# MarinerQ/npf_GWwaveform

Measured on AMD Instinct MI355X. Metric: waveform target-points/sec (train step), higher is better.
Workload: dtype f32 (every contraction of the step: fp32 operands as three exact bf16 terms, six v_mfma_f32_16x16x32_bf16 per product group, f32 accumulation -- f32 results, DESIGN.md 3.1 / 3.2; the 1-4-wide first / last layers: f32 FMAs); 1 GPU; BASELINE config 2: AttnCNP scaledot, r=256, 4-layer xy-encoder/decoder, 256 context / 1024 target points, 256 tasks per GPU (256 global), fp32 train step (fwd+loss+bwd+allreduce+Adam); tasks_per_gpu=256, global_tasks=256, context_points=256, target_points=1024, r_dim=256, n_params=799588, parallelism=dp1, hip_graph=True

## Files before the change

include/npf_hip.h:

```cpp
#ifndef NPF_HIP_H
#define NPF_HIP_H

#include <stdint.h>

#ifdef __cplusplus
extern "C" {
#endif

#define NPF_OK 0
#define NPF_EINVAL (-1)
#define NPF_ELAUNCH (-2)

#define NPF_MAX_OPS 40
#define NPF_MAX_FEATURES 512

enum npf_opcode {
  NPF_OP_END = 0,
  NPF_OP_LOAD_PT = 1,
  NPF_OP_STORE_PT = 2,
  NPF_OP_LOAD_ROWS = 3,
  NPF_OP_STORE_ROWS = 4,
  NPF_OP_LINEAR = 5,
  NPF_OP_SOFTMAX = 6,
  NPF_OP_ADD_PT = 7,
  NPF_OP_MASK_POS = 8,
  NPF_OP_ADD_TASKVEC = 9,
  NPF_OP_ROWDOT_PT = 10,
  NPF_OP_SOFTMAX_BWD = 11,
  NPF_OP_RELU = 12,
  NPF_OP_SCALE = 13,
  NPF_OP_STORE_TR = 14,
  NPF_OP_LAYERNORM = 15,
  NPF_OP_STORE_WB = 18,
  NPF_OP_STORE_TRB = 19,
  NPF_OP_LOAD_RM = 17,
  NPF_OP_STORE_MASK = 20,
  NPF_OP_MASK_BITS = 21,
  NPF_OP_LAYERNORM_BWD = 16
};

enum npf_wmode {
  NPF_W_ROWMAJOR = 0,
  NPF_W_PT_ROWS = 1,
  NPF_W_PT_COLS = 2
};

#define NPF_F_RELU 1u
#define NPF_F_ADD_PT 2u
#define NPF_F_MASK_PT 4u
#define NPF_F_P16 16u
#define NPF_F_MASK_BITS 32u
#define NPF_F_ADD_RM 8u
#define NPF_F_STORE_IN 64u
#define NPF_F_STORE_BITS 256u
#define NPF_F_STORE_P16 128u

typedef struct npf_op {
  int32_t op;
  int32_t i0;
  int32_t i1;
  int32_t i2;
  int32_t i3;
  uint32_t flags;
  float f0;
  int32_t i4;
  const void *p0;
  const void *p1;
  const void *p2;
  int64_t s0;
  int64_t s1;
  void *p3;
} npf_op_t;

typedef struct npf_program {
  int32_t n_ops;
  int32_t n_tasks;
  int32_t pts_per_task;
  int32_t tiles_per_task;
  int32_t wg_per_task;
  int32_t reserved[3];
  npf_op_t ops[NPF_MAX_OPS];
} npf_program_t;

int npf_chain_run(const npf_program_t *prog, void *stream);

typedef struct npf_wgrad_job {
  const float *dZ;
  const float *A;
  float *dW;
  float *db;
  int64_t ldw;
  int32_t N, K;
  int32_t per_task;
  int32_t accumulate;
  int32_t ldz, lda, ldo;
  int32_t reserved;
} npf_wgrad_job_t;
#define NPF_WGRAD_ACCUMULATE 1
#define NPF_WGRAD_BF16 2
#define NPF_WGRAD_DZ16 4
#define NPF_WGRAD_A16 8
#define NPF_WGRAD_F32X6 16
#define NPF_WGRAD_NO_H16 32

#define NPF_MAX_WGRAD_JOBS 16
int npf_wgrad_run(const npf_wgrad_job_t *jobs, int32_t n_jobs, int32_t n_tasks, int32_t tiles_per_task,
                  float *partials, int64_t partials_bytes, void *stream);
int64_t npf_wgrad_partials_bytes(const npf_wgrad_job_t *jobs, int32_t n_jobs, int32_t n_tasks,
                                 int32_t tiles_per_task);

int npf_gauss_head_fwd(const float *suff, int32_t n_rows, int32_t pts, int32_t dy, int32_t homoskedastic,
                       const float *Y, int32_t n_y_rows, float *loc, float *scale, float *sum_logp,
                       void *stream);
int npf_gauss_head_bwd(const float *suff, const float *loc, const float *scale, int32_t n_rows, int32_t pts,
                       int32_t dy, int32_t homoskedastic, const float *Y, int32_t n_y_rows,
                       const float *d_loc, const float *d_scale, const float *d_sum_logp, float *d_suff,
                       void *stream);

int npf_masked_gauss_head_fwd(const float *suff, const int32_t *n_valid, int32_t n_tasks, int32_t n_rows, int32_t pts, int32_t dy,
                              int32_t homoskedastic, const float *Y, int32_t n_y_rows, float *loc, float *scale,
                              float *sum_logp, void *stream);
int npf_masked_gauss_head_bwd(const float *suff, const float *loc, const float *scale, const int32_t *n_valid, int32_t n_tasks,
                              int32_t n_rows, int32_t pts, int32_t dy, int32_t homoskedastic, const float *Y, int32_t n_y_rows,
                              const float *d_loc, const float *d_scale, const float *d_sum_logp, float *d_suff, void *stream);

int npf_mixture_summary(const float *suff, const int32_t *n_valid, int32_t n_z, int32_t n_tasks, int32_t pts, int32_t dy,
                        int32_t homoskedastic, const float *z_p, int32_t n_probs, const float *probs, float *mean, float *std,
                        float *quant, void *stream);

int npf_mixture_score(const float *suff, const float *Y, const int32_t *n_valid, int32_t n_z, int32_t n_tasks, int32_t pts,
                      int32_t dy, int32_t homoskedastic, float *log_density, float *pit, float *crps, void *stream);

int npf_mc_objective_fwd(const float *log_w, int32_t n_z, int32_t n_tasks, int32_t mode, const float *inv_weights,
                         int32_t m, float *out, void *stream);
int npf_mc_objective_bwd(const float *log_w, int32_t n_z, int32_t n_tasks, int32_t mode, const float *inv_weights,
                         int32_t m, const float *d_out, float *d_log_w, float *workspace, void *stream);

int npf_mean_agg_fwd(const float *R_pt, int32_t n_tasks, int32_t pts_per_task, int32_t F, float *out,
                     void *stream);
int npf_mean_agg_bwd(const float *d_out, int32_t n_tasks, int32_t pts_per_task, int32_t F, float *dR_pt,
                     int32_t accumulate, void *stream);

int npf_pack_pt(const float *rows, int32_t n_tasks, int32_t pts_per_task, int32_t F_valid, float *pt,
                void *stream);
int npf_unpack_pt(const float *pt, int32_t n_tasks, int32_t pts_per_task, int32_t F_valid, float *rows,
                  void *stream);
int npf_transpose(const float *src, int32_t rows, int32_t cols, float *dst, void *stream);
int npf_split_heads(const float *src, int32_t n_tasks, int32_t pts_per_task, int32_t F, int32_t n_heads, float *dst,
                    void *stream);
int npf_merge_heads(const float *src, int32_t n_tasks, int32_t pts_per_task, int32_t F, int32_t n_heads, float *dst,
                    void *stream);

int npf_mha_fwd(const float *q, const float *k, const float *v, int32_t n_tasks, int32_t n_heads, int32_t n_keys,
                int32_t n_queries, int32_t F, float *out, float *lse, void *stream);
int npf_mha_bwd(const float *q, const float *k, const float *v, const float *out, const float *d_out, const float *lse,
                int32_t n_tasks, int32_t n_heads, int32_t n_keys, int32_t n_queries, int32_t F, float *d_q, float *d_k, float *d_v,
                void *stream);

int npf_add_layernorm_fwd(const float *a, const float *b, const float *gamma, const float *beta, float eps, int32_t n_tasks,
                          int32_t pts_per_task, int32_t F, float *y, float *stats, void *stream);
int npf_add_layernorm_bwd(const float *a, const float *b, const float *gamma, const float *stats, const float *dy, int32_t n_tasks,
                          int32_t pts_per_task, int32_t F, float *dx, float *partials, void *stream);

int npf_gather_points(const float *x, const float *y, const int64_t *idx, int32_t n_tasks, int32_t n_points,
                      int32_t n_sel, int32_t x_dim, int32_t y_dim, float *out_x, float *out_y, void *stream);

int npf_cast_bf16_weights(const float *src, int32_t n_rows, int32_t n_cols, int32_t ld, int32_t transposed, void *dst,
                          void *stream);

typedef struct npf_wprep_job {
  const float *src;
  void *dst;
  int32_t n_rows, n_cols, ld, kind;
} npf_wprep_job_t;
#define NPF_MAX_WPREP_JOBS 32
int npf_prepare_weights(const npf_wprep_job_t *jobs, int32_t n_jobs, void *stream);

#define NPF_X6_MAX_LAYERS 8
typedef struct {
  const void *w_img;
  const float *bias;
  const float *mask;
  float *store_in;
  float *store_out;
  const float *addend;
  unsigned long long *store_bits;
  const unsigned long long *mask_bits;
  int32_t relu;
  int32_t reserved;
} npf_x6_layer_t;
int npf_mlp_x6_run(const npf_x6_layer_t *layers, int32_t n_layers, const float *x, float *y, int32_t n_tasks,
                   int32_t tiles_per_task, void *stream);
int npf_mlp_x6_run_rows(const npf_x6_layer_t *layers, int32_t n_layers, const float *x, const float *in_rows, const float *in_w,
                        float *y, const float *out_w, const float *out_b, float *out_rows, int32_t n_tasks,
                        int32_t tiles_per_task, void *stream);

#define NPF_X6_MAX_OPS 12
typedef struct npf_x6_op {
  const float *in_pt;
  const float *in_rows;
  const float *in_w;
  const float *in_b;
  const float *pre_add;
  const float *mask;
  const unsigned long long *mask_bits;
  const float *sbwd_p;
  float *store_in;
  unsigned long long *store_in_bits;
  const void *w_img;
  int64_t w_task_stride;
  const float *bias;
  int64_t bias_task_stride;
  const float *addend;
  float *store_out;
  unsigned long long *store_bits;
  int32_t in_n;
  int32_t in_relu;
  int32_t relu;
  int32_t softmax_n;
  float softmax_scale;
  float sbwd_scale;
  int32_t reserved[2];
} npf_x6_op_t;
#define NPF_X6_IN_RM 1
#define NPF_X6_ADD_RM 2
#define NPF_X6_STORE_IN_F32 4
#define NPF_X6_STORE_OUT_F32 8
#define NPF_X6_DEFAULT_VARIANT 3
int npf_x6_run_ex(const npf_x6_op_t *ops, int32_t n_ops, const float *out_w, const float *out_b, float *out_rows,
                  int32_t n_tasks, int32_t tiles_per_task, int32_t pts_per_task, int32_t per_task, int32_t width,
                  int32_t variant, void *stream);
int npf_x6_run(const npf_x6_op_t *ops, int32_t n_ops, const float *out_w, const float *out_b, float *out_rows,
               int32_t n_tasks, int32_t tiles_per_task, int32_t per_task, int32_t width, void *stream);
int npf_x6_task_images(const float *src, int32_t n_tasks, int32_t pts, int32_t width, void *row_img, void *tr_img, void *stream);

int npf_b16_run(const npf_x6_op_t *ops, int32_t n_ops, const float *out_w, const float *out_b, float *out_rows, int32_t n_tasks,
                int32_t tiles_per_task, int32_t per_task, int32_t width, int32_t variant, void *stream);
int npf_b16_task_images(const float *src, int32_t n_tasks, int32_t pts, int32_t width, void *row_img, void *tr_img, void *stream);

int npf_masked_attn_fwd(const float *q, const float *k, const float *v, const int32_t *n_valid, int32_t n_tasks, int32_t n_keys,
                        int32_t n_queries, int32_t d, float scale, float *out, float *lse, void *stream);
int npf_masked_attn_bwd(const float *q, const float *k, const float *v, const int32_t *n_valid, const float *out, const float *d_out,
                        const float *lse, int32_t n_tasks, int32_t n_keys, int32_t n_queries, int32_t d, float scale, float *d_q,
                        float *d_k, float *d_v, void *stream);
int npf_masked_attn_fwd_nq(const float *q, const float *k, const float *v, const int32_t *n_valid, const int32_t *n_q_valid,
                           int32_t n_tasks, int32_t n_keys, int32_t n_queries, int32_t d, float scale, float *out, float *lse,
                           void *stream);
int npf_masked_attn_bwd_nq(const float *q, const float *k, const float *v, const int32_t *n_valid, const int32_t *n_q_valid,
                           const float *out, const float *d_out, const float *lse, int32_t n_tasks, int32_t n_keys, int32_t n_queries,
                           int32_t d, float scale, float *d_q, float *d_k, float *d_v, void *stream);
int npf_masked_attn_fwd_prefix(const float *q, const float *k_pre, const float *v_pre, const int32_t *n_prefix, const float *k_tail,
                               const float *v_tail, const int32_t *n_tail, const int32_t *n_q_valid, int32_t n_tasks,
                               int32_t n_prefix_tasks, int32_t c_pad, int32_t m_tail, int32_t n_queries, int32_t d, float scale,
                               float *out, void *stream);
int npf_masked_attn_fwd_loo(const float *q, const float *k, const float *v, const int32_t *n_valid, const int32_t *n_q_valid,
                            int32_t n_tasks, int32_t n_keys, int32_t n_queries, int32_t d, float scale, float *out, void *stream);
int npf_masked_mean_fwd(const float *R_pt, const int32_t *n_valid, int32_t n_tasks, int32_t pts_per_task, int32_t F, float *out,
                        void *stream);
int npf_masked_mean_bwd(const float *d_out, const int32_t *n_valid, int32_t n_tasks, int32_t pts_per_task, int32_t F, float *dR_pt,
                        int32_t accumulate, void *stream);
int npf_loo_mean(const float *R_pt, const int32_t *n_valid, int32_t n_tasks, int32_t pts_per_task, int32_t F, float *out,
                 void *stream);

#define NPF_APPEND_MAX_PAIRS 3
typedef struct npf_append_pair {
  const float *src;
  float *dst;
  int32_t F;
  int32_t reserved;
} npf_append_pair_t;
int npf_append_points(const npf_append_pair_t *pairs, int32_t n_pairs, int32_t *n_valid, const int32_t *n_new, int32_t n_tasks,
                      int32_t n_rows, int32_t capacity, void *stream);

int npf_version(void);

#ifdef __cplusplus
}
#endif
#endif
```

npf_gwwaveform_amd/_lib.py:

```python
from __future__ import annotations

import ctypes as C
import os
from typing import Optional

import torch

from . import _build

NPF_MAX_OPS = 40
NPF_MAX_FEATURES = 512
NPF_WGRAD_BLOCK = 256
NPF_MAX_FUSED_ROW = 256

OP_END, OP_LOAD_PT, OP_STORE_PT, OP_LOAD_ROWS, OP_STORE_ROWS, OP_LINEAR, OP_SOFTMAX, OP_ADD_PT, OP_MASK_POS, \
    OP_ADD_TASKVEC, OP_ROWDOT_PT, OP_SOFTMAX_BWD, OP_RELU, OP_SCALE, OP_STORE_TR, OP_LAYERNORM, OP_LAYERNORM_BWD, OP_LOAD_RM, OP_STORE_WB, OP_STORE_TRB, \
    OP_STORE_MASK, OP_MASK_BITS = range(22)
W_ROWMAJOR, W_PT_ROWS, W_PT_COLS = range(3)
F_RELU, F_ADD_PT, F_MASK_PT, F_ADD_RM, F_P16, F_MASK_BITS, F_STORE_IN, F_STORE_P16, F_STORE_BITS = 1, 2, 4, 8, 16, 32, 64, 128, 256


class NpfOp(C.Structure):
    _fields_ = [
        ("op", C.c_int32), ("i0", C.c_int32), ("i1", C.c_int32), ("i2", C.c_int32), ("i3", C.c_int32),
        ("flags", C.c_uint32), ("f0", C.c_float), ("i4", C.c_int32),
        ("p0", C.c_void_p), ("p1", C.c_void_p), ("p2", C.c_void_p),
        ("s0", C.c_int64), ("s1", C.c_int64), ("p3", C.c_void_p),
    ]


class NpfProgram(C.Structure):
    _fields_ = [
        ("n_ops", C.c_int32), ("n_tasks", C.c_int32), ("pts_per_task", C.c_int32), ("tiles_per_task", C.c_int32),
        ("wg_per_task", C.c_int32), ("reserved", C.c_int32 * 3),
        ("ops", NpfOp * NPF_MAX_OPS),
    ]


class NpfWgradJob(C.Structure):
    _fields_ = [
        ("dZ", C.c_void_p), ("A", C.c_void_p), ("dW", C.c_void_p), ("db", C.c_void_p), ("ldw", C.c_int64),
        ("N", C.c_int32), ("K", C.c_int32), ("per_task", C.c_int32), ("accumulate", C.c_int32),
        ("ldz", C.c_int32), ("lda", C.c_int32), ("ldo", C.c_int32), ("reserved", C.c_int32),
    ]


NPF_MAX_WGRAD_JOBS = 16
WGRAD_F32X6 = 16
WGRAD_NO_H16 = 32


class NpfWprepJob(C.Structure):
    _fields_ = [("src", C.c_void_p), ("dst", C.c_void_p), ("n_rows", C.c_int32), ("n_cols", C.c_int32), ("ld", C.c_int32),
                ("kind", C.c_int32)]


NPF_MAX_WPREP_JOBS = 32
NPF_X6_MAX_LAYERS = 8


class NpfX6Layer(C.Structure):
    _fields_ = [("w_img", C.c_void_p), ("bias", C.c_void_p), ("mask", C.c_void_p), ("store_in", C.c_void_p),
                ("store_out", C.c_void_p), ("addend", C.c_void_p), ("store_bits", C.c_void_p), ("mask_bits", C.c_void_p),
                ("relu", C.c_int32), ("reserved", C.c_int32)]


NPF_X6_MAX_OPS = 12
X6_IN_RM, X6_ADD_RM = 1, 2
X6_STORE_IN_F32, X6_STORE_OUT_F32 = 4, 8


class NpfX6Op(C.Structure):
    _fields_ = [("in_pt", C.c_void_p), ("in_rows", C.c_void_p), ("in_w", C.c_void_p), ("in_b", C.c_void_p),
                ("pre_add", C.c_void_p), ("mask", C.c_void_p), ("mask_bits", C.c_void_p), ("sbwd_p", C.c_void_p),
                ("store_in", C.c_void_p), ("store_in_bits", C.c_void_p), ("w_img", C.c_void_p), ("w_task_stride", C.c_int64),
                ("bias", C.c_void_p), ("bias_task_stride", C.c_int64), ("addend", C.c_void_p), ("store_out", C.c_void_p),
                ("store_bits", C.c_void_p), ("in_n", C.c_int32), ("in_relu", C.c_int32), ("relu", C.c_int32),
                ("softmax_n", C.c_int32), ("softmax_scale", C.c_float), ("sbwd_scale", C.c_float), ("reserved", C.c_int32 * 2)]


NPF_APPEND_MAX_PAIRS = 3


class NpfAppendPair(C.Structure):
    _fields_ = [("src", C.c_void_p), ("dst", C.c_void_p), ("F", C.c_int32), ("reserved", C.c_int32)]


assert C.sizeof(NpfAppendPair) == 24
assert C.sizeof(NpfX6Op) == 17 * 8 + 8 * 4
assert C.sizeof(NpfOp) == 80 and C.sizeof(NpfProgram) == 32 + 80 * NPF_MAX_OPS and C.sizeof(NpfWgradJob) == 72 and C.sizeof(NpfWprepJob) == 32

_i32, _i64, _p = C.c_int32, C.c_int64, C.c_void_p
SIGNATURES = {
    "npf_chain_run": (C.c_int, [C.POINTER(NpfProgram), _p]),
    "npf_wgrad_run": (C.c_int, [C.POINTER(NpfWgradJob), _i32, _i32, _i32, _p, _i64, _p]),
    "npf_wgrad_partials_bytes": (_i64, [C.POINTER(NpfWgradJob), _i32, _i32, _i32]),
    "npf_gauss_head_fwd": (C.c_int, [_p, _i32, _i32, _i32, _i32, _p, _i32, _p, _p, _p, _p]),
    "npf_gauss_head_bwd": (C.c_int, [_p, _p, _p, _i32, _i32, _i32, _i32, _p, _i32, _p, _p, _p, _p, _p]),
    "npf_mc_objective_fwd": (C.c_int, [_p, _i32, _i32, _i32, _p, _i32, _p, _p]),
    "npf_mc_objective_bwd": (C.c_int, [_p, _i32, _i32, _i32, _p, _i32, _p, _p, _p, _p]),
    "npf_mean_agg_fwd": (C.c_int, [_p, _i32, _i32, _i32, _p, _p]),
    "npf_mean_agg_bwd": (C.c_int, [_p, _i32, _i32, _i32, _p, _i32, _p]),
    "npf_pack_pt": (C.c_int, [_p, _i32, _i32, _i32, _p, _p]),
    "npf_unpack_pt": (C.c_int, [_p, _i32, _i32, _i32, _p, _p]),
    "npf_transpose": (C.c_int, [_p, _i32, _i32, _p, _p]),
    "npf_cast_bf16_weights": (C.c_int, [_p, _i32, _i32, _i32, _i32, _p, _p]),
    "npf_prepare_weights": (C.c_int, [C.POINTER(NpfWprepJob), _i32, _p]),
    "npf_gather_points": (C.c_int, [_p, _p, _p, _i32, _i32, _i32, _i32, _i32, _p, _p, _p]),
    "npf_split_heads": (C.c_int, [_p, _i32, _i32, _i32, _i32, _p, _p]),
    "npf_merge_heads": (C.c_int, [_p, _i32, _i32, _i32, _i32, _p, _p]),
    "npf_mlp_x6_run": (C.c_int, [C.POINTER(NpfX6Layer), _i32, _p, _p, _i32, _i32, _p]),
    "npf_mlp_x6_run_rows": (C.c_int, [C.POINTER(NpfX6Layer), _i32, _p, _p, _p, _p, _p, _p, _p, _i32, _i32, _p]),
    "npf_x6_run": (C.c_int, [C.POINTER(NpfX6Op), _i32, _p, _p, _p, _i32, _i32, _i32, _i32, _p]),
    "npf_x6_run_ex": (C.c_int, [C.POINTER(NpfX6Op), _i32, _p, _p, _p, _i32, _i32, _i32, _i32, _i32, _i32, _p]),
    "npf_x6_task_images": (C.c_int, [_p, _i32, _i32, _i32, _p, _p, _p]),
    "npf_b16_run": (C.c_int, [C.POINTER(NpfX6Op), _i32, _p, _p, _p, _i32, _i32, _i32, _i32, _i32, _p]),
    "npf_b16_task_images": (C.c_int, [_p, _i32, _i32, _i32, _p, _p, _p]),
    "npf_mha_fwd": (C.c_int, [_p, _p, _p, _i32, _i32, _i32, _i32, _i32, _p, _p, _p]),
    "npf_mha_bwd": (C.c_int, [_p, _p, _p, _p, _p, _p, _i32, _i32, _i32, _i32, _i32, _p, _p, _p, _p]),
    "npf_add_layernorm_fwd": (C.c_int, [_p, _p, _p, _p, C.c_float, _i32, _i32, _i32, _p, _p, _p]),
    "npf_add_layernorm_bwd": (C.c_int, [_p, _p, _p, _p, _p, _i32, _i32, _i32, _p, _p, _p]),
    "npf_masked_attn_fwd": (C.c_int, [_p, _p, _p, _p, _i32, _i32, _i32, _i32, C.c_float, _p, _p, _p]),
    "npf_masked_attn_bwd": (C.c_int, [_p, _p, _p, _p, _p, _p, _p, _i32, _i32, _i32, _i32, C.c_float, _p, _p, _p, _p]),
    "npf_masked_attn_fwd_nq": (C.c_int, [_p, _p, _p, _p, _p, _i32, _i32, _i32, _i32, C.c_float, _p, _p, _p]),
    "npf_masked_attn_bwd_nq": (C.c_int, [_p, _p, _p, _p, _p, _p, _p, _p, _i32, _i32, _i32, _i32, C.c_float, _p, _p, _p, _p]),
    "npf_masked_attn_fwd_prefix": (C.c_int, [_p, _p, _p, _p, _p, _p, _p, _p, _i32, _i32, _i32, _i32, _i32, _i32, C.c_float, _p, _p]),
    "npf_masked_attn_fwd_loo": (C.c_int, [_p, _p, _p, _p, _p, _i32, _i32, _i32, _i32, C.c_float, _p, _p]),
    "npf_loo_mean": (C.c_int, [_p, _p, _i32, _i32, _i32, _p, _p]),
    "npf_masked_gauss_head_fwd": (C.c_int, [_p, _p, _i32, _i32, _i32, _i32, _i32, _p, _i32, _p, _p, _p, _p]),
    "npf_masked_gauss_head_bwd": (C.c_int, [_p, _p, _p, _p, _i32, _i32, _i32, _i32, _i32, _p, _i32, _p, _p, _p, _p, _p]),
    "npf_mixture_summary": (C.c_int, [_p, _p, _i32, _i32, _i32, _i32, _i32, _p, _i32, _p, _p, _p, _p, _p]),
    "npf_mixture_score": (C.c_int, [_p, _p, _p, _i32, _i32, _i32, _i32, _i32, _p, _p, _p, _p]),
    "npf_masked_mean_fwd": (C.c_int, [_p, _p, _i32, _i32, _i32, _p, _p]),
    "npf_masked_mean_bwd": (C.c_int, [_p, _p, _i32, _i32, _i32, _p, _i32, _p]),
    "npf_append_points": (C.c_int, [C.POINTER(NpfAppendPair), _i32, _p, _p, _i32, _i32, _i32, _p]),
    "npf_version": (C.c_int, []),
}

_lib: Optional[C.CDLL] = None


def lib_path() -> str:
    return os.environ.get("NPF_HIP_LIB") or _build.LIB_PATH


def load() -> C.CDLL:
    global _lib
    if _lib is not None:
        return _lib
    path = lib_path()
    if not os.path.exists(path):
        raise RuntimeError(
            f"HIP extension {path} is missing. Build it with `python -m npf_gwwaveform_amd._build` "
            "(needs hipcc); there is no CPU fallback for the neural-process path."
        )
    try:
        lib = C.CDLL(path)
    except OSError as e:
        raise RuntimeError(f"HIP extension {path} failed to load: {e}") from e
    for name, (res, args) in SIGNATURES.items():
        fn = getattr(lib, name)
        fn.restype = res
        fn.argtypes = args
    _lib = lib
    return lib


def check(rc: int, what: str) -> None:
    if rc != 0:
        raise RuntimeError(f"{what} failed with status {rc} "
                           f"({'invalid argument/unsupported size' if rc == -1 else 'kernel launch error'})")


def stream_ptr(device: Optional[torch.device] = None) -> int:
    return torch.cuda.current_stream(device).cuda_stream


def ptr(t: Optional[torch.Tensor], strided: bool = False) -> Optional[int]:
    if t is None:
        return None
    if not t.is_cuda:
        raise RuntimeError("the HIP path takes device tensors only (got a CPU tensor); there is no CPU fallback")
    if t.dtype != torch.float32:
        raise RuntimeError(f"the HIP path computes in fp32 (got {t.dtype})")
    if not strided and not t.is_contiguous():
        raise RuntimeError("tensor handed to the HIP path must be contiguous")
    return t.data_ptr()
```

npf_gwwaveform_amd/chain.py:

```python
from __future__ import annotations

import ctypes as C
import os
import sys
from dataclasses import dataclass, field
from typing import List, Optional, Sequence, Tuple

import torch

from . import _lib as L


PROFILE = None
TRACE = None
DEBUG_ABLATE = 0
FORCE_WG = int(os.environ.get("NPF_FORCE_WG", "0"))
PT16_INTERNAL = os.environ.get("NPF_NO_PT16", "0") != "1"
MASK_BITS = os.environ.get("NPF_NO_MASK_BITS", "0") != "1"
PAD_SMALL_K = os.environ.get("NPF_NO_PAD_SMALL_K", "0") != "1"
DUMP_PROGRAMS = os.environ.get("NPF_DUMP_PROGRAMS", "0") == "1"
FUSE_STORES = os.environ.get("NPF_NO_FUSED_STORE", "0") != "1"
WGRAD_X6 = os.environ.get("NPF_NO_WGRAD_X6", "0") != "1"
X6_NARROW_NATIVE = os.environ.get("NPF_X6_ALL", "0") != "1"
WGRAD_H16 = os.environ.get("NPF_NO_WGRAD_H16", "0") != "1"
# ... 208 lines not shown
            raise ValueError("a program is either all-fp32 or all-bf16")
        ok = W_img.dtype == torch.bfloat16 and W_img.is_contiguous() and W_img.shape[-1] == pad32(K)
        ok = ok and ((W_img.dim() == 3 and W_img.shape[0] == self.n_tasks and W_img.shape[1] >= N) if per_task
                     else tuple(W_img.shape) == (N, pad32(K)))
        if not ok:
            raise ValueError(f"bad bf16 weight image {tuple(W_img.shape)} {W_img.dtype} for a {K}->{N} layer")
        self.bf16 = True
        if true_K is not None:
            self._pad_k += (K - true_K) * N
        p_add, fl_add = self._pt(addend) if addend is not None else (None, 0)
        flags = (L.F_RELU if relu else 0) | ((L.F_ADD_PT | fl_add) if addend is not None else 0)
        p3 = None
        last = self.ops[-1] if self.ops else None
        if FUSE_STORES and last is not None and last.op == L.OP_STORE_PT and last.i0 == pad32(K):
            self.ops.pop()
            p3 = last.p0
            flags |= L.F_STORE_IN | (L.F_STORE_P16 if last.flags & L.F_P16 else 0)
        self.keep.append(W_img)
        self._op(op=L.OP_LINEAR, i0=K, i1=N, i2=L.W_ROWMAJOR, i3=pad32(K) // 2, flags=flags, i4=addend_modulus,
                 p0=W_img.data_ptr(), p1=self._p(bias), p2=p_add, p3=p3,
                 s0=(W_img.shape[1] * pad32(K) // 2 if per_task else 0), s1=b_task_stride)

    def store_wb(self, img, F):
        self.bf16 = True
        self.keep.append(img)
        self._op(op=L.OP_STORE_WB, i0=F, i1=img.shape[1], p0=img.data_ptr())

    def store_trb(self, img, F):
        self.bf16 = True
        self.keep.append(img)
        self._op(op=L.OP_STORE_TRB, i0=F, i1=img.shape[2], p0=img.data_ptr())

    def flops(self) -> int:
        return (sum(2 * o.i0 * o.i1 for o in self.ops if o.op == L.OP_LINEAR) - 2 * self._pad_k) * self.n_tasks * self.pts

    def hbm_bytes(self) -> int:
        pts = self.n_tasks * tiles_of(self.pts) * 32
        per_pt = 0
        fixed = 0
        for o in self.ops:
            if o.op in (L.OP_LOAD_PT, L.OP_STORE_PT, L.OP_ADD_PT, L.OP_MASK_POS, L.OP_ROWDOT_PT, L.OP_SOFTMAX_BWD,
                        L.OP_LOAD_RM):
                per_pt += (2 if o.flags & L.F_P16 else 4) * o.i0
            elif o.op in (L.OP_LOAD_ROWS, L.OP_STORE_ROWS, L.OP_STORE_TR):
                per_pt += 4 * o.i0
            elif o.op in (L.OP_STORE_WB, L.OP_STORE_TRB):
                per_pt += 2 * pad32(o.i0)
            elif o.op in (L.OP_STORE_MASK, L.OP_MASK_BITS):
                per_pt += 16 * ((o.i0 + 127) // 128)
            elif o.op == L.OP_SOFTMAX and o.i1:
                per_pt += 8
            elif o.op == L.OP_LAYERNORM_BWD:
                per_pt += 4 * pad32(o.i0) * (2 if o.p2 else 1)
            elif o.op == L.OP_LINEAR:
                if o.flags & (L.F_ADD_PT | L.F_MASK_PT | L.F_ADD_RM):
                    per_pt += (2 if o.flags & L.F_P16 else 4) * pad32(o.i1)
                if o.flags & (L.F_MASK_BITS | L.F_STORE_BITS):
                    per_pt += 16 * ((pad32(o.i1) + 127) // 128)
                if o.flags & L.F_STORE_IN:
                    per_pt += (2 if o.flags & L.F_STORE_P16 else 4) * pad32(o.i0)
                per_task = o.i2 != L.W_ROWMAJOR or o.s0 != 0
                fixed += 4 * o.i0 * o.i1 * (self.n_tasks if per_task else 1)
        return per_pt * pts + fixed - 4 * self._pad_k

    def launch(self) -> None:
        if not self.ops:
            return
        if PROFILE is not None:
            ev0, ev1 = torch.cuda.Event(enable_timing=True), torch.cuda.Event(enable_timing=True)
            ev0.record()
            self._launch()
            ev1.record()
            PROFILE.append(("chain_kernel", self.flops(), ev0, ev1, self.hbm_bytes()))
        else:
            self._launch()

    def only_rows_loaded(self) -> bool:
        return bool(self.ops) and self.ops[0].op == L.OP_LOAD_ROWS and all(o.op == L.OP_STORE_PT for o in self.ops[1:])

    def describe(self) -> str:
        names = {v: k[3:] for k, v in vars(L).items() if k.startswith("OP_")}
        flag_names = [(L.F_RELU, "relu"), (L.F_ADD_PT, "add_pt"), (L.F_MASK_PT, "mask_pt"), (L.F_ADD_RM, "add_rm"),
                      (L.F_P16, "p16"), (L.F_MASK_BITS, "mask_bits"), (L.F_STORE_IN, "store_in"),
                      (L.F_STORE_P16, "store_p16"), (L.F_STORE_BITS, "store_bits")]
        lines = [f"program: {self.n_tasks} tasks x {self.pts} points, wg_per_task={int(self.wg_per_task)}, bf16={int(self.bf16)}"]
        for o in self.ops:
            fl = "|".join(n for b, n in flag_names if o.flags & b)
            lines.append(f"  {names.get(o.op, o.op):12s} i0={o.i0:4d} i1={o.i1:4d} i2={o.i2} i4={o.i4} {fl}")
        return "\n".join(lines)

    def _launch(self) -> None:
        if DUMP_PROGRAMS:
            print(self.describe(), file=sys.stderr)
        prog = L.NpfProgram()
        prog.n_ops = len(self.ops)
        prog.n_tasks, prog.pts_per_task, prog.tiles_per_task = self.n_tasks, self.pts, tiles_of(self.pts)
        prog.wg_per_task = int(self.wg_per_task)
        prog.reserved[0] = DEBUG_ABLATE
        prog.reserved[1] = FORCE_WG
        prog.reserved[2] = int(self.bf16)
        for i, o in enumerate(self.ops):
            prog.ops[i] = o
        L.check(L.load().npf_chain_run(C.byref(prog), L.stream_ptr()), "npf_chain_run")


def run_wgrad(jobs: Sequence[dict], n_tasks: int, pts: int, device, tag: str = "") -> None:
    if not jobs:
        return
    if PROFILE is not None:
        ev0, ev1 = torch.cuda.Event(enable_timing=True), torch.cuda.Event(enable_timing=True)
        ev0.record()
        _run_wgrad(jobs, n_tasks, pts, device)
        ev1.record()
        padded = n_tasks * tiles_of(pts) * 32
        nbytes = sum((j["dZ"].element_size() * pad32(j["N"]) + j["A"].element_size() * pad32(j["K"])) * padded
                     + 4 * j["N"] * j["K"] * (n_tasks if j.get("per_task") else 1) for j in jobs)
        PROFILE.append(("wgrad_kernel", sum(2 * j["N"] * j["K"] for j in jobs) * n_tasks * pts, ev0, ev1, nbytes, tag))
    else:
        _run_wgrad(jobs, n_tasks, pts, device)


def _block_jobs(jobs: Sequence[dict]) -> List[dict]:
    Bk = L.NPF_WGRAD_BLOCK
    out = []
    for jb in jobs:
        N, K = jb["N"], jb["K"]
        if N <= Bk and K <= Bk:
            out.append(jb)
            continue
        if jb.get("per_task") and N > Bk:
            raise NotImplementedError("per-task weight gradients (attention keys / values) over more than 256 points")
        dZ, A = jb["dZ"], jb["A"]
        Fz, Fa = pad32(N), pad32(K)
        ldw = jb.get("ldw") or K
        for n0 in range(0, N, Bk):
            for k0 in range(0, K, Bk):
                blk = dict(jb, N=min(Bk, N - n0), K=min(Bk, K - k0), ldz=Fz, lda=Fa,
                           dZ_off=n0 * 32, A_off=k0 * 32)
                if jb.get("per_task"):
                    blk.update(dW_off=k0 * 32, ldo=Fa)
                else:
                    blk.update(dW_off=n0 * ldw + k0, ldw=ldw, db=jb.get("db") if k0 == 0 else None, db_off=n0)
                out.append(blk)
    return out


def _run_wgrad(jobs: Sequence[dict], n_tasks: int, pts: int, device) -> None:
    jobs = _block_jobs(jobs)
    x6 = WGRAD_X6 and COMPUTE_DTYPE != "bf16"
    if x6 and X6_NARROW_NATIVE:
        narrow = [jb for jb in jobs if min(jb["N"], jb["K"]) <= 32]
        wide = [jb for jb in jobs if min(jb["N"], jb["K"]) > 32]
        if narrow and wide:
            _launch_wgrad(wide, n_tasks, pts, device, True)
            _launch_wgrad(narrow, n_tasks, pts, device, False)
            return
        x6 = bool(wide)
    _launch_wgrad(jobs, n_tasks, pts, device, x6)


def _launch_wgrad(jobs: Sequence[dict], n_tasks: int, pts: int, device, x6: bool) -> None:
    lib = L.load()
    for i0 in range(0, len(jobs), L.NPF_MAX_WGRAD_JOBS):
        chunk = jobs[i0:i0 + L.NPF_MAX_WGRAD_JOBS]
        arr = (L.NpfWgradJob * len(chunk))()
        for j, jb in enumerate(chunk):
            z16, a16 = jb["dZ"].dtype == torch.bfloat16, jb["A"].dtype == torch.bfloat16
            if (z16 or a16) and COMPUTE_DTYPE != "bf16":
                raise RuntimeError("PT16 operands exist in the bf16 compute mode only")
            arr[j].dZ = (jb["dZ"].data_ptr() if z16 else L.ptr(jb["dZ"])) + jb.get("dZ_off", 0) * jb["dZ"].element_size()
            arr[j].A = (jb["A"].data_ptr() if a16 else L.ptr(jb["A"])) + jb.get("A_off", 0) * jb["A"].element_size()
            arr[j].dW = L.ptr(jb["dW"]) + 4 * jb.get("dW_off", 0)
            arr[j].db = (L.ptr(jb["db"]) + 4 * jb.get("db_off", 0)) if jb.get("db") is not None else None
            arr[j].ldz, arr[j].lda, arr[j].ldo = jb.get("ldz", 0), jb.get("lda", 0), jb.get("ldo", 0)
            arr[j].ldw = jb.get("ldw") or jb["K"]
            arr[j].N, arr[j].K = jb["N"], jb["K"]
            arr[j].per_task = int(jb.get("per_task", False))
            arr[j].accumulate = (int(jb.get("accumulate", False)) | (2 if COMPUTE_DTYPE == "bf16" else 0)
                                 | (4 if z16 else 0) | (8 if a16 else 0)
                                 | (L.WGRAD_F32X6 if x6 else 0) | (L.WGRAD_NO_H16 if (x6 and not WGRAD_H16) else 0))
        nbytes = lib.npf_wgrad_partials_bytes(arr, len(chunk), n_tasks, tiles_of(pts))
        if nbytes < 0:
            raise RuntimeError("npf_wgrad_partials_bytes: invalid wgrad jobs")
        ws = torch.empty((nbytes + 3) // 4, dtype=torch.float32, device=device)
        L.check(lib.npf_wgrad_run(arr, len(chunk), n_tasks, tiles_of(pts), L.ptr(ws), nbytes, L.stream_ptr()),
                "npf_wgrad_run")


def cast_bf16_weights(W: torch.Tensor, transposed: bool = False) -> torch.Tensor:
    N, K = W.shape
    if W.stride(1) != 1:
        raise ValueError("weight rows must be contiguous")
    rows, cols = (K, N) if transposed else (N, K)
    out = torch.empty((rows, pad32(cols)), dtype=torch.bfloat16, device=W.device)
    L.check(L.load().npf_cast_bf16_weights(L.ptr(W, strided=True), N, K, W.stride(0), int(transposed), out.data_ptr(),
                                           L.stream_ptr()), "npf_cast_bf16_weights")
    return out


def prepare_weights(specs: Sequence[Tuple[torch.Tensor, int]], dsts: Optional[Sequence[torch.Tensor]] = None) -> List[torch.Tensor]:
    outs: List[torch.Tensor] = []
    lib = L.load()
    if dsts is not None:
        assert len(dsts) == len(specs) and os.environ.get("NPF_NO_BATCH_PREP") != "1"
    if os.environ.get("NPF_NO_BATCH_PREP") == "1":
        if any(kind & 4 for _, kind in specs):
            raise RuntimeError("NPF_NO_BATCH_PREP needs NPF_NO_PAD_SMALL_K=1 as well")
        return [transpose(W.contiguous()) if kind == 0 else cast_bf16_weights(W, transposed=kind == 2) for W, kind in specs]
    for i0 in range(0, len(specs), L.NPF_MAX_WPREP_JOBS):
        chunk = specs[i0:i0 + L.NPF_MAX_WPREP_JOBS]
        arr = (L.NpfWprepJob * len(chunk))()
        for j, (W, kind) in enumerate(chunk):
            N, K = W.shape
            if W.stride(1) != 1 or W.dtype != torch.float32:
                raise ValueError("weight rows must be contiguous fp32")
            if kind == 0:
                shape, dt = (K, N), torch.float32
            else:
                rows, cols = (K, N) if kind & 3 == 2 else (N, K)
                shape, dt = (rows, 256 if kind & 4 else pad32(cols)), torch.bfloat16
            if dsts is not None:
                out = dsts[i0 + j]
                if tuple(out.shape) != shape or out.dtype != dt or not out.is_contiguous():
                    raise ValueError(f"prepare_weights: destination {tuple(out.shape)} {out.dtype} for an image {shape} {dt}")
            else:
                out = torch.empty(shape, dtype=dt, device=W.device)
            arr[j].src, arr[j].dst = L.ptr(W, strided=True), out.data_ptr()
            arr[j].n_rows, arr[j].n_cols, arr[j].ld, arr[j].kind = N, K, W.stride(0), kind
            outs.append(out)
        L.check(lib.npf_prepare_weights(arr, len(chunk), L.stream_ptr()), "npf_prepare_weights")
    return outs


def transpose(W: torch.Tensor) -> torch.Tensor:
    rows, cols = W.shape
    out = torch.empty((cols, rows), dtype=torch.float32, device=W.device)
    L.check(L.load().npf_transpose(L.ptr(W.contiguous()), rows, cols, L.ptr(out), L.stream_ptr()), "npf_transpose")
    return out


@dataclass
class _Step:
    kind: str
    t: dict = field(default_factory=dict)
    a: dict = field(default_factory=dict)


class Chain:

    def __init__(self, n_tasks: int, pts_per_task: int, device, wg_per_task: bool = False):
        self.n_tasks, self.pts, self.device, self.wg_per_task = n_tasks, pts_per_task, device, wg_per_task
        self.steps: List[_Step] = []
        self.tensors: List[Optional[torch.Tensor]] = []
        self.F = 0

    def _t(self, t: Optional[torch.Tensor]) -> int:
        if t is None:
            return -1
        self.tensors.append(t)
        return len(self.tensors) - 1

    def input_pt(self, t: torch.Tensor, F: int, modulus: int = 0) -> "Chain":
        self.steps.append(_Step("input_pt", {"x": self._t(t)}, {"F": F, "mod": modulus}))
        self.F = F
        return self

    def input_rm(self, t: torch.Tensor, F: int, modulus: int = 0) -> "Chain":
        if F % 32 or not t.is_contiguous() or t.shape[-1] != F:
            raise ValueError("input_rm needs a contiguous tensor with a multiple of 32 features")
        self.steps.append(_Step("input_rm", {"x": self._t(t)}, {"F": F, "mod": modulus}))
        self.F = F
        return self

    def input_rows(self, t: torch.Tensor, kd: int, modulus: int = 0) -> "Chain":
        if kd > 32:
            raise NotImplementedError("row-major chain inputs are limited to 32 features")
        self.steps.append(_Step("input_rows", {"x": self._t(t)}, {"kd": kd, "mod": modulus}))
        self.F = kd
        return self

    def linear(self, W: torch.Tensor, b: Optional[torch.Tensor], relu: bool = False,
               addend: Optional[torch.Tensor] = None, addend_modulus: int = 0,
               bias_per_task: bool = False, addend_rm: bool = False, residual: bool = False) -> "Chain":
        N, K = W.shape
        if residual and N != K:
            raise ValueError(f"a residual layer keeps its width, got {K} -> {N}")
        if addend_rm and (addend is None or N % 32 or not addend.is_contiguous() or addend.shape[-1] != N):
            raise ValueError("a row-major addend must be contiguous with N % 32 == 0 features")
        if K != self.F:
            raise ValueError(f"Linear expects {K} inputs, chain carries {self.F}")
        if max(N, K) > L.NPF_MAX_FEATURES:
            raise NotImplementedError(
                f"layer {K}->{N}: the HIP chain keeps at most {L.NPF_MAX_FEATURES} features in registers")
        if W.stride(1) != 1:
            raise ValueError("weight rows must be contiguous")
        if bias_per_task and not self.wg_per_task:
            raise ValueError("per-task biases need wg_per_task=True")
        self.steps.append(_Step("linear", {"W": self._t(W), "b": self._t(b), "add": self._t(addend)},
                                {"N": N, "K": K, "relu": relu, "mod": addend_modulus, "bpt": bias_per_task,
                                 "add_rm": addend_rm, "res": residual}))
        self.F = N
        return self

    def add_pt(self, t: torch.Tensor, relu: bool = False, modulus: int = 0) -> "Chain":
        self.steps.append(_Step("add_pt", {"x": self._t(t)}, {"F": self.F, "relu": relu, "mod": modulus}))
        return self

    def dropout(self, sign_mask: torch.Tensor, p: float) -> "Chain":
        if not 0.0 <= p < 1.0:
            raise ValueError(f"dropout probability {p}")
        self.steps.append(_Step("dropout", {"m": self._t(sign_mask)}, {"F": self.F, "p": float(p)}))
        return self

    def add_taskvec(self, v: torch.Tensor, relu: bool = False, modulus: int = 0) -> "Chain":
        self.steps.append(_Step("add_taskvec", {"v": self._t(v)}, {"F": self.F, "relu": relu, "mod": modulus}))
        return self

    def layernorm(self, weight: torch.Tensor, bias: torch.Tensor, eps: float = 1e-5) -> "Chain":
        if self.F > L.NPF_MAX_FUSED_ROW or weight.shape != (self.F,) or bias.shape != (self.F,):
            raise ValueError(f"LayerNorm over {self.F} features with parameters {tuple(weight.shape)}")
        self.steps.append(_Step("layernorm", {"g": self._t(weight), "b": self._t(bias)}, {"F": self.F, "eps": float(eps)}))
        return self

    def store_bf16_images(self) -> "Chain":
        self.steps.append(_Step("store_wb", {}, {"F": self.F}))
        self.steps.append(_Step("store_trb", {}, {"F": self.F}))
        return self

    def attn_scores(self, keys_pt: torch.Tensor, n_keys: int, keys_tr: Optional[torch.Tensor] = None,
                    keys_img=None) -> "Chain":
        if not self.wg_per_task:
            raise ValueError("attention needs wg_per_task=True")
        if n_keys > L.NPF_MAX_FUSED_ROW:
# ... 452 lines not shown
```

npf_gwwaveform_amd/csrc/layout_kernels.hip:

```cpp
#include "npf_common.hpp"

namespace npf {

__global__ void pack_pt_kernel(const float* __restrict__ rows, int n_tasks, int pts, int Fv, int Fp, float* __restrict__ pt) {
  const int tiles = (pts + 31) / 32;
  const size_t total = (size_t)n_tasks * tiles * (Fp / 4) * 32;
  for (size_t idx = blockIdx.x * (size_t)blockDim.x + threadIdx.x; idx < total; idx += (size_t)gridDim.x * blockDim.x) {
    const int p = idx & 31;
    const size_t r = idx >> 5;
    const int f4 = r % (Fp / 4);
    const size_t tt = r / (Fp / 4);
    const int tile = tt % tiles;
    const size_t task = tt / tiles;
    const int point = tile * 32 + p;
    f32x4 v = {0.f, 0.f, 0.f, 0.f};
    if (point < pts) {
      const float* src = rows + (task * pts + point) * (size_t)Fv + 4 * f4;
#pragma unroll
      for (int j = 0; j < 4; ++j)
        if (4 * f4 + j < Fv) v[j] = src[j];
    }
    *(f32x4*)(pt + idx * 4) = v;
  }
}

__global__ void unpack_pt_kernel(const float* __restrict__ pt, int n_tasks, int pts, int Fv, int Fp, float* __restrict__ rows) {
  const int tiles = (pts + 31) / 32;
  const size_t total = (size_t)n_tasks * tiles * (Fp / 4) * 32;
  for (size_t idx = blockIdx.x * (size_t)blockDim.x + threadIdx.x; idx < total; idx += (size_t)gridDim.x * blockDim.x) {
    const int p = idx & 31;
    const size_t r = idx >> 5;
    const int f4 = r % (Fp / 4);
    const size_t tt = r / (Fp / 4);
    const int tile = tt % tiles;
    const size_t task = tt / tiles;
    const int point = tile * 32 + p;
    if (point < pts) {
      const f32x4 v = *(const f32x4*)(pt + idx * 4);
      float* dst = rows + (task * pts + point) * (size_t)Fv + 4 * f4;
#pragma unroll
      for (int j = 0; j < 4; ++j)
        if (4 * f4 + j < Fv) dst[j] = v[j];
    }
  }
}

template <bool SPLIT>
__global__ void heads_kernel(const float* __restrict__ src, int n_tasks, int pts, int Fp, int hsz, int n_heads,
                             float* __restrict__ dst) {
  const int tiles = (pts + 31) / 32;
  const int hq = ((hsz + 31) / 32) * 8;
  const int fq = Fp / 4;
  if (SPLIT) {
    const size_t total = (size_t)n_heads * n_tasks * tiles * hq * 32;
    for (size_t idx = blockIdx.x * (size_t)blockDim.x + threadIdx.x; idx < total; idx += (size_t)gridDim.x * blockDim.x) {
      const int p = idx & 31;
      const size_t r = idx >> 5;
      const int q = r % hq;
      const size_t tt = r / hq;
      const int tile = tt % tiles;
      const size_t ht = tt / tiles;
      const int h = ht / n_tasks, b = ht - (size_t)h * n_tasks;
      f32x4 v = {0.f, 0.f, 0.f, 0.f};
      if (4 * q < hsz) v = *(const f32x4*)(src + ((((size_t)b * tiles + tile) * fq + (h * hsz) / 4 + q) * 32 + p) * 4);
      *(f32x4*)(dst + idx * 4) = v;
    }
  } else {
    const size_t total = (size_t)n_tasks * tiles * fq * 32;
    for (size_t idx = blockIdx.x * (size_t)blockDim.x + threadIdx.x; idx < total; idx += (size_t)gridDim.x * blockDim.x) {
      const int p = idx & 31;
      const size_t r = idx >> 5;
      const int q = r % fq;
      const size_t tt = r / fq;
      const int tile = tt % tiles;
      const size_t b = tt / tiles;
      const int h = (4 * q) / hsz, qh = q - (h * hsz) / 4;
      f32x4 v = {0.f, 0.f, 0.f, 0.f};
      if (h < n_heads) v = *(const f32x4*)(src + (((((size_t)h * n_tasks + b) * tiles + tile) * hq + qh) * 32 + p) * 4);
      *(f32x4*)(dst + idx * 4) = v;
    }
  }
}

__global__ void gather_points_kernel(const float* __restrict__ x, const float* __restrict__ y,
                                     const long long* __restrict__ idx, int n_tasks, int n_points, int n_sel, int x_dim,
                                     int y_dim, float* __restrict__ out_x, float* __restrict__ out_y) {
  const size_t total = (size_t)n_tasks * n_sel;
  for (size_t t = blockIdx.x * (size_t)blockDim.x + threadIdx.x; t < total; t += (size_t)gridDim.x * blockDim.x) {
    const size_t b = t / n_sel;
    long long j = idx[t];
    j = j < 0 ? 0 : (j >= n_points ? n_points - 1 : j);
    const float* xs = x + (b * n_points + (size_t)j) * x_dim;
    for (int d = 0; d < x_dim; ++d) out_x[t * x_dim + d] = xs[d];
    if (y) {
      const float* ys = y + (b * n_points + (size_t)j) * y_dim;
      for (int d = 0; d < y_dim; ++d) out_y[t * y_dim + d] = ys[d];
    }
  }
}

__global__ void cast_bf16_weights_kernel(const float* __restrict__ src, int n_rows, int n_cols, int ld, int transposed,
                                         unsigned short* __restrict__ dst) {
  const int rows = transposed ? n_cols : n_rows, cols = transposed ? n_rows : n_cols;
  const int Kp = ((cols + 31) >> 5) * 32;
  const size_t total = (size_t)rows * Kp;
  for (size_t idx = blockIdx.x * (size_t)blockDim.x + threadIdx.x; idx < total; idx += (size_t)gridDim.x * blockDim.x) {
    const int r = idx / Kp, q = idx - (size_t)r * Kp;
    const int sgrp = q >> 5, g = (q & 31) >> 3, i = q & 7;
    const int c = 32 * sgrp + (i < 4 ? 4 * g + i : 16 + 4 * g + (i - 4));
    float v = 0.f;
    if (c < cols) v = transposed ? src[(size_t)c * ld + r] : src[(size_t)r * ld + c];
    const __bf16 b = (__bf16)v;
    dst[idx] = __builtin_bit_cast(unsigned short, b);
  }
}

__global__ void transpose_kernel(const float* __restrict__ src, int rows, int cols, float* __restrict__ dst) {
  __shared__ float tile[32][33];
  const int c0 = blockIdx.x * 32, r0 = blockIdx.y * 32;
  const int tx = threadIdx.x & 31, ty = threadIdx.x >> 5;
  for (int i = ty; i < 32; i += 8)
    if (r0 + i < rows && c0 + tx < cols) tile[i][tx] = src[(size_t)(r0 + i) * cols + c0 + tx];
  __syncthreads();
  for (int i = ty; i < 32; i += 8)
    if (c0 + i < cols && r0 + tx < rows) dst[(size_t)(c0 + i) * rows + r0 + tx] = tile[tx][i];
}

struct WprepJobs {
  npf_wprep_job_t job[NPF_MAX_WPREP_JOBS];
};
__global__ void prepare_weights_kernel(const WprepJobs J) {
  __shared__ float tile[32][33];
  const npf_wprep_job_t& jb = J.job[blockIdx.y];
  const float* __restrict__ src = jb.src;
  if (jb.kind == 0) {
    float* __restrict__ dst = (float*)jb.dst;
    const int rows = jb.n_rows, cols = jb.n_cols, ld = jb.ld;
    const int tc = (cols + 31) / 32, tr = (rows + 31) / 32;
    const int tx = threadIdx.x & 31, ty = threadIdx.x >> 5;
    for (int tl = blockIdx.x; tl < tc * tr; tl += gridDim.x) {
      const int c0 = (tl % tc) * 32, r0 = (tl / tc) * 32;
      for (int i = ty; i < 32; i += 8)
        if (r0 + i < rows && c0 + tx < cols) tile[i][tx] = src[(size_t)(r0 + i) * ld + c0 + tx];
      __syncthreads();
      for (int i = ty; i < 32; i += 8)
        if (c0 + i < cols && r0 + tx < rows) dst[(size_t)(c0 + i) * rows + r0 + tx] = tile[tx][i];
      __syncthreads();
    }
  } else {
    unsigned short* __restrict__ dst = (unsigned short*)jb.dst;
    const bool transposed = (jb.kind & 3) == 2;
    const int term = (jb.kind >> 4) & 3;
    const int rows = transposed ? jb.n_cols : jb.n_rows, cols = transposed ? jb.n_rows : jb.n_cols, ld = jb.ld;
    const int Kp = (jb.kind & 4) ? 256 : ((cols + 31) >> 5) * 32;
    const size_t total = (size_t)rows * Kp;
    for (size_t idx = blockIdx.x * (size_t)blockDim.x + threadIdx.x; idx < total; idx += (size_t)gridDim.x * blockDim.x) {
      const int r = idx / Kp, q = idx - (size_t)r * Kp;
      const int sgrp = q >> 5, g = (q & 31) >> 3, i = q & 7;
      const int c = 32 * sgrp + (i < 4 ? 4 * g + i : 16 + 4 * g + (i - 4));
      float v = 0.f;
      if (c < cols) v = transposed ? src[(size_t)c * ld + r] : src[(size_t)r * ld + c];
      for (int t = 1; t < term; ++t) v -= (float)(__bf16)v;
      const __bf16 b = (__bf16)v;
      dst[idx] = __builtin_bit_cast(unsigned short, b);
    }
  }
}

template <bool MASKED>
__global__ void mean_fwd_kernel(const float* __restrict__ R, const int32_t* __restrict__ n_valid, int pts, int F,
                                float* __restrict__ out) {
  const int tiles = (pts + 31) / 32;
  const int p = threadIdx.x & 31, f4 = blockIdx.x * 8 + (threadIdx.x >> 5);
  const size_t task = blockIdx.y;
  const int n = MASKED ? clamp_count(n_valid, task, pts) : pts;
  const bool in_F = MASKED || f4 < F / 4;
  f32x4 s = {0.f, 0.f, 0.f, 0.f};
  if (in_F) {
    const float* base = R + task * tiles * (size_t)(F * 32) + pt_off(f4, p);
    for (int t = 0; t * 32 < n; ++t)
      if (t * 32 + p < n) s += *(const f32x4*)(base + (size_t)t * F * 32);
  }
#pragma unroll
  for (int off = 16; off >= 1; off >>= 1)
#pragma unroll
    for (int j = 0; j < 4; ++j) s[j] += __shfl_xor(s[j], off);
  if (p == 0 && in_F) *(f32x4*)(out + task * F + 4 * f4) = (!MASKED || n > 0) ? s * (1.f / (float)n) : f32x4{0.f, 0.f, 0.f, 0.f};
}

__global__ void loo_mean_kernel(const float* __restrict__ R, const int32_t* __restrict__ n_valid, int pts, int F,
                                float* __restrict__ out) {
  const int tiles = (pts + 31) / 32;
  const int p = threadIdx.x & 31, f4 = blockIdx.x * 8 + (threadIdx.x >> 5);
  const size_t task = blockIdx.y;
  const int n = clamp_count(n_valid, task, pts);
  const size_t at = task * tiles * (size_t)(F * 32) + pt_off(f4, p);
  double s[4] = {0.0, 0.0, 0.0, 0.0};
  for (int t = 0; t * 32 < n; ++t)
    if (t * 32 + p < n) {
      const f32x4 r = *(const f32x4*)(R + at + (size_t)t * F * 32);
#pragma unroll
      for (int j = 0; j < 4; ++j) s[j] += (double)r[j];
    }
#pragma unroll
  for (int off = 16; off >= 1; off >>= 1)
#pragma unroll
    for (int j = 0; j < 4; ++j) s[j] += __shfl_xor(s[j], off);
  const double others = (double)(n - 1);
  for (int t = 0; t < tiles; ++t) {
    f32x4 v = {0.f, 0.f, 0.f, 0.f};
    if (n > 1 && t * 32 + p < n) {
      const f32x4 r = *(const f32x4*)(R + at + (size_t)t * F * 32);
#pragma unroll
      for (int j = 0; j < 4; ++j) v[j] = (float)((s[j] - (double)r[j]) / others);
    }
    *(f32x4*)(out + at + (size_t)t * F * 32) = v;
  }
}

template <bool MASKED>
__global__ void mean_bwd_kernel(const float* __restrict__ d_out, const int32_t* __restrict__ n_valid, int n_tasks, int pts, int F,
                                float* __restrict__ dR, int accumulate) {
  const int tiles = (pts + 31) / 32;
  const size_t total = (size_t)n_tasks * tiles * (F / 4) * 32;
  for (size_t idx = blockIdx.x * (size_t)blockDim.x + threadIdx.x; idx < total; idx += (size_t)gridDim.x * blockDim.x) {
    const int p = idx & 31;
    const size_t r = idx >> 5;
    const int f4 = r % (F / 4);
    const size_t tt = r / (F / 4);
    const int tile = tt % tiles;
    const size_t task = tt / tiles;
    const int n = MASKED ? clamp_count(n_valid, task, pts) : pts;
    f32x4 v = {0.f, 0.f, 0.f, 0.f};
    if (tile * 32 + p < n) v = *(const f32x4*)(d_out + task * F + 4 * f4) * (1.f / (float)n);
    if (accumulate) v += *(const f32x4*)(dR + idx * 4);
    *(f32x4*)(dR + idx * 4) = v;
  }
}

static unsigned grid_for(size_t total, int block) {
  size_t g = (total + block - 1) / block;
  if (g > 256u * 8u) g = 256u * 8u;
  if (g == 0) g = 1;
  return (unsigned)g;
}

}

extern "C" int npf_pack_pt(const float* rows, int32_t n_tasks, int32_t pts, int32_t Fv, float* pt, void* stream) {
  if (!rows || !pt || n_tasks <= 0 || pts <= 0 || Fv <= 0) return NPF_EINVAL;
  const int Fp = npf::round_up(Fv, 32);
  const size_t total = (size_t)n_tasks * ((pts + 31) / 32) * (Fp / 4) * 32;
  hipLaunchKernelGGL(npf::pack_pt_kernel, dim3(npf::grid_for(total, 256)), dim3(256), 0, (hipStream_t)stream, rows, n_tasks,
                     pts, Fv, Fp, pt);
  NPF_CHECK_LAUNCH();
  return NPF_OK;
}

extern "C" int npf_unpack_pt(const float* pt, int32_t n_tasks, int32_t pts, int32_t Fv, float* rows, void* stream) {
  if (!rows || !pt || n_tasks <= 0 || pts <= 0 || Fv <= 0) return NPF_EINVAL;
  const int Fp = npf::round_up(Fv, 32);
  const size_t total = (size_t)n_tasks * ((pts + 31) / 32) * (Fp / 4) * 32;
  hipLaunchKernelGGL(npf::unpack_pt_kernel, dim3(npf::grid_for(total, 256)), dim3(256), 0, (hipStream_t)stream, pt,
                     n_tasks, pts, Fv, Fp, rows);
  NPF_CHECK_LAUNCH();
  return NPF_OK;
}

extern "C" int npf_transpose(const float* src, int32_t rows, int32_t cols, float* dst, void* stream) {
  if (!src || !dst || rows <= 0 || cols <= 0) return NPF_EINVAL;
  hipLaunchKernelGGL(npf::transpose_kernel, dim3((cols + 31) / 32, (rows + 31) / 32), dim3(256), 0, (hipStream_t)stream,
                     src, rows, cols, dst);
  NPF_CHECK_LAUNCH();
  return NPF_OK;
}

static int heads_launch(bool split, const float* src, int32_t n_tasks, int32_t pts, int32_t F, int32_t n_heads, float* dst,
                        void* stream) {
  if (!src || !dst || n_tasks <= 0 || pts <= 0 || F <= 0 || n_heads <= 0 || F % n_heads) return NPF_EINVAL;
  const int hsz = F / n_heads;
  if (hsz & 3) return NPF_EINVAL;
  const int Fp = npf::round_up(F, 32), tiles = (pts + 31) / 32;
  if (split) {
    const size_t total = (size_t)n_heads * n_tasks * tiles * (npf::round_up(hsz, 32) / 4) * 32;
    hipLaunchKernelGGL(npf::heads_kernel<true>, dim3(npf::grid_for(total, 256)), dim3(256), 0, (hipStream_t)stream, src,
                       n_tasks, pts, Fp, hsz, n_heads, dst);
  } else {
    const size_t total = (size_t)n_tasks * tiles * (Fp / 4) * 32;
    hipLaunchKernelGGL(npf::heads_kernel<false>, dim3(npf::grid_for(total, 256)), dim3(256), 0, (hipStream_t)stream, src,
                       n_tasks, pts, Fp, hsz, n_heads, dst);
  }
  NPF_CHECK_LAUNCH();
  return NPF_OK;
}

extern "C" int npf_gather_points(const float* x, const float* y, const int64_t* idx, int32_t n_tasks, int32_t n_points,
                                 int32_t n_sel, int32_t x_dim, int32_t y_dim, float* out_x, float* out_y, void* stream) {
  if (!x || !idx || !out_x || n_tasks <= 0 || n_points <= 0 || n_sel < 0 || x_dim <= 0) return NPF_EINVAL;
  if (y && (!out_y || y_dim <= 0)) return NPF_EINVAL;
  if (n_sel == 0) return NPF_OK;
  const size_t total = (size_t)n_tasks * n_sel;
  hipLaunchKernelGGL(npf::gather_points_kernel, dim3(npf::grid_for(total, 256)), dim3(256), 0, (hipStream_t)stream, x, y,
                     (const long long*)idx, n_tasks, n_points, n_sel, x_dim, y_dim, out_x, out_y);
  NPF_CHECK_LAUNCH();
  return NPF_OK;
}

extern "C" int npf_cast_bf16_weights(const float* src, int32_t n_rows, int32_t n_cols, int32_t ld, int32_t transposed,
                                     void* dst, void* stream) {
  if (!src || !dst || n_rows <= 0 || n_cols <= 0 || ld < n_cols || (((uintptr_t)dst) & 15)) return NPF_EINVAL;
  const int rows = transposed ? n_cols : n_rows, cols = transposed ? n_rows : n_cols;
  const size_t total = (size_t)rows * npf::round_up(cols, 32);
  hipLaunchKernelGGL(npf::cast_bf16_weights_kernel, dim3(npf::grid_for(total, 256)), dim3(256), 0, (hipStream_t)stream, src,
                     n_rows, n_cols, ld, transposed, (unsigned short*)dst);
  NPF_CHECK_LAUNCH();
  return NPF_OK;
}

extern "C" int npf_prepare_weights(const npf_wprep_job_t* jobs, int32_t n_jobs, void* stream) {
  if (!jobs || n_jobs <= 0 || n_jobs > NPF_MAX_WPREP_JOBS) return NPF_EINVAL;
  npf::WprepJobs J;
  size_t most = 0;
  for (int j = 0; j < n_jobs; ++j) {
    const npf_wprep_job_t& b = jobs[j];
    const int base = b.kind & 15, term = b.kind >> 4;
    const bool kind_ok = b.kind >= 0 && ((term == 0 && (base <= 2 || base == 5 || base == 6)) || (term >= 1 && term <= 3 && (base == 1 || base == 2)));
    if (!b.src || !b.dst || b.n_rows <= 0 || b.n_cols <= 0 || b.ld < b.n_cols || !kind_ok) return NPF_EINVAL;
    if (b.kind != 0 && (((uintptr_t)b.dst) & 15)) return NPF_EINVAL;
    if ((b.kind == 5 && b.n_cols > 256) || (b.kind == 6 && b.n_rows > 256)) return NPF_EINVAL;
    J.job[j] = b;
    const size_t img_rows = (b.kind & 3) == 2 ? b.n_cols : b.n_rows;
    const size_t blocks = b.kind == 0   ? (size_t)((b.n_rows + 31) / 32) * ((b.n_cols + 31) / 32)
                          : (b.kind & 4) ? (img_rows * 256 + 255) / 256
                                         : ((size_t)b.n_rows * b.n_cols + 255) / 256;
    most = blocks > most ? blocks : most;
  }
  for (int j = n_jobs; j < NPF_MAX_WPREP_JOBS; ++j) J.job[j] = jobs[0];
  const unsigned gx = (unsigned)(most < 64 ? most : 64);
  hipLaunchKernelGGL(npf::prepare_weights_kernel, dim3(gx ? gx : 1, n_jobs), dim3(256), 0, (hipStream_t)stream, J);
  NPF_CHECK_LAUNCH();
  return NPF_OK;
}

extern "C" int npf_split_heads(const float* src, int32_t n_tasks, int32_t pts, int32_t F, int32_t n_heads, float* dst,
                               void* stream) {
  return heads_launch(true, src, n_tasks, pts, F, n_heads, dst, stream);
}

extern "C" int npf_merge_heads(const float* src, int32_t n_tasks, int32_t pts, int32_t F, int32_t n_heads, float* dst,
                               void* stream) {
  return heads_launch(false, src, n_tasks, pts, F, n_heads, dst, stream);
}

extern "C" int npf_mean_agg_fwd(const float* R_pt, int32_t n_tasks, int32_t pts, int32_t F, float* out, void* stream) {
  if (!R_pt || !out || n_tasks <= 0 || pts <= 0 || F <= 0 || (F & 31)) return NPF_EINVAL;
  hipLaunchKernelGGL(npf::mean_fwd_kernel<false>, dim3(F / 32, n_tasks), dim3(256), 0, (hipStream_t)stream, R_pt, nullptr, pts, F,
                     out);
  NPF_CHECK_LAUNCH();
  return NPF_OK;
}

extern "C" int npf_mean_agg_bwd(const float* d_out, int32_t n_tasks, int32_t pts, int32_t F, float* dR_pt,
                                int32_t accumulate, void* stream) {
  if (!d_out || !dR_pt || n_tasks <= 0 || pts <= 0 || F <= 0 || (F & 31)) return NPF_EINVAL;
  const size_t total = (size_t)n_tasks * ((pts + 31) / 32) * (F / 4) * 32;
  hipLaunchKernelGGL(npf::mean_bwd_kernel<false>, dim3(npf::grid_for(total, 256)), dim3(256), 0, (hipStream_t)stream, d_out,
                     nullptr, n_tasks, pts, F, dR_pt, accumulate);
  NPF_CHECK_LAUNCH();
  return NPF_OK;
}

extern "C" int npf_masked_mean_fwd(const float* R_pt, const int32_t* n_valid, int32_t n_tasks, int32_t pts, int32_t F, float* out,
                                   void* stream) {
  if (!R_pt || !n_valid || !out || n_tasks < 0 || pts <= 0 || F <= 0 || (F & 31)) return NPF_EINVAL;
  if ((((uintptr_t)R_pt) | ((uintptr_t)out)) & 15) return NPF_EINVAL;
  if (n_tasks == 0) return NPF_OK;
  hipLaunchKernelGGL(npf::mean_fwd_kernel<true>, dim3(F / 32, n_tasks), dim3(256), 0, (hipStream_t)stream, R_pt, n_valid, pts, F, out);
  NPF_CHECK_LAUNCH();
  return NPF_OK;
}

extern "C" int npf_masked_mean_bwd(const float* d_out, const int32_t* n_valid, int32_t n_tasks, int32_t pts, int32_t F, float* dR_pt,
                                   int32_t accumulate, void* stream) {
  if (!d_out || !n_valid || !dR_pt || n_tasks < 0 || pts <= 0 || F <= 0 || (F & 31)) return NPF_EINVAL;
  if ((((uintptr_t)d_out) | ((uintptr_t)dR_pt)) & 15) return NPF_EINVAL;
  if (n_tasks == 0) return NPF_OK;
  const size_t total = (size_t)n_tasks * ((pts + 31) / 32) * (F / 4) * 32;
  hipLaunchKernelGGL(npf::mean_bwd_kernel<true>, dim3(npf::grid_for(total, 256)), dim3(256), 0, (hipStream_t)stream, d_out, n_valid,
                     n_tasks, pts, F, dR_pt, accumulate);
  NPF_CHECK_LAUNCH();
  return NPF_OK;
}

extern "C" int npf_loo_mean(const float* R_pt, const int32_t* n_valid, int32_t n_tasks, int32_t pts, int32_t F, float* out,
                            void* stream) {
  if (!R_pt || !n_valid || !out || n_tasks < 0 || pts <= 0 || F <= 0 || (F & 31)) return NPF_EINVAL;
  if ((((uintptr_t)R_pt) | ((uintptr_t)out)) & 15) return NPF_EINVAL;
  if (n_tasks == 0) return NPF_OK;
  if (n_tasks > 65535) return NPF_EINVAL;
  hipLaunchKernelGGL(npf::loo_mean_kernel, dim3(F / 32, n_tasks), dim3(256), 0, (hipStream_t)stream, R_pt, n_valid, pts, F, out);
  NPF_CHECK_LAUNCH();
  return NPF_OK;
}

extern "C" int npf_version(void) { return 2; }
```

npf_gwwaveform_amd/csrc/wgrad_kernel.hip:

```cpp
#include "npf_common.hpp"

namespace npf {

constexpr int kWgThreads = 1024;
constexpr int kWgWaves = kWgThreads / 64;
constexpr int kWgMaxF = 256;
constexpr int kQRows = kWgMaxF / 4;
constexpr int kMaxJobs = 16;

struct WgradJobs {
  npf_wgrad_job_t job[kMaxJobs];
  int32_t first_wg[kMaxJobs + 1];
  int32_t n_jobs;
  int32_t n_tasks;
  int32_t tiles_per_task;
  int32_t pad;
  int64_t part_off[kMaxJobs];
};

__device__ __forceinline__ void wg_dma16(const float* src, float* lds_dst_wave_uniform) {
  __builtin_amdgcn_global_load_lds((const __attribute__((address_space(1))) void*)src,
                                   (__attribute__((address_space(3))) void*)lds_dst_wave_uniform, 16, 0, 0);
}

// ... 747 lines not shown
        for (int r = 0; r < 16; ++r) {
          const int row = 64 * rg + 32 * i + (r & 3) + 8 * (r >> 2) + row_l, col = 128 * cp + 32 * c + col_l;
          part[(size_t)row * Kp + col] = acc[i][c][r];
        }
#pragma unroll
    for (int v = 0; v < 2; ++v) {
#pragma unroll
      for (int e = 0; e < 4; ++e) {
        float x = dbacc[v][e];
        x += __shfl_xor(x, 1);
        x += __shfl_xor(x, 2);
        x += __shfl_xor(x, 16);
        x += __shfl_xor(x, 32);
        dbacc[v][e] = x;
      }
      if (pt_ld == 0) *(f32x4*)(part + (size_t)Np * Kp + 4 * (8 * wave + 4 * v + q_ld)) = dbacc[v];
    }
  }
}

__global__ void wgrad_reduce_kernel(const WgradJobs J, const float* __restrict__ partials) {
  const int j = blockIdx.y;
  const npf_wgrad_job_t& job = J.job[j];
  if (job.per_task) return;
  const int n_split = J.first_wg[j + 1] - J.first_wg[j];
  const int Np = ((job.N + 31) >> 5) * 32, Kp = ((job.K + 31) >> 5) * 32;
  const size_t slab = (size_t)Np * Kp + Np;
  const float* part = partials + J.part_off[j];
  const int total4 = (Np * Kp + Np) >> 2;
  for (int i4 = blockIdx.x * blockDim.x + threadIdx.x; i4 < total4; i4 += gridDim.x * blockDim.x) {
    const float* p = part + (size_t)i4 * 4;
    f32x4 s0 = {0.f, 0.f, 0.f, 0.f}, s1 = s0, s2 = s0, s3 = s0;
    int sp = 0;
    for (; sp + 4 <= n_split; sp += 4) {
      s0 += *(const f32x4*)(p + (size_t)sp * slab);
      s1 += *(const f32x4*)(p + (size_t)(sp + 1) * slab);
      s2 += *(const f32x4*)(p + (size_t)(sp + 2) * slab);
      s3 += *(const f32x4*)(p + (size_t)(sp + 3) * slab);
    }
    for (; sp < n_split; ++sp) s0 += *(const f32x4*)(p + (size_t)sp * slab);
    const f32x4 s = (s0 + s1) + (s2 + s3);
    const int idx = i4 * 4;
    if (idx < Np * Kp) {
      const int n = idx / Kp, k = idx - n * Kp;
      if (n < job.N) {
        float* d = job.dW + (size_t)n * job.ldw + k;
#pragma unroll
        for (int e = 0; e < 4; ++e)
          if (k + e < job.K) d[e] = (job.accumulate & NPF_WGRAD_ACCUMULATE) ? d[e] + s[e] : s[e];
      }
    } else if (job.db) {
      const int n = idx - Np * Kp;
#pragma unroll
      for (int e = 0; e < 4; ++e)
        if (n + e < job.N) job.db[n + e] = (job.accumulate & NPF_WGRAD_ACCUMULATE) ? job.db[n + e] + s[e] : s[e];
    }
  }
}

static int plan(const npf_wgrad_job_t* jobs, int n_jobs, int n_tasks, int tiles_per_task, WgradJobs* J) {
  if (!jobs || n_jobs <= 0 || n_jobs > kMaxJobs || n_tasks <= 0 || tiles_per_task <= 0) return NPF_EINVAL;
  const long total_tiles = (long)n_tasks * tiles_per_task;
  int n_shared = 0;
  for (int j = 0; j < n_jobs; ++j) {
    const npf_wgrad_job_t& b = jobs[j];
    if (!b.dZ || !b.A || !b.dW || b.N <= 0 || b.K <= 0 || b.N > npf::kWgMaxF || b.K > npf::kWgMaxF) return NPF_EINVAL;
    if ((((uintptr_t)b.dZ) | ((uintptr_t)b.A)) & 15) return NPF_EINVAL;
    if (b.per_task && (((uintptr_t)b.dW) & 15)) return NPF_EINVAL;
    if (!b.per_task && b.ldw < b.K) return NPF_EINVAL;
    if (b.ldz < 0 || b.lda < 0 || b.ldo < 0 || (b.ldz & 31) || (b.lda & 31) || (b.ldo & 31)) return NPF_EINVAL;
    if ((b.ldz && b.ldz < npf::round_up(b.N, 32)) || (b.lda && b.lda < npf::round_up(b.K, 32)) ||
        (b.ldo && b.ldo < npf::round_up(b.K, 32)))
      return NPF_EINVAL;
    n_shared += b.per_task ? 0 : 1;
  }
  bool bf16 = true, x6 = true;
  for (int j = 0; j < n_jobs; ++j) {
    bf16 &= (jobs[j].accumulate & NPF_WGRAD_BF16) != 0;
    x6 &= (jobs[j].accumulate & (NPF_WGRAD_F32X6 | NPF_WGRAD_BF16)) == NPF_WGRAD_F32X6;
  }
  double cost[kMaxJobs], cost_sum = 0.0;
  for (int j = 0; j < n_jobs; ++j) {
    const int Np = npf::round_up(jobs[j].N, 32), Kp = npf::round_up(jobs[j].K, 32);
    const int ar = (Np + 63) / 64, ac = (Kp + 63) / 64;
    const double zb = (jobs[j].accumulate & NPF_WGRAD_DZ16) ? 2.0 : 4.0, ab = (jobs[j].accumulate & NPF_WGRAD_A16) ? 2.0 : 4.0;
    const double bytes = 32.0 * (Np * zb + Kp * ab);
    if (jobs[j].per_task) cost[j] = 0.0;
    else if (bf16) cost[j] = bytes > 18432.0 ? bytes : 18432.0;
    else if (x6) {
      const int waves = ar * ((ac + 1) / 2);
      const double mf = 3072.0 * 1.6 * ((waves + 3) / 4) + 2500.0, mem = bytes / 6.5;
      cost[j] = mf > mem ? mf : mem;
    } else {
      const double mf = 4096.0 * (ar < ac ? ar : ac), mem = bytes / 6.5;
      cost[j] = mf > mem ? mf : mem;
    }
    cost_sum += cost[j];
  }
  J->n_jobs = n_jobs;
  J->n_tasks = n_tasks;
  J->tiles_per_task = tiles_per_task;
  J->pad = 0;
  long splits_of[kMaxJobs];
  long used = 0;
  for (int j = 0; j < n_jobs; ++j) {
    splits_of[j] = 0;
    if (jobs[j].per_task) continue;
    long sp = (long)(256.0 * cost[j] / cost_sum);
    if (sp < 1) sp = 1;
    if (sp > total_tiles) sp = total_tiles;
    splits_of[j] = sp;
    used += sp;
  }
  for (int j = 0; j < n_jobs && used < 256; ++j)
    if (!jobs[j].per_task && cost[j] * n_shared >= cost_sum && splits_of[j] < total_tiles) {
      ++splits_of[j];
      ++used;
    }
  int wg = 0;
  int64_t off = 0;
  for (int j = 0; j < n_jobs; ++j) {
    J->job[j] = jobs[j];
    J->first_wg[j] = wg;
    J->part_off[j] = off;
    if (jobs[j].per_task) {
      wg += n_tasks;
    } else {
      const int Np = npf::round_up(jobs[j].N, 32), Kp = npf::round_up(jobs[j].K, 32);
      const long splits = splits_of[j];
      wg += (int)splits;
      off += (int64_t)splits * ((int64_t)Np * Kp + Np);
    }
  }
  J->first_wg[n_jobs] = wg;
  for (int j = n_jobs + 1; j <= kMaxJobs; ++j) J->first_wg[j] = wg;
  return (int)0;
}

}

extern "C" int64_t npf_wgrad_partials_bytes(const npf_wgrad_job_t* jobs, int32_t n_jobs, int32_t n_tasks,
                                            int32_t tiles_per_task) {
  npf::WgradJobs J;
  if (npf::plan(jobs, n_jobs, n_tasks, tiles_per_task, &J) != 0) return -1;
  int64_t off = 0;
  for (int j = 0; j < n_jobs; ++j) {
    if (jobs[j].per_task) continue;
    const int Np = npf::round_up(jobs[j].N, 32), Kp = npf::round_up(jobs[j].K, 32);
    off += (int64_t)(J.first_wg[j + 1] - J.first_wg[j]) * ((int64_t)Np * Kp + Np);
  }
  return off * 4 + 16;
}

extern "C" int npf_wgrad_run(const npf_wgrad_job_t* jobs, int32_t n_jobs, int32_t n_tasks, int32_t tiles_per_task,
                             float* partials, int64_t partials_bytes, void* stream) {
  npf::WgradJobs J;
  const int rc = npf::plan(jobs, n_jobs, n_tasks, tiles_per_task, &J);
  if (rc != 0) return rc;
  const int64_t need = npf_wgrad_partials_bytes(jobs, n_jobs, n_tasks, tiles_per_task);
  bool any_shared = false;
  for (int j = 0; j < n_jobs; ++j) any_shared |= !jobs[j].per_task;
  if (any_shared && (!partials || partials_bytes < need || (((uintptr_t)partials) & 15))) return NPF_EINVAL;
  const int n_wg = J.first_wg[n_jobs];
  bool bf16 = true, x6 = true;
  for (int j = 0; j < n_jobs; ++j) {
    bf16 &= (jobs[j].accumulate & NPF_WGRAD_BF16) != 0;
    x6 &= (jobs[j].accumulate & (NPF_WGRAD_F32X6 | NPF_WGRAD_BF16)) == NPF_WGRAD_F32X6;
  }
  bool h16 = x6;
  for (int j = 0; j < n_jobs; ++j) h16 &= jobs[j].N == 256 && jobs[j].K == 256 && !(jobs[j].accumulate & NPF_WGRAD_NO_H16);
  if (h16)
    hipLaunchKernelGGL(npf::wgrad_h16_kernel, dim3(n_wg), dim3(512), 0, (hipStream_t)stream, J, partials);
  else if (x6)
    hipLaunchKernelGGL(npf::wgrad_x6_kernel, dim3(n_wg), dim3(npf::kXThreads), 0, (hipStream_t)stream, J, partials);
  else if (bf16)
    hipLaunchKernelGGL(npf::wgrad_kernel<true>, dim3(n_wg), dim3(npf::kWgThreads), 0, (hipStream_t)stream, J, partials);
  else
    hipLaunchKernelGGL(npf::wgrad_kernel<false>, dim3(n_wg), dim3(npf::kWgThreads), 0, (hipStream_t)stream, J, partials);
  NPF_CHECK_LAUNCH();
  if (any_shared) {
    hipLaunchKernelGGL(npf::wgrad_reduce_kernel, dim3(65, n_jobs), dim3(256), 0, (hipStream_t)stream, J,
                       (const float*)partials);
    NPF_CHECK_LAUNCH();
  }
  return NPF_OK;
}
```

npf_gwwaveform_amd/functional.py:

```python
from __future__ import annotations

import os
from typing import Optional

import torch

from . import _lib as L
from .chain import pad32, pt_empty, pt_shape, tiles_of


def _pack(rows: torch.Tensor) -> torch.Tensor:
    n_tasks, pts, F = rows.shape
    out = pt_empty(n_tasks, pts, F, rows.device)
    L.check(L.load().npf_pack_pt(L.ptr(rows.contiguous()), n_tasks, pts, F, L.ptr(out), L.stream_ptr()), "npf_pack_pt")
    return out


def _unpack(pt: torch.Tensor, pts: int, F: int) -> torch.Tensor:
    n_tasks = pt.shape[0]
    out = torch.empty((n_tasks, pts, F), dtype=torch.float32, device=pt.device)
    L.check(L.load().npf_unpack_pt(L.ptr(pt.contiguous()), n_tasks, pts, F, L.ptr(out), L.stream_ptr()), "npf_unpack_pt")
    return out


class _PackFn(torch.autograd.Function):
    @staticmethod
    def forward(ctx, rows):
        ctx.pts, ctx.F = rows.shape[1], rows.shape[2]
        return _pack(rows)

    @staticmethod
    def backward(ctx, g):
        return _unpack(g.contiguous(), ctx.pts, ctx.F)


class _UnpackFn(torch.autograd.Function):
    @staticmethod
    def forward(ctx, pt, pts, F):
        return _unpack(pt, pts, F)

    @staticmethod
    def backward(ctx, g):
        return _pack(g.contiguous()), None, None


def pack_pt(rows: torch.Tensor) -> torch.Tensor:
    return _PackFn.apply(rows)


def unpack_pt(pt: torch.Tensor, pts: int, F: int) -> torch.Tensor:
    return _UnpackFn.apply(pt, pts, F)


def sum_points_pt(pt: torch.Tensor, pts: int, F: int) -> torch.Tensor:
    n_tasks = pt.shape[0]
    Fp = pad32(F)
    out = torch.empty((n_tasks, Fp), dtype=torch.float32, device=pt.device)
    L.check(L.load().npf_mean_agg_fwd(L.ptr(pt), n_tasks, pts, Fp, L.ptr(out), L.stream_ptr()), "npf_mean_agg_fwd")
    return out * float(pts)


class _MeanFn(torch.autograd.Function):

    @staticmethod
    def forward(ctx, pt, n_valid, n_tasks, pts, F):
        Fp = pad32(F)
        ctx.geo = (n_tasks, pts, Fp)
        if n_valid is not None:
            ctx.save_for_backward(n_valid)
        out = torch.empty((n_tasks, Fp), dtype=torch.float32, device=pt.device)
        name, counts = ("npf_mean_agg_fwd", ()) if n_valid is None else ("npf_masked_mean_fwd", (_iptr(n_valid),))
        L.check(getattr(L.load(), name)(L.ptr(pt.contiguous()), *counts, n_tasks, pts, Fp, L.ptr(out), L.stream_ptr()), name)
        return out

    @staticmethod
    def backward(ctx, g):
        n_tasks, pts, Fp = ctx.geo
        d = pt_empty(n_tasks, pts, Fp, g.device)
        name, counts = ("npf_masked_mean_bwd", (_iptr(ctx.saved_tensors[0]),)) if ctx.saved_tensors else ("npf_mean_agg_bwd", ())
        L.check(getattr(L.load(), name)(L.ptr(g.contiguous()), *counts, n_tasks, pts, Fp, L.ptr(d), 0, L.stream_ptr()), name)
        return d, None, None, None, None


def mean_agg(pt: torch.Tensor, pts: int, F: int) -> torch.Tensor:
    return _MeanFn.apply(pt, None, pt.shape[0], pts, F)


class _GaussHeadFn(torch.autograd.Function):

    @staticmethod
    def forward(ctx, suff, Y, n_valid, dy, homosk, want_dist):
        n_rows, pts, two_dy = suff.shape
        n_tasks = 1 if n_valid is None else n_valid.shape[0]
        assert two_dy == 2 * dy and n_rows % n_tasks == 0
        suff = suff.contiguous()
        loc = scale = None
        if want_dist:
            loc = torch.empty((n_rows, pts, dy), dtype=torch.float32, device=suff.device)
            scale = torch.empty_like(loc)
        slp = None
        n_y = 0
        if Y is not None:
            Y = Y.contiguous()
            n_y = Y.shape[0]
            assert Y.shape[1:] == (pts, dy) and n_rows % n_y == 0 and n_y % n_tasks == 0
            slp = torch.empty((n_rows,), dtype=torch.float32, device=suff.device)
        elif not want_dist:
            raise ValueError("a loss-only head launch needs the targets")
        name, counts = ("npf_gauss_head_fwd", ()) if n_valid is None else ("npf_masked_gauss_head_fwd", (_iptr(n_valid), n_tasks))
        L.check(getattr(L.load(), name)(L.ptr(suff), *counts, n_rows, pts, dy, int(homosk), L.ptr(Y), n_y, L.ptr(loc), L.ptr(scale),
                                        L.ptr(slp), L.stream_ptr()), name)
        ctx.save_for_backward(suff, loc, scale, Y, *(() if n_valid is None else (n_valid,)))
        ctx.cfg = (dy, homosk)
        empty = suff.new_zeros((0,))
        outs = [loc if want_dist else empty, scale if want_dist else empty, slp if slp is not None else suff.new_zeros((n_rows,))]
        nd = ([] if want_dist else [outs[0], outs[1]]) + ([] if slp is not None else [outs[2]])
        if nd:
            ctx.mark_non_differentiable(*nd)
        return tuple(outs)

    @staticmethod
    def backward(ctx, d_loc, d_scale, d_slp):
        suff, loc, scale, Y, *n_valid = ctx.saved_tensors
        dy, homosk = ctx.cfg
        n_rows, pts, _ = suff.shape
        d_suff = torch.empty_like(suff)
        c = lambda t: t.contiguous() if t is not None else None
        if loc is None:
            d_loc = d_scale = None
        name, counts = ("npf_masked_gauss_head_bwd", (_iptr(n_valid[0]), n_valid[0].shape[0])) if n_valid else ("npf_gauss_head_bwd", ())
        L.check(getattr(L.load(), name)(L.ptr(suff), L.ptr(loc), L.ptr(scale), *counts, n_rows, pts, dy, int(homosk), L.ptr(Y),
                                        Y.shape[0] if Y is not None else 0, L.ptr(c(d_loc)), L.ptr(c(d_scale)),
                                        L.ptr(c(d_slp)) if Y is not None else None, L.ptr(d_suff), L.stream_ptr()), name)
        return d_suff, None, None, None, None, None


def gauss_head(suff: torch.Tensor, Y: Optional[torch.Tensor], dy: int, homoskedastic: bool, want_dist: bool = True,
               n_valid: Optional[torch.Tensor] = None):
    if n_valid is not None:
        n_tasks = n_valid.shape[0] if isinstance(n_valid, torch.Tensor) and n_valid.dim() == 1 else suff.shape[0]
        if suff.shape[0] % max(n_tasks, 1) != 0 or n_tasks == 0:
            raise ValueError(f"n_valid has {n_tasks} counts, the head {suff.shape[0]} rows (not a multiple)")
        n_valid = counts_i32(n_valid, n_tasks)
    return _GaussHeadFn.apply(suff, Y, n_valid, dy, homoskedastic, want_dist)


MIXTURE_MAX_NZ = 128
_Z_P_CACHE = {}


def check_probs(probs) -> tuple:
    if isinstance(probs, torch.Tensor) or not isinstance(probs, (tuple, list)):
        raise ValueError(f"probs must be a host sequence (tuple / list) of probabilities, got {type(probs).__name__}")
    out = []
    for p in probs:
        if isinstance(p, torch.Tensor) or isinstance(p, bool) or not isinstance(p, (int, float)):
            raise ValueError(f"probs must hold host floats, got {type(p).__name__}")
        if not (0.0 < float(p) < 1.0):
            raise ValueError(f"probs must lie strictly inside (0, 1), got {p}")
        out.append(float(p))
    return tuple(out)


def normal_quantiles(probs) -> tuple:
    probs = check_probs(probs)
    if not probs:
        return ()
    return tuple(torch.special.ndtri(torch.tensor(probs, dtype=torch.float64)).tolist())


def _z_p_device(probs: tuple, device: torch.device):
    key = (probs, device.type, device.index if device.index is not None else torch.cuda.current_device())
    hit = _Z_P_CACHE.get(key)
    if hit is None:
        hit = (torch.tensor(normal_quantiles(probs), dtype=torch.float64).to(torch.float32).to(device),
# ... 422 lines not shown
```

npf_gwwaveform_amd/neuralproc.py:

```python
from __future__ import annotations

import abc
import math
from functools import partial
from typing import NamedTuple, Optional, Tuple

import torch
import torch.nn as nn
from torch.distributions import Independent, Normal

from . import functional as FN
from .architectures import (MLP, DotAttender, LeaveOneOut, MergeFlatInputs, MultiheadAttender, PrefixTail, SelfAttention,
                            get_attender, merge_flat_input)
from .chain import Chain, PTensor, pad32, pt_shape

__all__ = ["NeuralProcessFamily", "LatentNeuralProcessFamily", "CNP", "LNP", "AttnCNP", "AttnLNP",
           "MultivariateNormalDiag", "HeadDistribution", "Conditioned", "Prediction", "Score"]


def MultivariateNormalDiag(loc, scale_diag):
    if loc.dim() < 1:
        raise ValueError("loc must be at least one-dimensional.")
    return Independent(Normal(loc, scale_diag, validate_args=False), 1)

# ... 394 lines not shown
            Xc_pt, R_pts = x6.context_side(self, X_cntxt, Y_cntxt)
            return Xc_pt, self._pool_pt(R_pts, B)
        Xc_pt = self._xenc_pt(X_cntxt, with_tr=self._attentive and not fused_t) if C > 0 else None
        return Xc_pt, self._encode_globally_pt(Xc_pt, Y_cntxt, B, C)

    def _target_stage(self, Xc_pt, R, X_trgt, Y_trgt, B, C, n_cntxt, n_trgt, fused_t, latent=None):
        T = X_trgt.shape[1]
        padded = n_cntxt is not None and C > 0
        n_valid = n_cntxt if padded else None
        X_raw = None
        if padded:
            Xt_pt = self._xenc_pt(X_trgt)
        elif fused_t:
            Xt_pt, X_raw = None, X_trgt
        elif self._xenc_with_query_projection(C, T):
            from . import x6

            Xt_pt, q_proj = x6.xenc_proj(self, X_trgt, self.attender.query_transform)
            Xt_pt.proj = q_proj
        else:
            Xt_pt = self._xenc_pt(X_trgt)
        self._X_trgt_raw = X_raw
        try:
            if latent is not None:
                z_samples, q_zCc, q_zCct = latent[0], latent[1], None
            elif self.encoded_path in ["latent", "both"]:
                z_samples, q_zCc, q_zCct = self._latent_path_pt(R, C, Xt_pt, Y_trgt, B, T, n_valid=n_valid, n_trgt=n_trgt)
            else:
                z_samples, q_zCc, q_zCct = None, None, None
            if self.encoded_path == "latent":
                R = None
            suff = self._target_suffstat(Xc_pt, z_samples, R, Xt_pt, B, C, T, n_valid=n_valid,
                                         n_q_valid=n_trgt if padded else None)
        finally:
            self._X_trgt_raw = None
        return self._head(suff, Y_trgt, B, T, n_trgt=n_trgt), z_samples, q_zCc, q_zCct

    def _n_z_for(self, n_z_samples=None) -> Optional[int]:
        return None

    def condition(self, X_cntxt, Y_cntxt, n_cntxt=None, n_z_samples=None) -> "Conditioned":
        with torch.no_grad():
            n_z = self._n_z_for(n_z_samples)
            if n_cntxt is not None:
                n_cntxt = self._check_counts(n_cntxt, X_cntxt, "n_cntxt")
            self._check_tensors(X_cntxt, Y_cntxt)
            B, C, _ = X_cntxt.shape
            if n_z is not None:
                self.n_z_samples = n_z
            fused_t = self._fused_target_side(C, 1)
            Xc_pt, R = self._context_stage(X_cntxt, Y_cntxt, n_cntxt, fused_t)
            z_samples = q_zCc = None
            if n_z is not None:
                q_zCc = self._infer_q_zCc(R, B, n_cntxt if C > 0 else None)
                z_samples = q_zCc.rsample([n_z])
        return Conditioned(self, Xc_pt, R, z_samples, q_zCc, n_cntxt, B, C, fused_t)

    def condition_with_capacity(self, X_cntxt, Y_cntxt, capacity, n_cntxt=None, n_z_samples=None) -> "Conditioned":
        self._refuse_unimplemented("capacity")
        with torch.no_grad():
            n_z = self._n_z_for(n_z_samples)
            if X_cntxt.dim() != 3 or Y_cntxt.dim() != 3 or X_cntxt.shape[:2] != Y_cntxt.shape[:2]:
                raise ValueError(f"X_cntxt / Y_cntxt must be [B, C, x_dim] / [B, C, y_dim], got {list(X_cntxt.shape)} / {list(Y_cntxt.shape)}")
            B, C, _ = X_cntxt.shape
            capacity = int(capacity)
            if capacity < max(C, 1):
                raise ValueError(f"capacity={capacity} must be at least the context size C={C} (and at least 1)")
            self._check_tensors(X_cntxt, Y_cntxt)
            if n_cntxt is not None:
                n_cntxt = self._check_counts(n_cntxt, X_cntxt, "n_cntxt")
            if n_z is not None:
                self.n_z_samples = n_z
            dev = X_cntxt.device
            R_pts = PTensor(torch.zeros(pt_shape(B, capacity, self.r_dim), device=dev), capacity, self.r_dim)
            Xc_pt = PTensor(torch.zeros(pt_shape(B, capacity, self.x_transf_dim), device=dev), capacity, self.x_transf_dim)
            counts = torch.zeros(B, dtype=torch.int32, device=dev)
            post = Conditioned(self, Xc_pt, R_pts if self._attentive else torch.zeros(B, 1, self.r_dim, device=dev), None, None, counts,
                               B, C, False, capacity=capacity, R_pts=R_pts)
            if C > 0:
                Xn_pt, Rn_pts = self._encode_points(X_cntxt, Y_cntxt)
                pairs = [(Rn_pts.t, R_pts.t, self.r_dim), (Xn_pt.t, Xc_pt.t, self.x_transf_dim)]
                FN.append_points(pairs, counts, n_cntxt, B, C, capacity)
            post._refresh()
            if n_z is not None:
                post.q_zCc = q = self._infer_q_zCc(post._R, B, counts)
                post.eps = torch.randn(n_z, B, 1, self.z_dim, device=dev)
                post.z_samples = q.base_dist.loc + q.base_dist.scale * post.eps
        return post

    def loo(self, X_cntxt, Y_cntxt, n_cntxt=None) -> HeadDistribution:
        self._refuse_loo()
        if X_cntxt.dim() != 3 or Y_cntxt.dim() != 3 or X_cntxt.shape[:2] != Y_cntxt.shape[:2]:
            raise ValueError(f"X_cntxt / Y_cntxt must be [B, C, x_dim] / [B, C, y_dim], got {list(X_cntxt.shape)} / {list(Y_cntxt.shape)}")
        B, C, _ = X_cntxt.shape
        if C == 0:
            raise ValueError("loo: no context points")
        with torch.no_grad():
            if n_cntxt is not None:
                n_cntxt = self._check_counts(n_cntxt, X_cntxt, "n_cntxt")
            self._check_tensors(X_cntxt, Y_cntxt)
            if n_cntxt is None:
                n_cntxt = torch.full((B,), C, dtype=torch.int32, device=X_cntxt.device)
            Xc_pt, R_pts = self._encode_points(X_cntxt, Y_cntxt)
            return self._loo_from(Xc_pt, R_pts, n_cntxt, B, C)

    def _refuse_loo(self):
        if self.encoded_path != "deterministic":
            raise NotImplementedError("loo is not implemented for latent models (LNP / AttnLNP): q(z | C without i) differs per "
                                      "left-out point and the decoder takes one z per task")
        self._refuse_unimplemented("loo")

    def _loo_from(self, Xc_pt, R_pts, n, B, rows) -> HeadDistribution:
        return self._head(self._loo_suffstat(Xc_pt, R_pts, n, B, rows), None, B, rows, n_trgt=n)

    def _decode_pointwise(self, R_t, X1_pt, B, T):
        from . import x6

        if x6.decoder_side_usable(self, T):
            return x6.decoder_side(self, R_t, X1_pt, T)
        ch = Chain(B, T, X1_pt.device, wg_per_task=True)
        ch.input_pt(R_t, self.r_dim)
        return self.decoder.finish_rows(ch, x1_pt=X1_pt)

    def _encode_points(self, X, Y):
        if self._fused_context_side(X.shape[1]):
            from . import x6

            return x6.context_side(self, X, Y)
        X_pt = self._xenc_pt(X)
        return X_pt, self._xyenc_pt(X_pt, Y, with_tr=False)

    def predict(self, X_cntxt, Y_cntxt, X_trgt, n_cntxt=None, n_trgt=None, n_z_samples=None, probs=(0.025, 0.5, 0.975)) -> Prediction:
        probs = FN.check_probs(probs)
        return self.condition(X_cntxt, Y_cntxt, n_cntxt=n_cntxt, n_z_samples=n_z_samples).query(X_trgt, n_trgt=n_trgt).summary(probs)

    def _refuse_unimplemented(self, what):
        from . import chain as _chain

        if getattr(self, "is_self_attn", False):
            raise NotImplementedError(f"{what} is not implemented for self-attention context encoders (is_self_attn=True)")
        if _chain.COMPUTE_DTYPE != "fp32":
            raise NotImplementedError(f"{what} is not implemented in the bf16 compute mode (set_compute_dtype('bf16'))")

    def _check_counts(self, n, X, what):
        self._refuse_unimplemented(what)
        n = FN.counts_i32(n, X.shape[0], what)
        if n.device != X.device:
            raise ValueError(f"{what} lives on {n.device}, the batch on {X.device}")
        return n

    def _validate_inputs(self, X_cntxt, Y_cntxt, X_trgt, Y_trgt):
        self._check_tensors(X_cntxt, Y_cntxt, X_trgt, Y_trgt)
        if self.training and self.validate_inputs:
            m = X_trgt.abs().amax() if X_trgt.numel() else X_trgt.new_zeros(())
            if X_cntxt.numel():
                m = torch.maximum(m, X_cntxt.abs().amax())
            if self.validate_inputs == "deferred":
                if getattr(self, "_range_seen", None) is None or self._range_seen.device != m.device:
                    self._range_seen = torch.zeros((), device=m.device)
                self._range_seen.copy_(torch.maximum(self._range_seen, m))
                return
            if not (m.item() <= 1.0):
                lo = min(X_cntxt.min().item() if X_cntxt.numel() else 0.0, X_trgt.min().item())
                hi = max(X_cntxt.max().item() if X_cntxt.numel() else 0.0, X_trgt.max().item())
                raise ValueError(f"Features during training should be in [-1,1]. Got [{lo}, {hi}].")

    @staticmethod
    def _check_tensors(*tensors):
        for t in tensors:
            if t is not None and (not t.is_cuda or t.dtype != torch.float32):
                raise RuntimeError("the HIP path takes fp32 device tensors only; there is no CPU fallback")

    def check_deferred_inputs(self):
        seen = getattr(self, "_range_seen", None)
        if seen is None:
            return
        worst = seen.item()
        seen.zero_()
        if not (worst <= 1.0):
            raise ValueError(f"Features during training should be in [-1,1]. Got max |x| = {worst}.")

    _attentive = False

    def _fused_target_side(self, C, T) -> bool:
        return False

    def _xenc_with_query_projection(self, C, T) -> bool:
        from . import x6

        att = getattr(self, "attender", None)
        if not (self._attentive and isinstance(att, MultiheadAttender) and C > 0):
            return False
        return FN.mha_usable(att.kq_head_size, att.value_head_size, C) and x6.xenc_proj_usable(self, att.query_transform, T)

    def _fused_context_side(self, C) -> bool:
        from . import x6

        return hasattr(self, "xy_encoder") and hasattr(self, "_pool_pt") and x6.context_side_usable(self, C)

    def _xenc_pt(self, X, with_tr=False) -> PTensor:
        B, P, dx = X.shape
        ch = Chain(B, P, X.device)
        ch.input_rows(X.contiguous(), dx)
        return self.x_encoder.append_to(ch).run_pt(as_weights=with_tr)

    def _xyenc_pt(self, X_enc: PTensor, Y, with_tr: Optional[bool] = None) -> PTensor:
        ch = Chain(X_enc.n_tasks, X_enc.pts, Y.device)
        ch.input_rows(Y.contiguous(), self.y_dim)
        return self.xy_encoder.run_pt(ch, X_enc.t, X_enc.n_tasks, X_enc.pts,
                                      with_tr=self._attentive if with_tr is None else with_tr)

    def _head(self, suff, Y_trgt, B, T, n_trgt=None):
        return HeadDistribution(suff, self.y_dim, not self.is_heteroskedastic, suff.shape[0] // B, B, T, n_trgt=n_trgt)

    def _decode_taskvec(self, Xt_pt, vec, B, T, n_rows):
        ch = Chain(n_rows, T, Xt_pt.t.device)
        ch.input_pt(Xt_pt.t, self.x_transf_dim, modulus=(B if n_rows != B else 0))
        return self.decoder.finish_rows(ch, taskvec=vec)

    @abc.abstractmethod
    def encode_globally(self, X_cntxt, Y_cntxt):
        pass

    @abc.abstractmethod
    def trgt_dependent_representation(self, X_cntxt, z_samples, R, X_trgt):
        pass

    def latent_path(self, X_cntxt, R, X_trgt, Y_trgt):
        raise NotImplementedError(
            f"`latent_path` not implemented. Cannot use encoded_path={self.encoded_path} in such case.")

    def decode(self, X_trgt, R_trgt):
        n_z, B, T, _ = R_trgt.shape
        suff = self.decoder(X_trgt, R_trgt).reshape(n_z * B, T, 2 * self.y_dim)
        return self._head(suff, None, B, T)

    def set_extrapolation(self, min_max):
        pass


class LatentNeuralProcessFamily(NeuralProcessFamily):

    _valid_paths = ["latent", "both"]

    def __init__(self, *args, is_q_zCct=False, n_z_samples_train=32, n_z_samples_test=32, LatentEncoder=None,
                 LatentDistribution=MultivariateNormalDiag, q_z_loc_transformer=None, q_z_scale_transformer=None,
                 z_dim=None, **kwargs):
        super().__init__(*args, **kwargs)
        self.is_q_zCct = is_q_zCct
        self.n_z_samples_train, self.n_z_samples_test = n_z_samples_train, n_z_samples_test
        self.z_dim = self.r_dim if z_dim is None else z_dim
        if LatentEncoder is None:
            LatentEncoder = self.dflt_Modules["LatentEncoder"]
        self.latent_encoder = LatentEncoder(self.r_dim, self.z_dim * 2)
        if self.encoded_path == "both":
            self.r_z_merger = nn.Linear(self.r_dim + self.z_dim, self.r_dim)
        self.LatentDistribution = LatentDistribution
        self.q_z_loc_transformer = nn.Identity() if q_z_loc_transformer is None else q_z_loc_transformer
        self.q_z_scale_transformer = _q_z_scale if q_z_scale_transformer is None else q_z_scale_transformer
        if self.z_dim != self.r_dim and self.encoded_path == "latent":
            self.reshaper_z = nn.Linear(self.z_dim, self.r_dim)

    @property
    def dflt_Modules(self):
        d = NeuralProcessFamily.dflt_Modules.__get__(self)
        d["LatentEncoder"] = partial(MLP, n_hidden_layers=1, hidden_size=self.r_dim)
        return d

    def forward(self, *args, **kwargs):
        self.n_z_samples = self._n_z_for()
        return super().forward(*args, **kwargs)

    def _n_z_for(self, n_z_samples=None) -> int:
        if n_z_samples is not None:
            if int(n_z_samples) < 1:
                raise ValueError(f"n_z_samples must be at least 1, got {n_z_samples}")
            return int(n_z_samples)
        try:
            return self.n_z_samples_train.rvs() if self.training else self.n_z_samples_test.rvs()
        except AttributeError:
            return self.n_z_samples_train if self.training else self.n_z_samples_test

    def infer_latent_dist(self, X, R):
        R_lat_inp = self.rep_to_lat_input(R)
        return self._latent_dist_from(R_lat_inp)

    def _latent_dist_from(self, R_lat_inp):
        suff = self.latent_encoder(R_lat_inp)
        q_z_loc, q_z_scale = suff.split(self.z_dim, dim=-1)
        return self.LatentDistribution(self.q_z_loc_transformer(q_z_loc), self.q_z_scale_transformer(q_z_scale))

    def rep_to_lat_input(self, R):
        return R

    def latent_path(self, X_cntxt, R, X_trgt, Y_trgt):
        q_zCc = self.infer_latent_dist(X_cntxt, R)
        if self.is_q_zCct and Y_trgt is not None:
            R_from_trgt = self.encode_globally(X_trgt, Y_trgt)
            q_zCct = self.infer_latent_dist(X_trgt, R_from_trgt)
            sampling_dist = q_zCct
        else:
            q_zCct, sampling_dist = None, q_zCc
        return sampling_dist.rsample([self.n_z_samples]), q_zCc, q_zCct

    def _infer_q_zCc(self, R, B, n_valid=None):
        return self._latent_dist_from(self._lat_input(R, B, n_valid=n_valid))

    def _latent_path_pt(self, R, C, Xt_pt, Y_trgt, B, T, n_valid=None, n_trgt=None):
        q_zCc = self._infer_q_zCc(R, B, n_valid)
        if self.is_q_zCct and Y_trgt is not None:
            if Xt_pt is None:
                if self._fused_context_side(T):
                    from . import x6

# ... 309 lines not shown
```

npf_gwwaveform_amd/x6.py:

```python
from __future__ import annotations

import ctypes as C
import math
import os
from typing import List, Optional, Sequence

import torch

from . import _lib as L
from . import chain as CH
from . import functional as FN

ENABLED = os.environ.get("NPF_NO_X6_FUSED", "0") != "1"
WIDTH = 256
VARIANT = int(os.environ.get("NPF_X6_VARIANT", "0"))
B16_ENABLED = os.environ.get("NPF_NO_B16_FUSED", "0") != "1"
B16_VARIANT = int(os.environ.get("NPF_B16_VARIANT", "0"))


class Program:

    def __init__(self, n_tasks: int, tiles: int, per_task: bool, width: int = WIDTH, pts: Optional[int] = None,
                 bf16: bool = False):
        self.n_tasks, self.tiles, self.per_task, self.width = n_tasks, tiles, per_task, width
# ... 18 lines not shown
    def _pt_ok(self, t, what, p16=False):
        want = (self.n_tasks, self.tiles, self.width // 8, 32, 8) if p16 else (self.n_tasks, self.tiles, self.width // 4, 32, 4)
        dt = torch.bfloat16 if p16 else torch.float32
        if t is not None and (tuple(t.shape) != want or t.dtype != dt):
            raise ValueError(f"x6 program operand {what}: {'PT16' if p16 else 'PT32'} tensor {tuple(t.shape)} {t.dtype}, "
                             f"expected {want} {dt}")

    def launch(self) -> None:
        if len(self.ops) > L.NPF_X6_MAX_OPS:
            raise RuntimeError(f"x6 program longer than NPF_X6_MAX_OPS={L.NPF_X6_MAX_OPS}")
        arr = (L.NpfX6Op * len(self.ops))()
        F, pts = self.width, self.n_tasks * self.tiles * 32
        flops = 0
        nbytes = 0
        for j, o in enumerate(self.ops):
            flags = 0
            for k in ("in_pt", "pre_add", "mask", "sbwd_p", "store_in", "addend", "store_out"):
                t = o.get(k)
                if t is not None and o.get(k + "_rm"):
                    if k not in ("in_pt", "addend") or tuple(t.shape) != (self.n_tasks, self.pts, F) or t.dtype != torch.float32:
                        raise ValueError(f"x6 program operand {k}: row-major tensor {tuple(t.shape)} {t.dtype}")
                    if self.bf16:
                        raise ValueError("b16 programs take no row-major operands")
                    flags |= L.X6_IN_RM if k == "in_pt" else L.X6_ADD_RM
                else:
                    p16 = self.bf16 and (k == "sbwd_p" or (k in ("store_in", "store_out") and not o.get(k + "_f32")))
                    if self.bf16 and k in ("store_in", "store_out") and o.get(k + "_f32") and t is not None:
                        flags |= L.X6_STORE_IN_F32 if k == "store_in" else L.X6_STORE_OUT_F32
                    if self.bf16 and k == "mask" and t is not None:
                        raise ValueError("b16 programs take ReLU masks as bits")
                    self._pt_ok(t, k, p16)
                setattr(arr[j], k, self._ptr(t, k))
                nbytes += pts * F * (t.element_size() if t is not None else 0)
            arr[j].reserved[0] = flags
            for k in ("mask_bits", "store_in_bits", "store_bits"):
                t = o.get(k)
                if t is not None and (tuple(t.shape) != (self.n_tasks, self.tiles, 2, 64) or t.dtype != torch.int64):
                    raise ValueError(f"x6 program operand {k}: bits tensor {tuple(t.shape)} {t.dtype}")
                setattr(arr[j], k, self._ptr(t, k))
                nbytes += pts * F // 8 if t is not None else 0
            if o.get("in_rows") is not None:
                rows, w, b = o["in_rows"], o["in_w"], o.get("in_b")
                n = w.shape[1]
                if tuple(rows.shape) != (self.n_tasks, self.tiles * 32, 4) or w.shape[0] != 4 or n % 16 or n > F:
                    raise ValueError(f"x6 rows prologue: rows {tuple(rows.shape)}, matrix {tuple(w.shape)}")
                if b is not None and tuple(b.shape) != (n,):
                    raise ValueError("x6 rows prologue: bias shape")
                arr[j].in_rows, arr[j].in_w, arr[j].in_b = L.ptr(rows), L.ptr(w), L.ptr(b)
                arr[j].in_n, arr[j].in_relu = n, int(bool(o.get("in_relu", False)))
                flops += 2 * 4 * n * pts
                nbytes += pts * 16
            img = o.get("img")
            if img is not None:
                per_task = bool(o.get("img_per_task", False))
                terms = (1,) if self.bf16 else (3,)
                want = ((self.n_tasks,) if per_task else ()) + (() if self.bf16 else (3,)) + (F, F)
                if tuple(img.shape) != want or img.dtype != torch.bfloat16 or not img.is_contiguous():
                    raise ValueError(f"x6 program weight image {tuple(img.shape)} {img.dtype}, expected {want} bfloat16")
                arr[j].w_img = img.data_ptr()
                arr[j].w_task_stride = terms[0] * F * F * 2 if per_task else 0
                bias = o.get("bias")
                if bias is not None:
                    bpt = bool(o.get("bias_per_task", False))
                    if tuple(bias.shape) != ((self.n_tasks, F) if bpt else (F,)):
                        raise ValueError(f"x6 program bias {tuple(bias.shape)}")
                    arr[j].bias = L.ptr(bias)
                    arr[j].bias_task_stride = F if bpt else 0
                arr[j].relu = int(bool(o.get("relu", False)))
                arr[j].softmax_n = int(o.get("softmax_n", 0))
                arr[j].softmax_scale = float(o.get("softmax_scale", 1.0))
                flops += 2 * o.get("true_k", F) * o.get("true_n", F) * pts
                nbytes += terms[0] * 2 * F * F * (self.n_tasks if per_task else 1)
            elif any(o.get(k) is not None for k in ("bias", "addend", "store_out", "store_bits")) or o.get("relu") or o.get("softmax_n"):
                raise ValueError("x6 program: an op without a multiply has no output side")
            arr[j].sbwd_scale = float(o.get("sbwd_scale", 1.0))
        tail = self.tail
        if tail is not None:
            flops += 2 * 4 * F * pts
            nbytes += pts * 16
        if CH.PROFILE is not None:
            ev0, ev1 = torch.cuda.Event(enable_timing=True), torch.cuda.Event(enable_timing=True)
            ev0.record()
        tw, tb, tr = (L.ptr(tail[0]) if tail else None, L.ptr(tail[1]) if (tail and tail[1] is not None) else None,
                      L.ptr(tail[2]) if tail else None)
        if self.bf16:
            if self.pts != self.tiles * 32:
                raise ValueError("b16 programs run on whole tiles")
            L.check(L.load().npf_b16_run(arr, len(self.ops), tw, tb, tr, self.n_tasks, self.tiles, int(self.per_task), F,
                                         B16_VARIANT, L.stream_ptr()), "npf_b16_run")
        else:
            L.check(L.load().npf_x6_run_ex(arr, len(self.ops), tw, tb, tr, self.n_tasks, self.tiles, self.pts, int(self.per_task), F,
                                           VARIANT if F in (256, 512) else 0, L.stream_ptr()), "npf_x6_run_ex")
        if CH.PROFILE is not None:
            ev1.record()
            CH.PROFILE.append(("b16_program_kernel" if self.bf16 else "x6_program_kernel", flops, ev0, ev1, nbytes, self.tag))
        if CH.TRACE is not None:
            CH.TRACE.append(("prog", self))


def task_images(pt: torch.Tensor, pts: int, row: bool = True, tr: bool = True, width: int = WIDTH, bf16: bool = False):
    n_tasks = pt.shape[0]
    if tuple(pt.shape) != (n_tasks, CH.tiles_of(pts), width // 4, 32, 4) or pts > width:
        raise ValueError(f"task_images: PT32 tensor {tuple(pt.shape)} for {pts} points x {width} features")
    shape = (n_tasks, width, width) if bf16 else (n_tasks, 3, width, width)
    mk = lambda: torch.empty(shape, dtype=torch.bfloat16, device=pt.device)
    ri, ti = (mk() if row else None), (mk() if tr else None)
    if CH.PROFILE is not None:
        ev0, ev1 = torch.cuda.Event(enable_timing=True), torch.cuda.Event(enable_timing=True)
        ev0.record()
    fn = L.load().npf_b16_task_images if bf16 else L.load().npf_x6_task_images
    L.check(fn(L.ptr(pt.detach().contiguous()), n_tasks, pts, width, ri.data_ptr() if row else None,
               ti.data_ptr() if tr else None, L.stream_ptr()), "npf_x6_task_images")
    if CH.PROFILE is not None:
        ev1.record()
        CH.PROFILE.append(("x6_task_images_kernel", 0, ev0, ev1,
                           pt.numel() * 4 + (int(row) + int(tr)) * n_tasks * (1 if bf16 else 3) * width * width * 2))
    return ri, ti


def _weight_images(Ws: Sequence[torch.Tensor], kinds: Sequence[int], width: int = WIDTH, bf16: bool = False) -> List[List[torch.Tensor]]:
    if bf16:
        n = len(Ws)
        buf = torch.empty((len(kinds), n, width, width), dtype=torch.bfloat16, device=Ws[0].device)
        CH.prepare_weights([(Ws[i].detach(), kind) for kind in kinds for i in range(n)],
                           dsts=[buf[k, i] for k in range(len(kinds)) for i in range(n)])
        return [[buf[k, i] for i in range(n)] for k in range(len(kinds))]
    from .mlp_x6 import _three_term_images

    return _three_term_images(Ws, kinds, width)


def _r16(t: Optional[torch.Tensor]) -> Optional[torch.Tensor]:
    return None if t is None else t.to(torch.bfloat16).to(torch.float32)


def _bits(n_tasks, tiles, dev):
    return torch.empty((n_tasks, tiles, 2, 64), dtype=torch.int64, device=dev)


_ZEROS = {}


def _zeros(shape, device) -> torch.Tensor:
    key = (tuple(shape), str(device))
    z = _ZEROS.get(key)
    if z is None:
        z = torch.zeros(shape, dtype=torch.float32, device=device)
        if not (z.is_cuda and torch.cuda.is_current_stream_capturing()):
            _ZEROS[key] = z
    return z


def _pad_rows4(X: torch.Tensor) -> torch.Tensor:
    d = X.shape[-1]
    if d == 4:
        return X.contiguous()
    return torch.cat((X, _zeros((*X.shape[:-1], 4 - d), X.device)), dim=-1)


def _first_layer_matrix(W: torch.Tensor, n_out: int) -> torch.Tensor:
    n, d = W.shape
    Wt = W.detach().t()
    if n < n_out:
        Wt = torch.cat((Wt, _zeros((d, n_out - n), W.device)), dim=1)
    if d < 4:
        Wt = torch.cat((Wt, _zeros((4 - d, n_out), W.device)), dim=0)
    return Wt.contiguous()


def decode_rows_usable(mod, x1: torch.Tensor, x2: torch.Tensor) -> bool:
    from .architectures import MLP

    if not (ENABLED and CH.COMPUTE_DTYPE == "fp32" and mod.is_sum_merge and isinstance(mod.flat_module, MLP)):
        return False
    F = x1.shape[-1]
    fm, rs = mod.flat_module, mod.resizer
    if F not in (128, 256, 512) or x2.shape[-1] != F or x1.shape[:-1] != x2.shape[:-1] or fm.is_res or rs.is_res:
        return False
    if any(m.dropout_p > 0 and m.training for m in (fm, rs)):
        return False
    if not (_square(rs.layers(), F) and _square([fm.to_hidden, *fm.linears], F) and fm.out.in_features == F
            and fm.out.out_features <= 4):
        return False
    return len(rs.layers()) + len(fm.linears) + 1 <= L.NPF_X6_MAX_OPS and x1.shape[-2] > 0


def decode_rows(mod, x1: torch.Tensor, x2: torch.Tensor) -> torch.Tensor:
    n, T, F = x1.shape
    fm, rs = mod.flat_module, mod.resizer
    lins = [*rs.layers(), fm.to_hidden, *fm.linears]
    imgs = _weight_images([l.weight for l in lins], (1,), F)[0]
    tiles = CH.tiles_of(T)
    prog = Program(n, tiles, per_task=False, width=F, pts=T)
    n_res = len(rs.layers())
    for i, lin in enumerate(lins):
        o = dict(img=imgs[i], bias=lin.bias.detach() if lin.bias is not None else None, relu=True)
        if i == 0:
            o.update(in_pt=x2.detach().contiguous(), in_pt_rm=True)
        if i == n_res - 1:
            o.update(addend=x1.detach().contiguous(), addend_rm=True)
        prog.op(**o)
    rows = torch.empty((n, tiles * 32, 4), dtype=torch.float32, device=x1.device)
    Wo, bo = _pad_out(fm.out.weight, fm.out.bias)
    prog.tail = (Wo, bo, rows)
    prog.tag = f"decode (merge + {F}-wide decoder + output layer) from row-major inputs"
    prog.launch()
    return rows[:, :T, :fm.out.out_features]


def _pad_out(W: torch.Tensor, b: Optional[torch.Tensor]):
    n = W.shape[0]
    if n == 4:
        return W.detach().contiguous(), (b.detach().contiguous() if b is not None else None)
    Wp = torch.zeros((4, W.shape[1]), dtype=torch.float32, device=W.device)
    Wp[:n] = W.detach()
    bp = None
    if b is not None:
        bp = torch.zeros((4,), dtype=torch.float32, device=W.device)
        bp[:n] = b.detach()
    return Wp, bp


class _TargetSideFn(torch.autograd.Function):

    @staticmethod
    def forward(ctx, X, K_pt, V_pt, C, scale, spec, zb, *params):
        n_x, n_mrz, n_res, n_flat = spec
        B, T, dx = X.shape
        dev = X.device
        tiles = T // 32
        Ws, bs = list(params[0::2]), list(params[1::2])
        W1, b1 = Ws[0], bs[0]
        W_out, b_out = Ws[-1], bs[-1]
        n_out = W_out.shape[0]
        mid_W, mid_b = Ws[1:-1], bs[1:-1]
        F = mid_W[0].shape[0]
        if n_mrz:
            mid_b[n_x] = zb
        train = any(ctx.needs_input_grad)
        bf16 = CH.COMPUTE_DTYPE == "bf16"
        imgs = _weight_images(mid_W, (1, 2) if train else (1,), F, bf16)
        fw = imgs[0]
        K_row, K_tr = task_images(K_pt, C, row=True, tr=train, width=F, bf16=bf16)
        V_row, V_tr = task_images(V_pt, C, row=train, tr=True, width=F, bf16=bf16)
        X4 = _pad_rows4(X.detach())
        W1p = _first_layer_matrix(W1, F)
        if bf16:
            X4, W1p = _r16(X4), _r16(W1p)
        pt = lambda: CH.pt_empty(B, T, F, dev)
        pb = (lambda: CH.pt16_empty(B, T, F, dev)) if bf16 else pt
        prog = Program(B, tiles, per_task=True, width=F, bf16=bf16)
        saved_acts, saved_bits = [], []
        h1 = pb() if train else None
        bits_h1 = _bits(B, tiles, dev) if train else None
        Xt_enc = pt()
        for i in range(n_x):
            last = i == n_x - 1
            o = dict(img=fw[i], w_ref=("shared", mid_W[i]), bias=mid_b[i].detach() if mid_b[i] is not None else None, relu=not last)
            if i == 0:
                o.update(in_rows=X4, in_w=W1p, in_b=b1.detach() if b1 is not None else None, in_relu=True, store_in=h1,
                         store_in_bits=bits_h1)
            if last:
                o["store_out"], o["store_out_f32"] = Xt_enc, True
            elif train:
                o["store_out"], o["store_bits"] = pb(), _bits(B, tiles, dev)
                saved_acts.append(o["store_out"])
                saved_bits.append(o["store_bits"])
            prog.op(**o)
        P = pb() if train else None
        prog.op(img=K_row, w_ref=("task_row", K_pt, C), img_per_task=True, softmax_n=C, softmax_scale=scale, store_out=P, true_n=C)
        R_trgt = pb() if train else None
        prog.op(img=V_tr, w_ref=("task_tr", V_pt, C), img_per_task=True, store_out=R_trgt, true_k=C)
        for i in range(n_mrz + n_res + n_flat):
            j = n_x + i
            o = dict(img=fw[j], w_ref=("shared", mid_W[j]), bias=mid_b[j].detach().contiguous() if mid_b[j] is not None else None,
                     relu=True, bias_per_task=bool(n_mrz and i == 0))
            if i == n_mrz + n_res - 1:
                o["addend"] = Xt_enc
            if train:
                o["store_out"], o["store_bits"] = pb(), _bits(B, tiles, dev)
                saved_acts.append(o["store_out"])
                saved_bits.append(o["store_bits"])
            prog.op(**o)
        rows = torch.empty((B, T, 4), dtype=torch.float32, device=dev)
        Wo, bo = _pad_out(W_out, b_out)
        if bf16:
            Wo = _r16(Wo)
        prog.tail = (Wo, bo, rows)
        prog.tag = "target side forward (x-encoder, attention, decoder, output layer)"
        prog.launch()
        ctx.geom = (B, T, tiles, dx, C, float(scale), n_out, F)
        ctx.spec, ctx.bf16 = spec, bf16
        ctx.trace_ref = ([W.detach() for W in mid_W], K_pt, V_pt) if CH.TRACE is not None else None
        ctx.has_b = [b is not None for b in bs]
        ctx.set_materialize_grads(False)
        if train:
            ctx.n_acts, ctx.n_bits = len(saved_acts), len(saved_bits)
            ctx.save_for_backward(X4, h1, bits_h1, Xt_enc, P, R_trgt, *saved_acts, *saved_bits, *imgs[1], V_row, K_tr, Wo)
        return rows[..., :n_out] if n_out != 4 else rows

    @staticmethod
    def backward(ctx, g):
        n_x, n_mrz, n_res, n_flat = ctx.spec
        n_dec = n_mrz + n_res + n_flat
        n_mid = n_x + n_dec
        n_par = 2 * (n_mid + 2)
        if g is None:
            return (None,) * (7 + n_par)
        B, T, tiles, dx, C, scale, n_out, F = ctx.geom
        sv = list(ctx.saved_tensors)
        X4, h1, bits_h1, Xt_enc, P, R_trgt = sv[:6]
        acts = sv[6:6 + ctx.n_acts]
        bits = sv[6 + ctx.n_acts:6 + ctx.n_acts + ctx.n_bits]
        rest = sv[6 + ctx.n_acts + ctx.n_bits:]
        bw, (V_row, K_tr, Wo) = rest[:n_mid], rest[n_mid:]
        dev = g.device
        bf16 = ctx.bf16
        g4 = g.contiguous() if n_out == 4 else torch.nn.functional.pad(g, (0, 4 - n_out)).contiguous()
        if bf16:
            g4 = _r16(g4)
        pt = lambda: CH.pt_empty(B, T, F, dev)
        pb = (lambda: CH.pt16_empty(B, T, F, dev)) if bf16 else pt
        x_acts, x_bits = acts[:n_x - 1], bits[:n_x - 1]
        d_acts, d_bits = acts[n_x - 1:], bits[n_x - 1:]
        prog = Program(B, tiles, per_task=True, width=F, bf16=bf16)
        tr = ctx.trace_ref
        wref = lambda j: ("shared", tr[0][j].t()) if tr is not None else None
        dz = [None] * n_mid
        for i in range(n_dec - 1, -1, -1):
            j = n_x + i
            is_merge = i == n_mrz + n_res - 1 or (n_mrz and i == 0)
            dz[j] = pt() if is_merge else pb()
            o = dict(mask_bits=d_bits[i], store_in=dz[j], store_in_f32=is_merge, img=bw[j], w_ref=wref(j))
            if i == n_dec - 1:
                o.update(in_rows=g4, in_w=Wo)
            prog.op(**o)
        dO, dS = pb(), pb()
        prog.op(store_in=dO, img=V_row, w_ref=("task_row", tr[2], C) if tr is not None else None, img_per_task=True, true_n=C)
        prog.op(sbwd_p=P, sbwd_scale=scale, store_in=dS, img=K_tr, w_ref=("task_tr", tr[1], C) if tr is not None else None,
                img_per_task=True, addend=dz[n_x + n_mrz + n_res - 1], true_k=C)
        for i in range(n_x - 1, -1, -1):
            dz[i] = pb()
            o = dict(store_in=dz[i], img=bw[i], w_ref=wref(i))
            if i < n_x - 1:
                o["mask_bits"] = x_bits[i]
            prog.op(**o)
        dz1 = pb()
        prog.op(mask_bits=bits_h1, store_in=dz1)
        prog.tag = "target side dgrad (decoder, attention backward, x-encoder)"
        prog.launch()
        jobs, grads = [], []
        dW1p = torch.empty((F, 4), dtype=torch.float32, device=dev)
        db1 = torch.empty((F,), dtype=torch.float32, device=dev) if ctx.has_b[0] else None
        jobs.append(dict(dZ=dz1, A=FN._pack(X4), N=F, K=4, dW=dW1p, db=db1))
        grads += [None, db1]
        ins = [h1, *x_acts, R_trgt, *d_acts[:-1]]
        for j in range(n_mid):
            dW = torch.empty((F, F), dtype=torch.float32, device=dev)
            db = torch.empty((F,), dtype=torch.float32, device=dev) if (ctx.has_b[1 + j] and not (n_mrz and j == n_x)) else None
            jobs.append(dict(dZ=dz[j], A=ins[j], N=F, K=F, dW=dW, db=db))
            grads += [dW, db]
        dz_out = torch.zeros(CH.pt_shape(B, T, 4), dtype=torch.float32, device=dev)
        dz_out[:, :, 0] = g4.view(B, tiles, 32, 4)
        dWo = torch.empty((n_out, F), dtype=torch.float32, device=dev)
        dbo = torch.empty((n_out,), dtype=torch.float32, device=dev) if ctx.has_b[-1] else None
        jobs.append(dict(dZ=dz_out, A=d_acts[-1], N=n_out, K=F, dW=dWo, db=dbo))
        grads += [dWo, dbo]
        mk = torch.zeros if C % 32 else torch.empty
        dK = mk(CH.pt_shape(B, C, F), dtype=torch.float32, device=dev) if ctx.needs_input_grad[1] else None
        dV = mk(CH.pt_shape(B, C, F), dtype=torch.float32, device=dev) if ctx.needs_input_grad[2] else None
        if dV is not None:
            jobs.append(dict(dZ=P, A=dO, N=C, K=F, dW=dV, per_task=True, ldz=F))
        if dK is not None:
            jobs.append(dict(dZ=dS, A=Xt_enc, N=C, K=F, dW=dK, per_task=True, ldz=F))
        CH.run_wgrad(jobs, B, T, dev, tag="target side weight / key / value gradients")
        if CH.TRACE is not None:
            CH.TRACE.append(("wgrad", jobs, B, T, bf16))
        grads[0] = dW1p[:, :dx].contiguous() if dx != 4 else dW1p
        d_zb = FN.sum_points_pt(dz[n_x], T, F)[:, :F].contiguous() if (n_mrz and ctx.needs_input_grad[6]) else None
        return (None, dK, dV, None, None, None, d_zb, *grads)


class _DecoderSideFn(torch.autograd.Function):

    @staticmethod
    def forward(ctx, R_pt, X1_pt, T, spec, zb, *params):
        n_mrz, n_res, n_flat = spec
        B, tiles = R_pt.shape[0], R_pt.shape[1]
        dev = R_pt.device
        Ws, bs = list(params[0::2]), list(params[1::2])
        W_out, b_out = Ws[-1], bs[-1]
        n_out = W_out.shape[0]
        mid_W, mid_b = Ws[:-1], bs[:-1]
        F = mid_W[0].shape[0]
        n_mid = n_mrz + n_res + n_flat
        if n_mrz:
            mid_b[0] = zb
        train = any(ctx.needs_input_grad)
        imgs = _weight_images(mid_W, (1, 2) if train else (1,), F)
        fw = imgs[0]
        R_pt, X1_pt = R_pt.contiguous(), X1_pt.contiguous()
        pt = lambda: CH.pt_empty(B, tiles * 32, F, dev)
        prog = Program(B, tiles, per_task=bool(n_mrz), width=F)
        acts, bits = [], []
        for i in range(n_mid):
            o = dict(img=fw[i], w_ref=("shared", mid_W[i]), bias=mid_b[i].detach().contiguous() if mid_b[i] is not None else None,
                     relu=True, bias_per_task=bool(n_mrz and i == 0))
            if i == 0:
                o["in_pt"] = R_pt.detach()
            if i == n_mrz + n_res - 1:
                o["addend"] = X1_pt.detach()
            if train:
                o["store_out"], o["store_bits"] = pt(), _bits(B, tiles, dev)
                acts.append(o["store_out"])
                bits.append(o["store_bits"])
            prog.op(**o)
        rows = torch.empty((B, tiles * 32, 4), dtype=torch.float32, device=dev)
        Wo, bo = _pad_out(W_out, b_out)
        prog.tail = (Wo, bo, rows)
        prog.tag = "decoder forward (resizer, merge, flat MLP, output layer)"
        prog.launch()
        ctx.geom = (B, T, tiles, n_out, F)
        ctx.spec = spec
        ctx.has_b = [b is not None for b in bs]
        ctx.set_materialize_grads(False)
        ctx.trace_ref = [W.detach() for W in mid_W] if CH.TRACE is not None else None
        if train:
            ctx.save_for_backward(R_pt.detach(), *acts, *bits, *imgs[1], Wo)
        return rows[:, :T, :n_out]

    @staticmethod
    def backward(ctx, g):
        n_mrz, n_res, n_flat = ctx.spec
        n_mid = n_mrz + n_res + n_flat
        if g is None:
            return (None,) * (5 + 2 * (n_mid + 1))
        B, T, tiles, n_out, F = ctx.geom
        sv = list(ctx.saved_tensors)
        R_pt, acts, bits, bw, Wo = sv[0], sv[1:1 + n_mid], sv[1 + n_mid:1 + 2 * n_mid], sv[1 + 2 * n_mid:1 + 3 * n_mid], sv[-1]
        dev = g.device
        if T == tiles * 32 and n_out == 4:
            g4 = g.contiguous()
        else:
            g4 = torch.zeros((B, tiles * 32, 4), dtype=torch.float32, device=dev)
            g4[:, :T, :n_out] = g
        pt = lambda: CH.pt_empty(B, tiles * 32, F, dev)
        tr = ctx.trace_ref
        prog = Program(B, tiles, per_task=bool(n_mrz), width=F)
        dz = [None] * n_mid
        dR = pt() if ctx.needs_input_grad[0] else None
        for i in range(n_mid - 1, -1, -1):
            dz[i] = pt()
            o = dict(mask_bits=bits[i], store_in=dz[i], img=bw[i], w_ref=("shared", tr[i].t()) if tr is not None else None)
            if i == n_mid - 1:
                o.update(in_rows=g4, in_w=Wo)
            if i == 0 and dR is not None:
                o["store_out"] = dR
            prog.op(**o)
        prog.tag = "decoder dgrad"
        prog.launch()
        jobs, grads = [], []
        ins = [R_pt, *acts[:-1]]
        for j in range(n_mid):
            dW = torch.empty((F, F), dtype=torch.float32, device=dev)
            db = torch.empty((F,), dtype=torch.float32, device=dev) if (ctx.has_b[j] and not (n_mrz and j == 0)) else None
            jobs.append(dict(dZ=dz[j], A=ins[j], N=F, K=F, dW=dW, db=db))
            grads += [dW, db]
        dz_out = torch.zeros(CH.pt_shape(B, tiles * 32, 4), dtype=torch.float32, device=dev)
        dz_out[:, :, 0] = g4.view(B, tiles, 32, 4)
        dWo = torch.empty((n_out, F), dtype=torch.float32, device=dev)
        dbo = torch.empty((n_out,), dtype=torch.float32, device=dev) if ctx.has_b[-1] else None
        jobs.append(dict(dZ=dz_out, A=acts[-1], N=n_out, K=F, dW=dWo, db=dbo))
        grads += [dWo, dbo]
        CH.run_wgrad(jobs, B, tiles * 32, dev, tag="decoder weight gradients")
        if CH.TRACE is not None:
            CH.TRACE.append(("wgrad", jobs, B, tiles * 32, False))
        dX1 = dz[n_mrz + n_res - 1] if ctx.needs_input_grad[1] else None
        d_zb = FN.sum_points_pt(dz[0], tiles * 32, F)[:, :F].contiguous() if (n_mrz and ctx.needs_input_grad[4]) else None
        return (dR, dX1, None, None, d_zb, *grads)


def decoder_side_usable(model, T: int) -> bool:
    from .architectures import MLP, MergeFlatInputs

    if not (ENABLED and CH.COMPUTE_DTYPE == "fp32") or T <= 0:
        return False
    dec = getattr(model, "decoder", None)
    F = getattr(model, "r_dim", 0)
    if F != 128 or getattr(model, "x_transf_dim", F) != F or not isinstance(dec, MergeFlatInputs):
        return False
    if not (dec.is_sum_merge and isinstance(dec.flat_module, MLP)):
        return False
    fm, rs = dec.flat_module, dec.resizer
    for m in (fm, rs):
        if m.is_res or (m.dropout_p > 0 and m.training):
            return False
    if not (_square(rs.layers(), F) and _square([fm.to_hidden, *fm.linears], F) and fm.out.in_features == F
            and fm.out.out_features <= 4):
        return False
    return len(rs.layers()) + len(fm.linears) + 2 <= L.NPF_X6_MAX_OPS


def decoder_side(model, R_pt: torch.Tensor, X1_pt: torch.Tensor, T: int, zb: Optional[torch.Tensor] = None) -> torch.Tensor:
    dec = model.decoder
    fm, rs = dec.flat_module, dec.resizer
    lins = [*rs.layers(), fm.to_hidden, *fm.linears, fm.out]
    params = []
    for lin in lins:
        params += [lin.weight, lin.bias]
    if zb is not None:
        params[0:0] = [model.r_z_merger.weight[:, :model.r_dim], None]
    return _DecoderSideFn.apply(R_pt, X1_pt, T, (int(zb is not None), len(rs.layers()), len(fm.linears) + 1), zb, *params)


class _PairLinearFn(torch.autograd.Function):

    @staticmethod
    def forward(ctx, a_pt, b_pt, pts, Wa, Wb):
        B, tiles = a_pt.shape[0], a_pt.shape[1]
        F = Wa.shape[0]
        dev = a_pt.device
        train = any(ctx.needs_input_grad)
        imgs = _weight_images([Wa, Wb], (1, 2) if train else (1,), F)
        a_pt, b_pt = a_pt.contiguous(), b_pt.contiguous()
        oa, ob = CH.pt_empty(B, tiles * 32, F, dev), CH.pt_empty(B, tiles * 32, F, dev)
        prog = Program(B, tiles, per_task=False, width=F)
        prog.op(in_pt=a_pt.detach(), img=imgs[0][0], w_ref=("shared", Wa), store_out=oa)
        prog.op(in_pt=b_pt.detach(), img=imgs[0][1], w_ref=("shared", Wb), store_out=ob)
        prog.tag = "key / value projections"
        prog.launch()
        ctx.geom = (B, tiles, F, pts)
        ctx.set_materialize_grads(False)
        if train:
            ctx.save_for_backward(a_pt.detach(), b_pt.detach(), *imgs[1])
        return oa, ob

    @staticmethod
    def backward(ctx, ga, gb):
        if ga is None and gb is None:
            return (None,) * 5
        B, tiles, F, pts = ctx.geom
        a_pt, b_pt, ia, ib = ctx.saved_tensors
        dev = a_pt.device
        zeros = lambda: torch.zeros(CH.pt_shape(B, tiles * 32, F), dtype=torch.float32, device=dev)
        ga = ga.contiguous() if ga is not None else zeros()
        gb = gb.contiguous() if gb is not None else zeros()
        da, db = CH.pt_empty(B, tiles * 32, F, dev), CH.pt_empty(B, tiles * 32, F, dev)
        prog = Program(B, tiles, per_task=False, width=F)
        prog.op(in_pt=ga, img=ia, store_out=da)
        prog.op(in_pt=gb, img=ib, store_out=db)
        prog.tag = "key / value projections dgrad"
        prog.launch()
        dWa, dWb = (torch.empty((F, F), dtype=torch.float32, device=dev) for _ in range(2))
        CH.run_wgrad([dict(dZ=ga, A=a_pt, N=F, K=F, dW=dWa, db=None), dict(dZ=gb, A=b_pt, N=F, K=F, dW=dWb, db=None)], B, pts, dev,
                     tag="key / value projection weight gradients")
        return da, db, None, dWa, dWb


def pair_linear_usable(lin_a, lin_b) -> bool:
    F = lin_a.in_features
    return (ENABLED and CH.COMPUTE_DTYPE == "fp32" and F in (128, 256) and lin_a.bias is None and lin_b.bias is None
            and _square([lin_a, lin_b], F))


def pair_linear(a_pt: torch.Tensor, b_pt: torch.Tensor, pts: int, lin_a, lin_b):
    return _PairLinearFn.apply(a_pt, b_pt, pts, lin_a.weight, lin_b.weight)


class _XEncProjFn(torch.autograd.Function):

    @staticmethod
    def forward(ctx, X, n_x, *params):
        B, P, dx = X.shape
        dev = X.device
        tiles = P // 32
        Ws, bs = list(params[0::2]), list(params[1::2])
        W1, b1 = Ws[0], bs[0]
        x_W, x_b = Ws[1:1 + n_x], bs[1:1 + n_x]
        Wq, bq = Ws[-1], bs[-1]
        F = Wq.shape[0]
        train = any(ctx.needs_input_grad)
        imgs = _weight_images([*x_W, Wq], (1, 2) if train else (1,), F)
        fw = imgs[0]
        X4 = _pad_rows4(X.detach())
        pt = lambda: CH.pt_empty(B, P, F, dev)
        prog = Program(B, tiles, per_task=False, width=F)
        acts, bits = [], []
        h1 = pt() if train else None
        bits_h1 = _bits(B, tiles, dev) if train else None
        X_enc, Q = pt(), pt()
        for i in range(n_x):
            last = i == n_x - 1
            o = dict(img=fw[i], w_ref=("shared", x_W[i]), bias=x_b[i].detach() if x_b[i] is not None else None, relu=not last)
            if i == 0:
                o.update(in_rows=X4, in_w=_first_layer_matrix(W1, F), in_b=b1.detach() if b1 is not None else None, in_relu=True,
                         store_in=h1, store_in_bits=bits_h1)
            if last:
                o["store_out"] = X_enc
            elif train:
                o["store_out"], o["store_bits"] = pt(), _bits(B, tiles, dev)
                acts.append(o["store_out"])
                bits.append(o["store_bits"])
            prog.op(**o)
        prog.op(img=fw[n_x], w_ref=("shared", Wq), bias=bq.detach() if bq is not None else None, store_out=Q)
        prog.tag = "x-encoder + query projection"
        prog.launch()
        ctx.geom = (B, P, tiles, dx, F)
        ctx.n_x = n_x
        ctx.has_b = [b is not None for b in bs]
        ctx.set_materialize_grads(False)
        if train:
            ctx.save_for_backward(X4, h1, bits_h1, X_enc, *acts, *bits, *imgs[1])
        return X_enc, Q

    @staticmethod
    def backward(ctx, gX, gQ):
        n_x = ctx.n_x
        n_par = 2 * (n_x + 2)
        if gX is None and gQ is None:
            return (None,) * (2 + n_par)
        B, P, tiles, dx, F = ctx.geom
        sv = list(ctx.saved_tensors)
        X4, h1, bits_h1, X_enc = sv[:4]
        acts, bits, bw = sv[4:4 + n_x - 1], sv[4 + n_x - 1:4 + 2 * (n_x - 1)], sv[4 + 2 * (n_x - 1):]
        dev = X4.device
        pt = lambda: CH.pt_empty(B, P, F, dev)
        prog = Program(B, tiles, per_task=False, width=F)
        jobs, grads = [], [None] * n_par

        def wjob(pos, dZ, A, N, K):
            dW = torch.empty((N, K), dtype=torch.float32, device=dev)
            db = torch.empty((N,), dtype=torch.float32, device=dev) if ctx.has_b[pos] else None
            jobs.append(dict(dZ=dZ, A=A, N=N, K=K, dW=dW, db=db))
            grads[2 * pos], grads[2 * pos + 1] = dW, db
            return dW

        if gQ is not None:
            gQ = gQ.contiguous()
            prog.op(in_pt=gQ, img=bw[n_x])
            wjob(n_x + 1, gQ, X_enc, F, F)
            first = dict(pre_add=gX.contiguous()) if gX is not None else {}
        else:
            first = dict(in_pt=gX.contiguous())
        x_in = [h1, *acts]
        for i in range(n_x - 1, -1, -1):
            dz = pt()
            o = dict(store_in=dz, img=bw[i])
            if i == n_x - 1:
                o.update(first)
            else:
                o["mask_bits"] = bits[i]
            prog.op(**o)
            wjob(1 + i, dz, x_in[i], F, F)
        dz1 = pt()
        prog.op(mask_bits=bits_h1, store_in=dz1)
        dW1p = wjob(0, dz1, FN._pack(X4), F, 4)
        prog.tag = "x-encoder + query projection dgrad"
        prog.launch()
        CH.run_wgrad(jobs, B, P, dev, tag="x-encoder + query projection weight gradients")
        if dx != 4:
            grads[0] = dW1p[:, :dx].contiguous()
        return (None, None, *grads)


def xenc_proj_usable(model, lin_q, T: int) -> bool:
    from .architectures import MLP

    if not (ENABLED and CH.COMPUTE_DTYPE == "fp32") or T <= 0:
        return False
    F = _width_of(model)
    xe = model.x_encoder
    if not F or not (isinstance(xe, MLP) and xe.input_size <= 4 and xe.hidden_size == F and xe.output_size == F
                     and not xe.is_res and not (xe.dropout_p > 0 and xe.training)):
        return False
    return lin_q.in_features == F and lin_q.out_features == F and len(xe.linears) + 3 <= L.NPF_X6_MAX_OPS


def xenc_proj(model, X: torch.Tensor, lin_q):
    xe = model.x_encoder
    lins = [xe.to_hidden, *xe.linears, xe.out, lin_q]
    params = []
    for lin in lins:
        params += [lin.weight, lin.bias]
    T = X.shape[1]
    if T % 32:
        X = torch.nn.functional.pad(X, (0, 0, 0, CH.pad32(T) - T))
    Xe, Q = _XEncProjFn.apply(X, len(xe.linears) + 1, *params)
    return CH.PTensor(Xe, T, model.r_dim), Q


class _MlpPtFn(torch.autograd.Function):

    @staticmethod
    def forward(ctx, x_pt, pts, *params):
        B, tiles = x_pt.shape[0], x_pt.shape[1]
        dev = x_pt.device
        Ws, bs = list(params[0::2]), list(params[1::2])
        n, F = len(Ws), Ws[0].shape[0]
        train = any(ctx.needs_input_grad)
        imgs = _weight_images(Ws, (1, 2) if train else (1,), F)
        x_pt = x_pt.contiguous()
        pt = lambda: CH.pt_empty(B, tiles * 32, F, dev)
        prog = Program(B, tiles, per_task=False, width=F)
        acts, bits = [], []
        y = pt()
        for i in range(n):
            last = i == n - 1
            o = dict(img=imgs[0][i], w_ref=("shared", Ws[i]), bias=bs[i].detach() if bs[i] is not None else None, relu=not last)
            if i == 0:
                o["in_pt"] = x_pt.detach()
            if last:
                o["store_out"] = y
            elif train:
                o["store_out"], o["store_bits"] = pt(), _bits(B, tiles, dev)
                acts.append(o["store_out"])
                bits.append(o["store_bits"])
            prog.op(**o)
        prog.tag = "MLP block forward"
        prog.launch()
        ctx.geom = (B, tiles, F, pts, n)
        ctx.has_b = [b is not None for b in bs]
        ctx.set_materialize_grads(False)
        if train:
            ctx.save_for_backward(x_pt.detach(), *acts, *bits, *imgs[1])
        return y

    @staticmethod
    def backward(ctx, g):
        B, tiles, F, pts, n = ctx.geom
        if g is None:
            return (None,) * (2 + 2 * n)
        sv = list(ctx.saved_tensors)
        x_pt, acts, bits, bw = sv[0], sv[1:n], sv[n:2 * n - 1], sv[2 * n - 1:]
        dev = g.device
        g = g.contiguous()
        pt = lambda: CH.pt_empty(B, tiles * 32, F, dev)
        prog = Program(B, tiles, per_task=False, width=F)
        dz = [None] * n
        dx = pt()
        for i in range(n - 1, -1, -1):
            o = dict(img=bw[i])
            if i == n - 1:
                o["in_pt"], dz[i] = g, g
            else:
                dz[i] = pt()
                o.update(mask_bits=bits[i], store_in=dz[i])
            if i == 0:
                o["store_out"] = dx
            prog.op(**o)
        prog.tag = "MLP block dgrad"
        prog.launch()
        ins = [x_pt, *acts]
        jobs, grads = [], []
        for i in range(n):
            dW = torch.empty((F, F), dtype=torch.float32, device=dev)
            db = torch.empty((F,), dtype=torch.float32, device=dev) if ctx.has_b[i] else None
            jobs.append(dict(dZ=dz[i], A=ins[i], N=F, K=F, dW=dW, db=db))
            grads += [dW, db]
        CH.run_wgrad(jobs, B, pts, dev, tag="MLP block weight gradients")
        return (dx, None, *grads)


def mlp_pt_usable(mlp) -> bool:
    from .architectures import MLP

    if not (ENABLED and CH.COMPUTE_DTYPE == "fp32" and isinstance(mlp, MLP)):
        return False
    F = mlp.input_size
    if F not in (128, 256) or mlp.is_res or (mlp.dropout_p > 0 and mlp.training):
        return False
    return _square(mlp.layers(), F) and len(mlp.layers()) <= L.NPF_X6_MAX_OPS


def mlp_pt(mlp, x_pt: torch.Tensor, pts: int) -> torch.Tensor:
    params = []
    for lin in mlp.layers():
        params += [lin.weight, lin.bias]
    return _MlpPtFn.apply(x_pt, pts, *params)


def _width_of(model) -> int:
    F = getattr(model, "r_dim", 0)
    return F if (F in (128, 256) and getattr(model, "x_transf_dim", F) == F) else 0


def _mode_ok() -> bool:
    return ENABLED and (CH.COMPUTE_DTYPE == "fp32" or (CH.COMPUTE_DTYPE == "bf16" and B16_ENABLED))


def _square(lins, width=WIDTH) -> bool:
    return all(l.in_features == width and l.out_features == width for l in lins)


def target_side_usable(model, C: int, T: int, latent_merge: bool = False) -> bool:
    from .architectures import MLP, DotAttender

    if not _mode_ok():
        return False
    WIDTH = _width_of(model)
    if not WIDTH:
        return False
    xe, dec, att = model.x_encoder, model.decoder, getattr(model, "attender", None)
    if not isinstance(att, DotAttender) or att.kq_size != WIDTH or att.value_size != WIDTH:
        return False
    if not ((WIDTH // 2 < C or (WIDTH == 128 and C >= 1)) and C <= WIDTH and T > 0):
        return False
    if not (isinstance(xe, MLP) and xe.input_size <= 4 and xe.hidden_size == WIDTH and xe.output_size == WIDTH
            and not xe.is_res and not (xe.dropout_p > 0 and xe.training)):
        return False
    if not (dec.is_sum_merge and isinstance(dec.flat_module, MLP)):
        return False
    fm, rs = dec.flat_module, dec.resizer
    for m in (fm, rs):
        if m.is_res or (m.dropout_p > 0 and m.training):
            return False
    if not (_square(rs.layers(), WIDTH) and _square([fm.to_hidden, *fm.linears], WIDTH) and fm.out.in_features == WIDTH
            and fm.out.out_features <= 4):
        return False
    n_mrz = int(latent_merge)
    if n_mrz:
        mz = getattr(model, "r_z_merger", None)
        if mz is None or mz.out_features != WIDTH or mz.in_features <= WIDTH or model.r_dim != WIDTH:
            return False
    n_x, n_res, n_flat = len(xe.linears) + 1, len(rs.layers()), len(fm.linears) + 1
    return n_x + 2 + n_mrz + n_res + n_flat + 1 <= L.NPF_X6_MAX_OPS


def target_side(model, X_trgt: torch.Tensor, K: CH.PTensor, V: CH.PTensor, zb: Optional[torch.Tensor] = None) -> torch.Tensor:
    xe, dec, att = model.x_encoder, model.decoder, model.attender
    fm, rs = dec.flat_module, dec.resizer
    lins = [xe.to_hidden, *xe.linears, xe.out, *rs.layers(), fm.to_hidden, *fm.linears, fm.out]
    params = []
    for lin in lins:
        params += [lin.weight, lin.bias]
    n_x = len(xe.linears) + 1
    if zb is not None:
        params[2 * (n_x + 1):2 * (n_x + 1)] = [model.r_z_merger.weight[:, :model.r_dim], None]
    spec = (n_x, int(zb is not None), len(rs.layers()), len(fm.linears) + 1)
    scale = 1.0 / math.sqrt(att.kq_size) if att.is_scale else 1.0
    T = X_trgt.shape[1]
    Tp = CH.pad32(T)
    if Tp != T:
        X_trgt = torch.nn.functional.pad(X_trgt, (0, 0, 0, Tp - T))
    rows = _TargetSideFn.apply(X_trgt, K.t, V.t, K.pts, scale, spec, zb, *params)
    return rows if Tp == T else rows[:, :T].contiguous()


class _ContextSideFn(torch.autograd.Function):

    @staticmethod
    def forward(ctx, X, Y, spec, *params):
        n_x, n_flat = spec
        B, Cn, dx = X.shape
        dy = Y.shape[-1]
        dev = X.device
        tiles = Cn // 32
        Ws, bs = list(params[0::2]), list(params[1::2])
        W1, b1 = Ws[0], bs[0]
        x_W, x_b = Ws[1:1 + n_x], bs[1:1 + n_x]
        Wr1, br1, Wr2, br2 = Ws[1 + n_x], bs[1 + n_x], Ws[2 + n_x], bs[2 + n_x]
        f_W, f_b = Ws[3 + n_x:], bs[3 + n_x:]
        h = Wr1.shape[0]
        F = Wr2.shape[0]
        train = any(ctx.needs_input_grad)
        bf16 = CH.COMPUTE_DTYPE == "bf16"
        Wr2p = torch.zeros((F, F), dtype=torch.float32, device=dev)
        Wr2p[:, :h] = Wr2.detach()
        imgs = _weight_images([*x_W, Wr2p, *f_W], (1, 2) if train else (1,), F, bf16)
        fw = imgs[0]
        X4, Y4 = _pad_rows4(X.detach()), _pad_rows4(Y.detach())
        W1p, Wr1p = _first_layer_matrix(W1, F), _first_layer_matrix(Wr1, h)
        if bf16:
            X4, Y4, W1p, Wr1p = _r16(X4), _r16(Y4), _r16(W1p), _r16(Wr1p)
        pt = lambda: CH.pt_empty(B, Cn, F, dev)
        pb = (lambda: CH.pt16_empty(B, Cn, F, dev)) if bf16 else pt
        prog = Program(B, tiles, per_task=False, width=F, bf16=bf16)
        acts, bits = [], []
        h1 = pb() if train else None
        bits_h1 = _bits(B, tiles, dev) if train else None
        Xc_enc = pt()
        for i in range(n_x):
            last = i == n_x - 1
            o = dict(img=fw[i], w_ref=("shared", x_W[i]), bias=x_b[i].detach() if x_b[i] is not None else None, relu=not last)
            if i == 0:
                o.update(in_rows=X4, in_w=W1p, in_b=b1.detach() if b1 is not None else None,
                         in_relu=True, store_in=h1, store_in_bits=bits_h1)
            if last:
                o["store_out"], o["store_out_f32"] = Xc_enc, True
            elif train:
                o["store_out"], o["store_bits"] = pb(), _bits(B, tiles, dev)
                acts.append(o["store_out"])
                bits.append(o["store_bits"])
            prog.op(**o)
        hy = pb() if train else None
        bits_hy = _bits(B, tiles, dev) if train else None
        o = dict(in_rows=Y4, in_w=Wr1p, in_b=br1.detach() if br1 is not None else None, in_relu=True,
                 store_in=hy, store_in_bits=bits_hy, img=fw[n_x], w_ref=("shared", Wr2p),
                 bias=br2.detach() if br2 is not None else None, relu=True, addend=Xc_enc, true_k=h)
        if train:
            o["store_out"], o["store_bits"] = pb(), _bits(B, tiles, dev)
            acts.append(o["store_out"])
            bits.append(o["store_bits"])
        prog.op(**o)
        R = pt()
        for i in range(n_flat):
            last = i == n_flat - 1
            o = dict(img=fw[n_x + 1 + i], w_ref=("shared", f_W[i]), bias=f_b[i].detach() if f_b[i] is not None else None,
                     relu=not last)
            if last:
                o["store_out"], o["store_out_f32"] = R, True
            elif train:
                o["store_out"], o["store_bits"] = pb(), _bits(B, tiles, dev)
                acts.append(o["store_out"])
                bits.append(o["store_bits"])
            prog.op(**o)
        prog.tag = "context side forward (x-encoder, XY-encoder)"
        prog.launch()
        ctx.geom = (B, Cn, tiles, dx, dy, h, F)
        ctx.spec, ctx.bf16 = spec, bf16
        ctx.trace_ref = [W.detach() for W in (*x_W, Wr2p, *f_W)] if CH.TRACE is not None else None
        ctx.has_b = [b is not None for b in bs]
        ctx.set_materialize_grads(False)
        if train:
            ctx.n_acts = len(acts)
            ctx.save_for_backward(X4, Y4, h1, bits_h1, hy, bits_hy, *acts, *bits, *imgs[1])
        return Xc_enc, R

    @staticmethod
    def backward(ctx, gK, gR):
        n_x, n_flat = ctx.spec
        n_par = 2 * (1 + n_x + 2 + n_flat)
        if gK is None and gR is None:
            return (None,) * (3 + n_par)
        B, Cn, tiles, dx, dy, h, F = ctx.geom
        sv = list(ctx.saved_tensors)
        X4, Y4, h1, bits_h1, hy, bits_hy = sv[:6]
        acts, bits = sv[6:6 + ctx.n_acts], sv[6 + ctx.n_acts:6 + 2 * ctx.n_acts]
        bw = sv[6 + 2 * ctx.n_acts:]
        dev = X4.device
        bf16 = ctx.bf16
        pt = lambda: CH.pt_empty(B, Cn, F, dev)
        pb = (lambda: CH.pt16_empty(B, Cn, F, dev)) if bf16 else pt
        x_acts, x_bits = acts[:n_x - 1], bits[:n_x - 1]
        m_act, m_bits = acts[n_x - 1], bits[n_x - 1]
        f_acts, f_bits = acts[n_x:], bits[n_x:]
        prog = Program(B, tiles, per_task=False, width=F, bf16=bf16)
        wref = lambda j: ("shared", ctx.trace_ref[j].t()) if ctx.trace_ref is not None else None
        jobs, grads = [], [None] * n_par

        def wjob(pos, dZ, A, N, K, **kw):
            dW = torch.empty((N, K), dtype=torch.float32, device=dev)
            db = torch.empty((N,), dtype=torch.float32, device=dev) if ctx.has_b[pos] else None
            jobs.append(dict(dZ=dZ, A=A, N=N, K=K, dW=dW, db=db, **kw))
            grads[2 * pos], grads[2 * pos + 1] = dW, db
            return dW

        dz_m = None
        if gR is not None:
            gR = gR.contiguous()
            f_in = [m_act, *f_acts]
            for i in range(n_flat - 1, -1, -1):
                o = dict(img=bw[n_x + 1 + i], w_ref=wref(n_x + 1 + i))
                if i == n_flat - 1:
                    o["in_pt"] = gR
                    dz = gR
                    if bf16:
                        dz = pb()
                        o["store_in"] = dz
                else:
                    dz = pb()
                    o.update(mask_bits=f_bits[i], store_in=dz)
                prog.op(**o)
                wjob(1 + n_x + 2 + i, dz, f_in[i], F, F)
            dz_m, dz_hy = pt(), pb()
            prog.op(mask_bits=m_bits, store_in=dz_m, store_in_f32=True, img=bw[n_x], w_ref=wref(n_x))
            prog.op(mask_bits=bits_hy, store_in=dz_hy)
            wjob(1 + n_x + 1, dz_m, hy, F, h, lda=F)
            dWr1 = wjob(1 + n_x, dz_hy, FN._pack(Y4), h, 4, ldz=F)
        if gK is not None or dz_m is not None:
            first = dict(in_pt=gK.contiguous(), pre_add=dz_m) if gK is not None else dict(in_pt=dz_m)
            x_in = [h1, *x_acts]
            for i in range(n_x - 1, -1, -1):
                dz = pb()
                o = dict(store_in=dz, img=bw[i], w_ref=wref(i))
                if i == n_x - 1:
                    o.update(first)
                else:
                    o["mask_bits"] = x_bits[i]
                prog.op(**o)
                wjob(1 + i, dz, x_in[i], F, F)
            dz1 = pb()
            prog.op(mask_bits=bits_h1, store_in=dz1)
            dW1p = wjob(0, dz1, FN._pack(X4), F, 4)
        prog.tag = "context side dgrad (XY-encoder, x-encoder)"
        prog.launch()
        CH.run_wgrad(jobs, B, Cn, dev, tag="context side weight gradients")
        if CH.TRACE is not None:
            CH.TRACE.append(("wgrad", jobs, B, Cn, bf16))
        if gR is not None and dy != 4:
            grads[2 * (1 + n_x)] = dWr1[:, :dy].contiguous()
        if (gK is not None or dz_m is not None) and dx != 4:
            grads[0] = dW1p[:, :dx].contiguous()
        return (None, None, None, *grads)


def context_side_usable(model, C: int) -> bool:
    from .architectures import MLP, MergeFlatInputs

    if not _mode_ok() or C <= 0:
        return False
    WIDTH = _width_of(model)
    if not WIDTH:
        return False
    xe, xy = model.x_encoder, getattr(model, "xy_encoder", None)
    if not (isinstance(xe, MLP) and xe.input_size <= 4 and xe.hidden_size == WIDTH and xe.output_size == WIDTH
            and not xe.is_res and not (xe.dropout_p > 0 and xe.training)):
        return False
    if not (isinstance(xy, MergeFlatInputs) and xy.is_sum_merge and isinstance(xy.flat_module, MLP)):
        return False
    fm, rs = xy.flat_module, xy.resizer
    for m in (fm, rs):
        if m.is_res or (m.dropout_p > 0 and m.training):
            return False
    if not (_square([fm.to_hidden, *fm.linears, fm.out], WIDTH) and len(rs.linears) == 0 and rs.input_size <= 4
            and rs.output_size == WIDTH and rs.hidden_size % 16 == 0 and rs.hidden_size <= WIDTH):
        return False
    n_x, n_flat = len(xe.linears) + 1, len(fm.linears) + 2
    return n_flat + 2 + n_x + 1 <= L.NPF_X6_MAX_OPS


def context_side(model, X_cntxt: torch.Tensor, Y_cntxt: torch.Tensor):
    xe, xy = model.x_encoder, model.xy_encoder
    fm, rs = xy.flat_module, xy.resizer
    lins = [xe.to_hidden, *xe.linears, xe.out, rs.to_hidden, rs.out, fm.to_hidden, *fm.linears, fm.out]
    params = []
    for lin in lins:
        params += [lin.weight, lin.bias]
    Cn = X_cntxt.shape[1]
    if Cn % 32:
        pad = CH.pad32(Cn) - Cn
        X_cntxt = torch.nn.functional.pad(X_cntxt, (0, 0, 0, pad))
        Y_cntxt = torch.nn.functional.pad(Y_cntxt, (0, 0, 0, pad))
    Xc, R = _ContextSideFn.apply(X_cntxt, Y_cntxt, (len(xe.linears) + 1, len(fm.linears) + 2), *params)
    return CH.PTensor(Xc, Cn, model.r_dim), CH.PTensor(R, Cn, model.r_dim)
```

Before: 43.46 million target-points/s.

## Fuse narrow-input padding/packing, share wgrad reduce across wide and narrow jobs

Adds a single kernel that zero-pads the narrow 1-4 wide input rows to 4 and also writes the point-tiled packed layout, replacing several torch cat/pad/zeros/slice-assign ops and a later separate pack in backward. Weight-gradient jobs split into wide (x6) and narrow groups now run as two main kernels plus one combined reduce instead of two full launch pairs. Deferred input range validation becomes one fused abs-max kernel with an atomicMax rather than several torch reductions. This trims many small launches and memory passes on the train step, at the cost of extra code paths and of holding the packed inputs in ctx until backward.

```diff
diff --git a/include/npf_hip.h b/include/npf_hip.h
--- a/include/npf_hip.h
+++ b/include/npf_hip.h
@@ -108,6 +108,10 @@
                   float *partials, int64_t partials_bytes, void *stream);
 int64_t npf_wgrad_partials_bytes(const npf_wgrad_job_t *jobs, int32_t n_jobs, int32_t n_tasks,
                                  int32_t tiles_per_task);
+int npf_wgrad_run_pair(const npf_wgrad_job_t *jobs_a, int32_t n_a, const npf_wgrad_job_t *jobs_b, int32_t n_b,
+                       int32_t n_tasks, int32_t tiles_per_task, float *partials, int64_t partials_bytes, void *stream);
+int64_t npf_wgrad_pair_partials_bytes(const npf_wgrad_job_t *jobs_a, int32_t n_a, const npf_wgrad_job_t *jobs_b,
+                                      int32_t n_b, int32_t n_tasks, int32_t tiles_per_task);
 
 int npf_gauss_head_fwd(const float *suff, int32_t n_rows, int32_t pts, int32_t dy, int32_t homoskedastic,
                        const float *Y, int32_t n_y_rows, float *loc, float *scale, float *sum_logp,
@@ -145,6 +149,9 @@
                 void *stream);
 int npf_unpack_pt(const float *pt, int32_t n_tasks, int32_t pts_per_task, int32_t F_valid, float *rows,
                   void *stream);
+int npf_pad_pack_rows(const float *rows, int32_t n_tasks, int32_t pts_per_task, int32_t d, int32_t pts_padded,
+                      float *rows4, float *pt, void *stream);
+int npf_range_fold(const float *a, int64_t n_a, const float *b, int64_t n_b, float *seen, void *stream);
 int npf_transpose(const float *src, int32_t rows, int32_t cols, float *dst, void *stream);
 int npf_split_heads(const float *src, int32_t n_tasks, int32_t pts_per_task, int32_t F, int32_t n_heads, float *dst,
                     void *stream);
diff --git a/npf_gwwaveform_amd/_lib.py b/npf_gwwaveform_amd/_lib.py
--- a/npf_gwwaveform_amd/_lib.py
+++ b/npf_gwwaveform_amd/_lib.py
@@ -95,6 +95,10 @@
     "npf_chain_run": (C.c_int, [C.POINTER(NpfProgram), _p]),
     "npf_wgrad_run": (C.c_int, [C.POINTER(NpfWgradJob), _i32, _i32, _i32, _p, _i64, _p]),
     "npf_wgrad_partials_bytes": (_i64, [C.POINTER(NpfWgradJob), _i32, _i32, _i32]),
+    "npf_wgrad_run_pair": (C.c_int, [C.POINTER(NpfWgradJob), _i32, C.POINTER(NpfWgradJob), _i32, _i32, _i32, _p, _i64, _p]),
+    "npf_wgrad_pair_partials_bytes": (_i64, [C.POINTER(NpfWgradJob), _i32, C.POINTER(NpfWgradJob), _i32, _i32, _i32]),
+    "npf_pad_pack_rows": (C.c_int, [_p, _i32, _i32, _i32, _i32, _p, _p, _p]),
+    "npf_range_fold": (C.c_int, [_p, _i64, _p, _i64, _p, _p]),
     "npf_gauss_head_fwd": (C.c_int, [_p, _i32, _i32, _i32, _i32, _p, _i32, _p, _p, _p, _p]),
     "npf_gauss_head_bwd": (C.c_int, [_p, _p, _p, _i32, _i32, _i32, _i32, _p, _i32, _p, _p, _p, _p, _p]),
     "npf_mc_objective_fwd": (C.c_int, [_p, _i32, _i32, _i32, _p, _i32, _p, _p]),
diff --git a/npf_gwwaveform_amd/chain.py b/npf_gwwaveform_amd/chain.py
--- a/npf_gwwaveform_amd/chain.py
+++ b/npf_gwwaveform_amd/chain.py
@@ -384,6 +384,10 @@
         narrow = [jb for jb in jobs if min(jb["N"], jb["K"]) <= 32]
         wide = [jb for jb in jobs if min(jb["N"], jb["K"]) > 32]
         if narrow and wide:
+            shared = sum(not jb.get("per_task") for jb in jobs)
+            if max(len(wide), len(narrow)) <= L.NPF_MAX_WGRAD_JOBS and shared <= L.NPF_MAX_WGRAD_JOBS:
+                _launch_wgrad_pair(wide, narrow, n_tasks, pts, device)
+                return
             _launch_wgrad(wide, n_tasks, pts, device, True)
             _launch_wgrad(narrow, n_tasks, pts, device, False)
             return
@@ -391,26 +395,42 @@
     _launch_wgrad(jobs, n_tasks, pts, device, x6)
 
 
+def _wgrad_job_array(chunk: Sequence[dict], x6: bool):
+    arr = (L.NpfWgradJob * len(chunk))()
+    for j, jb in enumerate(chunk):
+        z16, a16 = jb["dZ"].dtype == torch.bfloat16, jb["A"].dtype == torch.bfloat16
+        if (z16 or a16) and COMPUTE_DTYPE != "bf16":
+            raise RuntimeError("PT16 operands exist in the bf16 compute mode only")
+        arr[j].dZ = (jb["dZ"].data_ptr() if z16 else L.ptr(jb["dZ"])) + jb.get("dZ_off", 0) * jb["dZ"].element_size()
+        arr[j].A = (jb["A"].data_ptr() if a16 else L.ptr(jb["A"])) + jb.get("A_off", 0) * jb["A"].element_size()
+        arr[j].dW = L.ptr(jb["dW"]) + 4 * jb.get("dW_off", 0)
+        arr[j].db = (L.ptr(jb["db"]) + 4 * jb.get("db_off", 0)) if jb.get("db") is not None else None
+        arr[j].ldz, arr[j].lda, arr[j].ldo = jb.get("ldz", 0), jb.get("lda", 0), jb.get("ldo", 0)
+        arr[j].ldw = jb.get("ldw") or jb["K"]
+        arr[j].N, arr[j].K = jb["N"], jb["K"]
+        arr[j].per_task = int(jb.get("per_task", False))
+        arr[j].accumulate = (int(jb.get("accumulate", False)) | (2 if COMPUTE_DTYPE == "bf16" else 0)
+                             | (4 if z16 else 0) | (8 if a16 else 0)
+                             | (L.WGRAD_F32X6 if x6 else 0) | (L.WGRAD_NO_H16 if (x6 and not WGRAD_H16) else 0))
+    return arr
+
+
+def _launch_wgrad_pair(wide: Sequence[dict], narrow: Sequence[dict], n_tasks: int, pts: int, device) -> None:
+    lib = L.load()
+    a, b = _wgrad_job_array(wide, True), _wgrad_job_array(narrow, False)
+    nbytes = lib.npf_wgrad_pair_partials_bytes(a, len(wide), b, len(narrow), n_tasks, tiles_of(pts))
+    if nbytes < 0:
+        raise RuntimeError("npf_wgrad_pair_partials_bytes: invalid wgrad jobs")
+    ws = torch.empty((nbytes + 3) // 4, dtype=torch.float32, device=device)
+    L.check(lib.npf_wgrad_run_pair(a, len(wide), b, len(narrow), n_tasks, tiles_of(pts), L.ptr(ws), nbytes, L.stream_ptr()),
+            "npf_wgrad_run_pair")
+
+
 def _launch_wgrad(jobs: Sequence[dict], n_tasks: int, pts: int, device, x6: bool) -> None:
     lib = L.load()
     for i0 in range(0, len(jobs), L.NPF_MAX_WGRAD_JOBS):
         chunk = jobs[i0:i0 + L.NPF_MAX_WGRAD_JOBS]
-        arr = (L.NpfWgradJob * len(chunk))()
-        for j, jb in enumerate(chunk):
-            z16, a16 = jb["dZ"].dtype == torch.bfloat16, jb["A"].dtype == torch.bfloat16
-            if (z16 or a16) and COMPUTE_DTYPE != "bf16":
-                raise RuntimeError("PT16 operands exist in the bf16 compute mode only")
-            arr[j].dZ = (jb["dZ"].data_ptr() if z16 else L.ptr(jb["dZ"])) + jb.get("dZ_off", 0) * jb["dZ"].element_size()
-            arr[j].A = (jb["A"].data_ptr() if a16 else L.ptr(jb["A"])) + jb.get("A_off", 0) * jb["A"].element_size()
-            arr[j].dW = L.ptr(jb["dW"]) + 4 * jb.get("dW_off", 0)
-            arr[j].db = (L.ptr(jb["db"]) + 4 * jb.get("db_off", 0)) if jb.get("db") is not None else None
-            arr[j].ldz, arr[j].lda, arr[j].ldo = jb.get("ldz", 0), jb.get("lda", 0), jb.get("ldo", 0)
-            arr[j].ldw = jb.get("ldw") or jb["K"]
-            arr[j].N, arr[j].K = jb["N"], jb["K"]
-            arr[j].per_task = int(jb.get("per_task", False))
-            arr[j].accumulate = (int(jb.get("accumulate", False)) | (2 if COMPUTE_DTYPE == "bf16" else 0)
-                                 | (4 if z16 else 0) | (8 if a16 else 0)
-                                 | (L.WGRAD_F32X6 if x6 else 0) | (L.WGRAD_NO_H16 if (x6 and not WGRAD_H16) else 0))
+        arr = _wgrad_job_array(chunk, x6)
         nbytes = lib.npf_wgrad_partials_bytes(arr, len(chunk), n_tasks, tiles_of(pts))
         if nbytes < 0:
             raise RuntimeError("npf_wgrad_partials_bytes: invalid wgrad jobs")
diff --git a/npf_gwwaveform_amd/csrc/layout_kernels.hip b/npf_gwwaveform_amd/csrc/layout_kernels.hip
--- a/npf_gwwaveform_amd/csrc/layout_kernels.hip
+++ b/npf_gwwaveform_amd/csrc/layout_kernels.hip
@@ -79,6 +79,57 @@
       if (h < n_heads) v = *(const f32x4*)(src + (((((size_t)h * n_tasks + b) * tiles + tile) * hq + qh) * 32 + p) * 4);
       *(f32x4*)(dst + idx * 4) = v;
     }
+  }
+}
+
+__global__ void range_fold_kernel(const float* __restrict__ a, size_t na, const float* __restrict__ b, size_t nb,
+                                  unsigned* __restrict__ seen) {
+  __shared__ unsigned wave_max[4];
+  unsigned m = 0u;
+  const size_t total = na + nb;
+  for (size_t idx = blockIdx.x * (size_t)blockDim.x + threadIdx.x; idx < total; idx += (size_t)gridDim.x * blockDim.x) {
+    const float v = idx < na ? a[idx] : b[idx - na];
+    unsigned u = __float_as_uint(v) & 0x7fffffffu;
+    if (u > 0x7f800000u) u = 0x7fc00000u;
+    m = u > m ? u : m;
+  }
+#pragma unroll
+  for (int off = 32; off >= 1; off >>= 1) {
+    const unsigned o = (unsigned)__shfl_xor((int)m, off);
+    m = o > m ? o : m;
+  }
+  if ((threadIdx.x & 63) == 0) wave_max[threadIdx.x >> 6] = m;
+  __syncthreads();
+  if (threadIdx.x == 0) {
+    for (int w = 1; w < 4; ++w) m = wave_max[w] > m ? wave_max[w] : m;
+    if (m) atomicMax(seen, m);
+  }
+}
+
+__global__ void pad_pack_rows_kernel(const float* __restrict__ src, int n_tasks, int pts, int d, int pts_p,
+                                     float* __restrict__ rows4, float* __restrict__ pt) {
+  const int tiles = (pts_p + 31) / 32;
+  const int qn = pt ? 8 : 1;
+  const size_t total = (size_t)n_tasks * tiles * qn * 32;
+  for (size_t idx = blockIdx.x * (size_t)blockDim.x + threadIdx.x; idx < total; idx += (size_t)gridDim.x * blockDim.x) {
+    const int p = idx & 31;
+    const size_t r = idx >> 5;
+    const int q = r % qn;
+    const size_t tt = r / qn;
+    const int tile = tt % tiles;
+    const size_t task = tt / tiles;
+    const int point = tile * 32 + p;
+    f32x4 v = {0.f, 0.f, 0.f, 0.f};
+    if (q == 0) {
+      if (point < pts) {
+        const float* s = src + (task * pts + point) * (size_t)d;
+#pragma unroll
+        for (int j = 0; j < 4; ++j)
+          if (j < d) v[j] = s[j];
+      }
+      if (rows4 && point < pts_p) *(f32x4*)(rows4 + (task * pts_p + point) * (size_t)4) = v;
+    }
+    if (pt) *(f32x4*)(pt + idx * 4) = v;
   }
 }
 
@@ -267,6 +318,29 @@
   return NPF_OK;
 }
 
+extern "C" int npf_range_fold(const float* a, int64_t n_a, const float* b, int64_t n_b, float* seen, void* stream) {
+  if (!seen || n_a < 0 || n_b < 0 || (n_a && !a) || (n_b && !b) || (((uintptr_t)seen) & 3)) return NPF_EINVAL;
+  const size_t total = (size_t)n_a + (size_t)n_b;
+  if (total == 0) return NPF_OK;
+  size_t g = (total + 2047) / 2048;
+  g = g > 256 ? 256 : g;
+  hipLaunchKernelGGL(npf::range_fold_kernel, dim3((unsigned)g), dim3(256), 0, (hipStream_t)stream, a, (size_t)n_a, b, (size_t)n_b,
+                     (unsigned*)seen);
+  NPF_CHECK_LAUNCH();
+  return NPF_OK;
+}
+
+extern "C" int npf_pad_pack_rows(const float* rows, int32_t n_tasks, int32_t pts, int32_t d, int32_t pts_padded, float* rows4,
+                                 float* pt, void* stream) {
+  if (!rows || (!rows4 && !pt) || n_tasks <= 0 || pts <= 0 || d <= 0 || d > 4 || pts_padded < pts) return NPF_EINVAL;
+  if ((((uintptr_t)rows4) | ((uintptr_t)pt)) & 15) return NPF_EINVAL;
+  const size_t total = (size_t)n_tasks * ((pts_padded + 31) / 32) * (pt ? 8 : 1) * 32;
+  hipLaunchKernelGGL(npf::pad_pack_rows_kernel, dim3(npf::grid_for(total, 256)), dim3(256), 0, (hipStream_t)stream, rows,
+                     n_tasks, pts, d, pts_padded, rows4, pt);
+  NPF_CHECK_LAUNCH();
+  return NPF_OK;
+}
+
 extern "C" int npf_transpose(const float* src, int32_t rows, int32_t cols, float* dst, void* stream) {
   if (!src || !dst || rows <= 0 || cols <= 0) return NPF_EINVAL;
   hipLaunchKernelGGL(npf::transpose_kernel, dim3((cols + 31) / 32, (rows + 31) / 32), dim3(256), 0, (hipStream_t)stream,
diff --git a/npf_gwwaveform_amd/csrc/wgrad_kernel.hip b/npf_gwwaveform_amd/csrc/wgrad_kernel.hip
--- a/npf_gwwaveform_amd/csrc/wgrad_kernel.hip
+++ b/npf_gwwaveform_amd/csrc/wgrad_kernel.hip
@@ -923,6 +923,68 @@
   return off * 4 + 16;
 }
 
+namespace npf {
+
+static int64_t shared_floats(const WgradJobs& J) {
+  int64_t off = 0;
+  for (int j = 0; j < J.n_jobs; ++j) {
+    if (J.job[j].per_task) continue;
+    const int Np = round_up(J.job[j].N, 32), Kp = round_up(J.job[j].K, 32);
+    off += (int64_t)(J.first_wg[j + 1] - J.first_wg[j]) * ((int64_t)Np * Kp + Np);
+  }
+  return off;
+}
+
+static int launch_main(const WgradJobs& J, float* partials, void* stream) {
+  const int n_jobs = J.n_jobs;
+  const int n_wg = J.first_wg[n_jobs];
+  bool bf16 = true, x6 = true;
+  for (int j = 0; j < n_jobs; ++j) {
+    bf16 &= (J.job[j].accumulate & NPF_WGRAD_BF16) != 0;
+    x6 &= (J.job[j].accumulate & (NPF_WGRAD_F32X6 | NPF_WGRAD_BF16)) == NPF_WGRAD_F32X6;
+  }
+  bool h16 = x6;
+  for (int j = 0; j < n_jobs; ++j) h16 &= J.job[j].N == 256 && J.job[j].K == 256 && !(J.job[j].accumulate & NPF_WGRAD_NO_H16);
+  if (h16)
+    hipLaunchKernelGGL(wgrad_h16_kernel, dim3(n_wg), dim3(512), 0, (hipStream_t)stream, J, partials);
+  else if (x6)
+    hipLaunchKernelGGL(wgrad_x6_kernel, dim3(n_wg), dim3(kXThreads), 0, (hipStream_t)stream, J, partials);
+  else if (bf16)
+    hipLaunchKernelGGL(wgrad_kernel<true>, dim3(n_wg), dim3(kWgThreads), 0, (hipStream_t)stream, J, partials);
+  else
+    hipLaunchKernelGGL(wgrad_kernel<false>, dim3(n_wg), dim3(kWgThreads), 0, (hipStream_t)stream, J, partials);
+  NPF_CHECK_LAUNCH();
+  return NPF_OK;
+}
+
+static int merge_for_reduce(const WgradJobs& A, const WgradJobs& B, int64_t b_off, WgradJobs* R) {
+  int k = 0, wg = 0;
+  for (int g = 0; g < 2; ++g) {
+    const WgradJobs& J = g ? B : A;
+    for (int j = 0; j < J.n_jobs; ++j) {
+      if (J.job[j].per_task) continue;
+      if (k == kMaxJobs) return NPF_EINVAL;
+      R->job[k] = J.job[j];
+      R->first_wg[k] = wg;
+      R->part_off[k] = J.part_off[j] + (g ? b_off : 0);
+      wg += J.first_wg[j + 1] - J.first_wg[j];
+      ++k;
+    }
+  }
+  for (int j = k; j <= kMaxJobs; ++j) R->first_wg[j] = wg;
+  for (int j = k; j < kMaxJobs; ++j) {
+    R->job[j] = A.job[0];
+    R->part_off[j] = 0;
+  }
+  R->n_jobs = k;
+  R->n_tasks = A.n_tasks;
+  R->tiles_per_task = A.tiles_per_task;
+  R->pad = 0;
+  return NPF_OK;
+}
+
+}
+
 extern "C" int npf_wgrad_run(const npf_wgrad_job_t* jobs, int32_t n_jobs, int32_t n_tasks, int32_t tiles_per_task,
                              float* partials, int64_t partials_bytes, void* stream) {
   npf::WgradJobs J;
@@ -932,23 +994,8 @@
   bool any_shared = false;
   for (int j = 0; j < n_jobs; ++j) any_shared |= !jobs[j].per_task;
   if (any_shared && (!partials || partials_bytes < need || (((uintptr_t)partials) & 15))) return NPF_EINVAL;
-  const int n_wg = J.first_wg[n_jobs];
-  bool bf16 = true, x6 = true;
-  for (int j = 0; j < n_jobs; ++j) {
-    bf16 &= (jobs[j].accumulate & NPF_WGRAD_BF16) != 0;
-    x6 &= (jobs[j].accumulate & (NPF_WGRAD_F32X6 | NPF_WGRAD_BF16)) == NPF_WGRAD_F32X6;
-  }
-  bool h16 = x6;
-  for (int j = 0; j < n_jobs; ++j) h16 &= jobs[j].N == 256 && jobs[j].K == 256 && !(jobs[j].accumulate & NPF_WGRAD_NO_H16);
-  if (h16)
-    hipLaunchKernelGGL(npf::wgrad_h16_kernel, dim3(n_wg), dim3(512), 0, (hipStream_t)stream, J, partials);
-  else if (x6)
-    hipLaunchKernelGGL(npf::wgrad_x6_kernel, dim3(n_wg), dim3(npf::kXThreads), 0, (hipStream_t)stream, J, partials);
-  else if (bf16)
-    hipLaunchKernelGGL(npf::wgrad_kernel<true>, dim3(n_wg), dim3(npf::kWgThreads), 0, (hipStream_t)stream, J, partials);
-  else
-    hipLaunchKernelGGL(npf::wgrad_kernel<false>, dim3(n_wg), dim3(npf::kWgThreads), 0, (hipStream_t)stream, J, partials);
-  NPF_CHECK_LAUNCH();
+  const int lrc = npf::launch_main(J, partials, stream);
+  if (lrc != NPF_OK) return lrc;
   if (any_shared) {
     hipLaunchKernelGGL(npf::wgrad_reduce_kernel, dim3(65, n_jobs), dim3(256), 0, (hipStream_t)stream, J,
                        (const float*)partials);
@@ -956,3 +1003,32 @@
   }
   return NPF_OK;
 }
+
+extern "C" int64_t npf_wgrad_pair_partials_bytes(const npf_wgrad_job_t* jobs_a, int32_t n_a, const npf_wgrad_job_t* jobs_b,
+                                                 int32_t n_b, int32_t n_tasks, int32_t tiles_per_task) {
+  npf::WgradJobs A, B;
+  if (npf::plan(jobs_a, n_a, n_tasks, tiles_per_task, &A) != 0 || npf::plan(jobs_b, n_b, n_tasks, tiles_per_task, &B) != 0) return -1;
+  return (npf::shared_floats(A) + npf::shared_floats(B)) * 4 + 16;
+}
+
+extern "C" int npf_wgrad_run_pair(const npf_wgrad_job_t* jobs_a, int32_t n_a, const npf_wgrad_job_t* jobs_b, int32_t n_b,
+                                  int32_t n_tasks, int32_t tiles_per_task, float* partials, int64_t partials_bytes, void* stream) {
+  npf::WgradJobs A, B, R;
+  int rc = npf::plan(jobs_a, n_a, n_tasks, tiles_per_task, &A);
+  if (rc != 0) return rc;
+  rc = npf::plan(jobs_b, n_b, n_tasks, tiles_per_task, &B);
+  if (rc != 0) return rc;
+  const int64_t fa = npf::shared_floats(A), fb = npf::shared_floats(B);
+  rc = npf::merge_for_reduce(A, B, fa, &R);
+  if (rc != 0) return rc;
+  if (R.n_jobs && (!partials || partials_bytes < (fa + fb) * 4 + 16 || (((uintptr_t)partials) & 15))) return NPF_EINVAL;
+  rc = npf::launch_main(A, partials, stream);
+  if (rc != NPF_OK) return rc;
+  rc = npf::launch_main(B, partials ? partials + fa : partials, stream);
+  if (rc != NPF_OK) return rc;
+  if (R.n_jobs) {
+    hipLaunchKernelGGL(npf::wgrad_reduce_kernel, dim3(65, R.n_jobs), dim3(256), 0, (hipStream_t)stream, R, (const float*)partials);
+    NPF_CHECK_LAUNCH();
+  }
+  return NPF_OK;
+}
diff --git a/npf_gwwaveform_amd/functional.py b/npf_gwwaveform_amd/functional.py
--- a/npf_gwwaveform_amd/functional.py
+++ b/npf_gwwaveform_amd/functional.py
@@ -21,6 +21,32 @@
     out = torch.empty((n_tasks, pts, F), dtype=torch.float32, device=pt.device)
     L.check(L.load().npf_unpack_pt(L.ptr(pt.contiguous()), n_tasks, pts, F, L.ptr(out), L.stream_ptr()), "npf_unpack_pt")
     return out
+
+
+def pad_pack_rows(rows: torch.Tensor, pts_padded: Optional[int] = None, pack: bool = True):
+    n_tasks, pts, d = rows.shape
+    Tp = pts if pts_padded is None else int(pts_padded)
+    rows = rows.contiguous()
+    keep = d == 4 and Tp == pts
+    if keep and not pack:
+        return rows, None
+    rows4 = None if keep else torch.empty((n_tasks, Tp, 4), dtype=torch.float32, device=rows.device)
+    pt = pt_empty(n_tasks, Tp, 4, rows.device) if pack else None
+    L.check(L.load().npf_pad_pack_rows(L.ptr(rows), n_tasks, pts, d, Tp, L.ptr(rows4), L.ptr(pt), L.stream_ptr()),
+            "npf_pad_pack_rows")
+    return (rows if keep else rows4), pt
+
+
+def range_fold(seen: torch.Tensor, *tensors: torch.Tensor) -> None:
+    ts = [t.contiguous() for t in tensors if t.numel()]
+    if len(ts) > 2:
+        raise ValueError("range_fold takes at most two tensors")
+    if not ts:
+        return
+    a = ts[0]
+    b = ts[1] if len(ts) > 1 else None
+    L.check(L.load().npf_range_fold(L.ptr(a), a.numel(), L.ptr(b), b.numel() if b is not None else 0, L.ptr(seen),
+                                    L.stream_ptr()), "npf_range_fold")
 
 
 class _PackFn(torch.autograd.Function):
diff --git a/npf_gwwaveform_amd/neuralproc.py b/npf_gwwaveform_amd/neuralproc.py
--- a/npf_gwwaveform_amd/neuralproc.py
+++ b/npf_gwwaveform_amd/neuralproc.py
@@ -570,14 +570,14 @@
     def _validate_inputs(self, X_cntxt, Y_cntxt, X_trgt, Y_trgt):
         self._check_tensors(X_cntxt, Y_cntxt, X_trgt, Y_trgt)
         if self.training and self.validate_inputs:
+            if self.validate_inputs == "deferred":
+                if getattr(self, "_range_seen", None) is None or self._range_seen.device != X_trgt.device:
+                    self._range_seen = torch.zeros((), device=X_trgt.device)
+                FN.range_fold(self._range_seen, X_cntxt, X_trgt)
+                return
             m = X_trgt.abs().amax() if X_trgt.numel() else X_trgt.new_zeros(())
             if X_cntxt.numel():
                 m = torch.maximum(m, X_cntxt.abs().amax())
-            if self.validate_inputs == "deferred":
-                if getattr(self, "_range_seen", None) is None or self._range_seen.device != m.device:
-                    self._range_seen = torch.zeros((), device=m.device)
-                self._range_seen.copy_(torch.maximum(self._range_seen, m))
-                return
             if not (m.item() <= 1.0):
                 lo = min(X_cntxt.min().item() if X_cntxt.numel() else 0.0, X_trgt.min().item())
                 hi = max(X_cntxt.max().item() if X_cntxt.numel() else 0.0, X_trgt.max().item())
diff --git a/npf_gwwaveform_amd/x6.py b/npf_gwwaveform_amd/x6.py
--- a/npf_gwwaveform_amd/x6.py
+++ b/npf_gwwaveform_amd/x6.py
@@ -194,10 +194,21 @@
 
 
 def _pad_rows4(X: torch.Tensor) -> torch.Tensor:
-    d = X.shape[-1]
-    if d == 4:
-        return X.contiguous()
-    return torch.cat((X, _zeros((*X.shape[:-1], 4 - d), X.device)), dim=-1)
+    return FN.pad_pack_rows(X, pack=False)[0]
+
+
+def _rows4_packed(X: torch.Tensor, pack: bool):
+    return FN.pad_pack_rows(X, pack=pack)
+
+
+def _packed_rows(ctx, name: str, X4: torch.Tensor) -> torch.Tensor:
+    pt = getattr(ctx, name, None)
+    setattr(ctx, name, None)
+    return pt if pt is not None else FN._pack(X4)
+
+
+def _grad_rows(g: torch.Tensor, n_out: int, pts_padded: int):
+    return FN.pad_pack_rows(g, pts_padded=pts_padded, pack=True)
 
 
 def _first_layer_matrix(W: torch.Tensor, n_out: int) -> torch.Tensor:
@@ -285,7 +296,7 @@
         fw = imgs[0]
         K_row, K_tr = task_images(K_pt, C, row=True, tr=train, width=F, bf16=bf16)
         V_row, V_tr = task_images(V_pt, C, row=train, tr=True, width=F, bf16=bf16)
-        X4 = _pad_rows4(X.detach())
+        X4, X4_pt = _rows4_packed(X.detach(), train and not bf16)
         W1p = _first_layer_matrix(W1, F)
         if bf16:
             X4, W1p = _r16(X4), _r16(W1p)
@@ -339,6 +350,7 @@
         if train:
             ctx.n_acts, ctx.n_bits = len(saved_acts), len(saved_bits)
             ctx.save_for_backward(X4, h1, bits_h1, Xt_enc, P, R_trgt, *saved_acts, *saved_bits, *imgs[1], V_row, K_tr, Wo)
+            ctx.x4_pt = X4_pt
         return rows[..., :n_out] if n_out != 4 else rows
 
     @staticmethod
@@ -358,9 +370,13 @@
         bw, (V_row, K_tr, Wo) = rest[:n_mid], rest[n_mid:]
         dev = g.device
         bf16 = ctx.bf16
-        g4 = g.contiguous() if n_out == 4 else torch.nn.functional.pad(g, (0, 4 - n_out)).contiguous()
         if bf16:
+            g4 = g.contiguous() if n_out == 4 else torch.nn.functional.pad(g, (0, 4 - n_out)).contiguous()
             g4 = _r16(g4)
+            dz_out = torch.zeros(CH.pt_shape(B, T, 4), dtype=torch.float32, device=dev)
+            dz_out[:, :, 0] = g4.view(B, tiles, 32, 4)
+        else:
+            g4, dz_out = _grad_rows(g, n_out, T)
         pt = lambda: CH.pt_empty(B, T, F, dev)
         pb = (lambda: CH.pt16_empty(B, T, F, dev)) if bf16 else pt
         x_acts, x_bits = acts[:n_x - 1], bits[:n_x - 1]
@@ -394,7 +410,7 @@
         jobs, grads = [], []
         dW1p = torch.empty((F, 4), dtype=torch.float32, device=dev)
         db1 = torch.empty((F,), dtype=torch.float32, device=dev) if ctx.has_b[0] else None
-        jobs.append(dict(dZ=dz1, A=FN._pack(X4), N=F, K=4, dW=dW1p, db=db1))
+        jobs.append(dict(dZ=dz1, A=_packed_rows(ctx, "x4_pt", X4), N=F, K=4, dW=dW1p, db=db1))
         grads += [None, db1]
         ins = [h1, *x_acts, R_trgt, *d_acts[:-1]]
         for j in range(n_mid):
@@ -402,8 +418,6 @@
             db = torch.empty((F,), dtype=torch.float32, device=dev) if (ctx.has_b[1 + j] and not (n_mrz and j == n_x)) else None
             jobs.append(dict(dZ=dz[j], A=ins[j], N=F, K=F, dW=dW, db=db))
             grads += [dW, db]
-        dz_out = torch.zeros(CH.pt_shape(B, T, 4), dtype=torch.float32, device=dev)
-        dz_out[:, :, 0] = g4.view(B, tiles, 32, 4)
         dWo = torch.empty((n_out, F), dtype=torch.float32, device=dev)
         dbo = torch.empty((n_out,), dtype=torch.float32, device=dev) if ctx.has_b[-1] else None
         jobs.append(dict(dZ=dz_out, A=d_acts[-1], N=n_out, K=F, dW=dWo, db=dbo))
@@ -481,11 +495,7 @@
         sv = list(ctx.saved_tensors)
         R_pt, acts, bits, bw, Wo = sv[0], sv[1:1 + n_mid], sv[1 + n_mid:1 + 2 * n_mid], sv[1 + 2 * n_mid:1 + 3 * n_mid], sv[-1]
         dev = g.device
-        if T == tiles * 32 and n_out == 4:
-            g4 = g.contiguous()
-        else:
-            g4 = torch.zeros((B, tiles * 32, 4), dtype=torch.float32, device=dev)
-            g4[:, :T, :n_out] = g
+        g4, dz_out = _grad_rows(g, n_out, tiles * 32)
         pt = lambda: CH.pt_empty(B, tiles * 32, F, dev)
         tr = ctx.trace_ref
         prog = Program(B, tiles, per_task=bool(n_mrz), width=F)
@@ -508,8 +518,6 @@
             db = torch.empty((F,), dtype=torch.float32, device=dev) if (ctx.has_b[j] and not (n_mrz and j == 0)) else None
             jobs.append(dict(dZ=dz[j], A=ins[j], N=F, K=F, dW=dW, db=db))
             grads += [dW, db]
-        dz_out = torch.zeros(CH.pt_shape(B, tiles * 32, 4), dtype=torch.float32, device=dev)
-        dz_out[:, :, 0] = g4.view(B, tiles, 32, 4)
         dWo = torch.empty((n_out, F), dtype=torch.float32, device=dev)
         dbo = torch.empty((n_out,), dtype=torch.float32, device=dev) if ctx.has_b[-1] else None
         jobs.append(dict(dZ=dz_out, A=acts[-1], N=n_out, K=F, dW=dWo, db=dbo))
@@ -624,7 +632,7 @@
         train = any(ctx.needs_input_grad)
         imgs = _weight_images([*x_W, Wq], (1, 2) if train else (1,), F)
         fw = imgs[0]
-        X4 = _pad_rows4(X.detach())
+        X4, X4_pt = _rows4_packed(X.detach(), train)
         pt = lambda: CH.pt_empty(B, P, F, dev)
         prog = Program(B, tiles, per_task=False, width=F)
         acts, bits = [], []
@@ -653,6 +661,7 @@
         ctx.set_materialize_grads(False)
         if train:
             ctx.save_for_backward(X4, h1, bits_h1, X_enc, *acts, *bits, *imgs[1])
+            ctx.x4_pt = X4_pt
         return X_enc, Q
 
     @staticmethod
@@ -696,7 +705,7 @@
             wjob(1 + i, dz, x_in[i], F, F)
         dz1 = pt()
         prog.op(mask_bits=bits_h1, store_in=dz1)
-        dW1p = wjob(0, dz1, FN._pack(X4), F, 4)
+        dW1p = wjob(0, dz1, _packed_rows(ctx, "x4_pt", X4), F, 4)
         prog.tag = "x-encoder + query projection dgrad"
         prog.launch()
         CH.run_wgrad(jobs, B, P, dev, tag="x-encoder + query projection weight gradients")
@@ -910,7 +919,7 @@
         Wr2p[:, :h] = Wr2.detach()
         imgs = _weight_images([*x_W, Wr2p, *f_W], (1, 2) if train else (1,), F, bf16)
         fw = imgs[0]
-        X4, Y4 = _pad_rows4(X.detach()), _pad_rows4(Y.detach())
+        (X4, X4_pt), (Y4, Y4_pt) = _rows4_packed(X.detach(), train and not bf16), _rows4_packed(Y.detach(), train and not bf16)
         W1p, Wr1p = _first_layer_matrix(W1, F), _first_layer_matrix(Wr1, h)
         if bf16:
             X4, Y4, W1p, Wr1p = _r16(X4), _r16(Y4), _r16(W1p), _r16(Wr1p)
@@ -966,6 +975,7 @@
         if train:
             ctx.n_acts = len(acts)
             ctx.save_for_backward(X4, Y4, h1, bits_h1, hy, bits_hy, *acts, *bits, *imgs[1])
+            ctx.x4_pt, ctx.y4_pt = X4_pt, Y4_pt
         return Xc_enc, R
 
     @staticmethod
@@ -1018,7 +1028,7 @@
             prog.op(mask_bits=m_bits, store_in=dz_m, store_in_f32=True, img=bw[n_x], w_ref=wref(n_x))
             prog.op(mask_bits=bits_hy, store_in=dz_hy)
             wjob(1 + n_x + 1, dz_m, hy, F, h, lda=F)
-            dWr1 = wjob(1 + n_x, dz_hy, FN._pack(Y4), h, 4, ldz=F)
+            dWr1 = wjob(1 + n_x, dz_hy, _packed_rows(ctx, "y4_pt", Y4), h, 4, ldz=F)
         if gK is not None or dz_m is not None:
             first = dict(in_pt=gK.contiguous(), pre_add=dz_m) if gK is not None else dict(in_pt=dz_m)
             x_in = [h1, *x_acts]
@@ -1033,7 +1043,7 @@
                 wjob(1 + i, dz, x_in[i], F, F)
             dz1 = pb()
             prog.op(mask_bits=bits_h1, store_in=dz1)
-            dW1p = wjob(0, dz1, FN._pack(X4), F, 4)
+            dW1p = wjob(0, dz1, _packed_rows(ctx, "x4_pt", X4), F, 4)
         prog.tag = "context side dgrad (XY-encoder, x-encoder)"
         prog.launch()
         CH.run_wgrad(jobs, B, Cn, dev, tag="context side weight gradients")
```

Measured after the change: 43.95 million target-points/s (median of 6 runs). No clear change (+1.1%).
